# scanner-research/scannertools

Measured on AMD Instinct MI355X. Metric: 1080p frames/sec (optical-flow + histogram ops), higher is better.
Workload: dtype f32 (u8 frames in; the box filter's running sums in f64, re-anchored every 32 rows / 8 columns, column sums handed to the row pass as f32)

## Files before the change

scannertools_amd/csrc/st_context.hip:

```cpp
#include <cstring>
#include <vector>
#include <mutex>
#include <chrono>
#include <cstdlib>

#include "st_internal.h"

int st_set_error(st_ctx* ctx, int status, const char* fmt, ...) {
  char buf[512];
  va_list ap;
  va_start(ap, fmt);
  vsnprintf(buf, sizeof(buf), fmt, ap);
  va_end(ap);
  if (ctx) ctx->last_error = buf;
  return status;
}

int st_enter(st_ctx* ctx) {
  if (!ctx) return ST_ERR_INVALID;
  ST_HIP(ctx, hipSetDevice(ctx->device));
  return ST_OK;
}

namespace {
struct CtxRegistry { std::mutex mu; std::vector<st_ctx*> live; };
CtxRegistry& registry() { static CtxRegistry* r = new CtxRegistry; return *r; }
long long now_ns() {
  return std::chrono::duration_cast<std::chrono::nanoseconds>(std::chrono::steady_clock::now().time_since_epoch()).count();
}
void reg_add(st_ctx* c) { CtxRegistry& r = registry(); std::lock_guard<std::mutex> lk(r.mu); r.live.push_back(c); }
void reg_remove(st_ctx* c) {
  CtxRegistry& r = registry();
  std::lock_guard<std::mutex> lk(r.mu);
  for (size_t i = 0; i < r.live.size(); ++i)
    if (r.live[i] == c) { r.live.erase(r.live.begin() + i); break; }
}
}

bool st_flow_call_begins(st_ctx* ctx) {
  const long long t = now_ns();
  ctx->flow_enter_ns.store(t, std::memory_order_relaxed);
  ctx->flow_busy.store(true, std::memory_order_release);
  if (ctx->concurrency_mode >= 0) return ctx->concurrency_mode != 0;
  constexpr long long kWindowNs = 50LL * 1000 * 1000;
  int others = 0;
  CtxRegistry& r = registry();
  std::lock_guard<std::mutex> lk(r.mu);
  for (st_ctx* o : r.live)
    if (o != ctx && o->device == ctx->device && o->flow_busy.load(std::memory_order_acquire) &&
        t - o->flow_enter_ns.load(std::memory_order_relaxed) < kWindowNs)
      ++others;
  return others >= 2;
}

ST_EXPORT int st_abi_version(void) { return ST_ABI_VERSION; }

#ifndef ST_SRC_HASH
#define ST_SRC_HASH "unknown"
#endif
#ifndef ST_BUILD_HOST
#define ST_BUILD_HOST "unknown"
#endif
#ifndef ST_BUILD_TIME
#define ST_BUILD_TIME "unknown"
#endif
ST_EXPORT const char* st_build_info(void) { return "src=" ST_SRC_HASH " host=" ST_BUILD_HOST " at=" ST_BUILD_TIME; }

ST_EXPORT const char* st_status_string(int status) {
  switch (status) {
    case ST_OK: return "ok";
    case ST_ERR_INVALID: return "invalid argument";
    case ST_ERR_HIP: return "HIP runtime error";
    case ST_ERR_OOM: return "out of device memory";
    case ST_ERR_UNSUPPORTED: return "unsupported parameters";
    default: return "unknown status";
  }
}

ST_EXPORT int st_device_count(int* count) {
  if (!count) return ST_ERR_INVALID;
  int n = 0;
  hipError_t e = hipGetDeviceCount(&n);
  if (e != hipSuccess) { *count = 0; return ST_ERR_HIP; }
  *count = n;
  return ST_OK;
}

static constexpr size_t kMinLdsBytes = 160 * 1024;

ST_EXPORT int st_ctx_create(int device_id, st_ctx** out_ctx) {
  if (!out_ctx) return ST_ERR_INVALID;
  *out_ctx = nullptr;
  int n = 0;
  if (hipGetDeviceCount(&n) != hipSuccess || device_id < 0 || device_id >= n) return ST_ERR_INVALID;
  if (hipSetDevice(device_id) != hipSuccess) return ST_ERR_HIP;
  st_ctx* c = new (std::nothrow) st_ctx();
  if (!c) return ST_ERR_OOM;
  c->device = device_id;
  if (hipStreamCreateWithFlags(&c->own_stream, hipStreamNonBlocking) != hipSuccess) {
    delete c;
    return ST_ERR_HIP;
  }
  c->stream = c->own_stream;
  if (const char* e = getenv("ST_ITER_TILE")) c->tile_mode = atoi(e);
  c->fold_gray = getenv("ST_PYR_FOLD_GRAY") != nullptr;
  if (const char* e = getenv("ST_POLY_U8")) c->poly_u8 = atoi(e) != 0;
  if (const char* e = getenv("ST_ITER_ROLES")) c->roles_mode = atoi(e);
  if (const char* e = getenv("ST_ROLES_NCW")) c->roles_ncw = atoi(e);
  if (const char* e = getenv("ST_PYR_ROLES")) c->pyr_roles = atoi(e);
  if (const char* e = getenv("ST_PYR_ROLES_RGB")) c->pyr_roles_rgb = atoi(e) != 0;
  if (const char* e = getenv("ST_CONV_TILE")) c->conv_tile = atoi(e);
  if (const char* e = getenv("ST_CONCURRENT")) c->concurrency_mode = atoi(e);
  hipDeviceProp_t prop;
  if (hipGetDeviceProperties(&prop, device_id) == hipSuccess) {
    c->num_cus = prop.multiProcessorCount;
    if (prop.sharedMemPerBlock < kMinLdsBytes || strncmp(prop.gcnArchName, "gfx950", 6) != 0) {
      (void)hipStreamDestroy(c->own_stream);
      delete c;
      return ST_ERR_UNSUPPORTED;
    }
  }
  reg_add(c);
  *out_ctx = c;
  return ST_OK;
}

ST_EXPORT int st_ctx_destroy(st_ctx* ctx) {
  if (!ctx) return ST_ERR_INVALID;
  reg_remove(ctx);
  (void)hipSetDevice(ctx->device);
  (void)hipStreamSynchronize(ctx->stream);
  for (auto& t : ctx->timing) {
    for (auto e : t.starts) (void)hipEventDestroy(e);
    for (auto e : t.stops) (void)hipEventDestroy(e);
  }
  if (ctx->ws) (void)hipFree(ctx->ws);
  st_jpeg_release(ctx);
  st_jpeg_enc_release(ctx);
  st_netin_release(ctx);
  st_detect_release(ctx);
  if (ctx->own_stream) (void)hipStreamDestroy(ctx->own_stream);
  delete ctx;
  return ST_OK;
}

ST_EXPORT int st_ctx_set_stream(st_ctx* ctx, void* hip_stream) {
  ST_TRY(st_enter(ctx));
  ST_HIP(ctx, hipStreamSynchronize(ctx->stream));
  ctx->flow_busy.store(false, std::memory_order_release);
  ctx->stream = (hipStream_t)hip_stream;
  return ST_OK;
}

ST_EXPORT int st_ctx_reset_stream(st_ctx* ctx) {
  ST_TRY(st_enter(ctx));
  ST_HIP(ctx, hipStreamSynchronize(ctx->stream));
  ctx->flow_busy.store(false, std::memory_order_release);
  ctx->stream = ctx->own_stream;
  return ST_OK;
}

ST_EXPORT int st_ctx_sync(st_ctx* ctx) {
  ST_TRY(st_enter(ctx));
  ST_HIP(ctx, hipStreamSynchronize(ctx->stream));
  ctx->flow_busy.store(false, std::memory_order_release);
  return ST_OK;
}

ST_EXPORT int st_ctx_flow_concurrent(st_ctx* ctx) { return ctx && ctx->flow_concurrent ? 1 : 0; }

ST_EXPORT int st_ctx_set_workspace_limit(st_ctx* ctx, size_t bytes) {
  if (!ctx) return ST_ERR_INVALID;
  ctx->ws_limit = bytes ? bytes : ((size_t)64 << 30);
  return ST_OK;
}

ST_EXPORT int st_ctx_release_workspace(st_ctx* ctx) {
  ST_TRY(st_enter(ctx));
  ST_HIP(ctx, hipStreamSynchronize(ctx->stream));
  if (ctx->ws) ST_HIP(ctx, hipFree(ctx->ws));
  ctx->ws = nullptr;
  ctx->ws_bytes = 0;
  ctx->ws_off = 0;
  return ST_OK;
}

ST_EXPORT const char* st_ctx_last_error(const st_ctx* ctx) { return ctx ? ctx->last_error.c_str() : "null context"; }

int st_ws_reserve(st_ctx* ctx, size_t total_bytes) {
  ctx->ws_off = 0;
  if (total_bytes <= ctx->ws_bytes) return ST_OK;
  if (total_bytes > ctx->ws_limit)
    return st_set_error(ctx, ST_ERR_OOM, "workspace request %zu exceeds limit %zu", total_bytes, ctx->ws_limit);
  ST_HIP(ctx, hipStreamSynchronize(ctx->stream));
  if (ctx->ws) ST_HIP(ctx, hipFree(ctx->ws));
  ctx->ws = nullptr;
  ctx->ws_bytes = 0;
  size_t want = total_bytes + total_bytes / 8;
  if (want > ctx->ws_limit) want = total_bytes;
  hipError_t e = hipMalloc(&ctx->ws, want);
  if (e != hipSuccess) {
    (void)hipGetLastError();
    want = total_bytes;
    e = hipMalloc(&ctx->ws, want);
  }
  if (e != hipSuccess) {
    (void)hipGetLastError();
    ctx->ws = nullptr;
    return st_set_error(ctx, ST_ERR_OOM, "hipMalloc(%zu) failed: %s", want, hipGetErrorString(e));
  }
  ctx->ws_bytes = want;
  return ST_OK;
}

void st_ws_reset(st_ctx* ctx) { ctx->ws_off = 0; }

void* st_ws_alloc(st_ctx* ctx, size_t bytes) {
  size_t off = st_align_up(ctx->ws_off);
  if (off + bytes > ctx->ws_bytes) return nullptr;
  ctx->ws_off = off + bytes;
  return (char*)ctx->ws + off;
}

ST_EXPORT int st_ctx_timing_enable(st_ctx* ctx, unsigned kernel_mask) {
  if (!ctx) return ST_ERR_INVALID;
  ctx->timing_mask = kernel_mask;
  return ST_OK;
}

static int timing_fold(st_ctx* ctx, st_timing_slot& t) {
  for (size_t i = 0; i < t.used; ++i) {
    float ms = 0.f;
    ST_HIP(ctx, hipEventElapsedTime(&ms, t.starts[i], t.stops[i]));
    t.total_ms += ms;
  }
  t.used = 0;
  return ST_OK;
}

ST_EXPORT int st_ctx_timing_reset(st_ctx* ctx) {
  ST_TRY(st_enter(ctx));
  ST_HIP(ctx, hipStreamSynchronize(ctx->stream));
  for (auto& t : ctx->timing) {
    t.used = 0;
    t.launches = 0;
    t.total_ms = 0.0;
  }
  return ST_OK;
}

ST_EXPORT int st_ctx_timing_read(st_ctx* ctx, int kernel_id, int* launches, double* total_ms) {
  ST_TRY(st_enter(ctx));
  if (kernel_id < 0 || kernel_id >= ST_K_COUNT) return ST_ERR_INVALID;
  ST_HIP(ctx, hipStreamSynchronize(ctx->stream));
  st_timing_slot& t = ctx->timing[kernel_id];
  ST_TRY(timing_fold(ctx, t));
  if (launches) *launches = t.launches;
  if (total_ms) *total_ms = t.total_ms;
  return ST_OK;
}

int st_time_begin(st_ctx* ctx, int id) {
  if (!(ctx->timing_mask & (1u << id))) return ST_OK;
  st_timing_slot& t = ctx->timing[id];
  if (t.used == t.starts.size()) {
    if (t.used >= 4096) {
      ST_HIP(ctx, hipStreamSynchronize(ctx->stream));
      ST_TRY(timing_fold(ctx, t));
    } else {
      hipEvent_t a, b;
      ST_HIP(ctx, hipEventCreate(&a));
      if (hipEventCreate(&b) != hipSuccess) {
        (void)hipEventDestroy(a);
        return st_set_error(ctx, ST_ERR_HIP, "timing: hipEventCreate failed");
      }
      t.starts.push_back(a);
      t.stops.push_back(b);
    }
  }
  ST_HIP(ctx, hipEventRecord(t.starts[t.used], ctx->stream));
  return ST_OK;
}

int st_time_dispatch(st_ctx* ctx, int id, hipEvent_t* start, hipEvent_t* stop) {
  *start = *stop = nullptr;
  if (!(ctx->timing_mask & (1u << id))) return ST_OK;
  st_timing_slot& t = ctx->timing[id];
  if (t.used == t.starts.size()) {
    if (t.used >= 4096) {
      ST_HIP(ctx, hipStreamSynchronize(ctx->stream));
      ST_TRY(timing_fold(ctx, t));
    } else {
      hipEvent_t a, b;
      ST_HIP(ctx, hipEventCreate(&a));
      if (hipEventCreate(&b) != hipSuccess) {
        (void)hipEventDestroy(a);
        return st_set_error(ctx, ST_ERR_HIP, "timing: hipEventCreate failed");
      }
      t.starts.push_back(a);
      t.stops.push_back(b);
    }
  }
  *start = t.starts[t.used];
  *stop = t.stops[t.used];
  t.used++;
  t.launches++;
  return ST_OK;
}

int st_time_end(st_ctx* ctx, int id) {
  if (!(ctx->timing_mask & (1u << id))) return ST_OK;
  st_timing_slot& t = ctx->timing[id];
  if (t.used >= t.stops.size()) return st_set_error(ctx, ST_ERR_INVALID, "timing: bracket closed without an open one");
  ST_HIP(ctx, hipEventRecord(t.stops[t.used], ctx->stream));
  t.used++;
  t.launches++;
  return ST_OK;
}
```

scannertools_amd/csrc/st_farneback.hip:

```cpp
#include <hip/hip_ext.h>

#include <cmath>
#include <cstdlib>
#include <cstring>

#include "st_internal.h"

namespace {

constexpr int kMaxTaps = 32;
constexpr int kMaxPolyN = 7;

inline int cv_round(double v) { return (int)lrint(v); }

struct LevelGeom {
  int lh, lw, ksize;
  double sigma, scale;
};

int fb_levels(int h, int w, const st_fb_params& p) {
  int k;
  double scale = 1;
  for (k = 0; k < p.num_levels; ++k) {
    scale *= p.pyr_scale;
// ... 644 lines not shown
          v.w = (hm[3] + hp[3]) * a.k0[0] + hc[3] * a.k0[1];
          *reinterpret_cast<float4*>(o0 + (size_t)yo * w + X0 + 4 * t) = v;
        }
#pragma unroll
        for (int j = 0; j < 4; ++j) { hm[j] = hc[j]; hc[j] = hp[j]; }
      }
      {
#pragma unroll
        for (int e = 0; e < 2; ++e) {
          const float nA = pf_rowfilter<3>(bb + 3 + 2 * e, a.k1), nB = pf_rowfilter<3>(bb + 4 + 2 * e, a.k1);
#pragma unroll
          for (int j = 0; j < 3; ++j) { r1A[e][j] = r1A[e][j + 1]; r1B[e][j] = r1B[e][j + 1]; }
          r1A[e][3] = nA; r1B[e][3] = nB;
        }
        if ((r & 1) == 0) {
          const int dy = (y - 2) >> 1;
          if (live && dy >= (Y0 >> 1) && dy < (Y1 >> 1)) {
            float2 v;
            {
              const float b00 = pf_colfilter<3>(r1A[0], a.k1), b01 = pf_colfilter<3>(r1B[0], a.k1);
              const float b10 = pf_colfilter<3>(r1A[0] + 1, a.k1), b11 = pf_colfilter<3>(r1B[0] + 1, a.k1);
              v.x = ((b00 + b01) + (b10 + b11)) * 0.25f;
            }
            {
              const float b00 = pf_colfilter<3>(r1A[1], a.k1), b01 = pf_colfilter<3>(r1B[1], a.k1);
              const float b10 = pf_colfilter<3>(r1A[1] + 1, a.k1), b11 = pf_colfilter<3>(r1B[1] + 1, a.k1);
              v.y = ((b00 + b01) + (b10 + b11)) * 0.25f;
            }
            *reinterpret_cast<float2*>(o1 + (size_t)dy * (w >> 1) + (X0 >> 1) + 2 * t) = v;
          }
        }
      }
      {
        const float nA = pf_rowfilter<9>(bb + 1, a.k2), nB = pf_rowfilter<9>(bb + 2, a.k2);
#pragma unroll
        for (int j = 0; j < 9; ++j) { r2A[j] = r2A[j + 1]; r2B[j] = r2B[j + 1]; }
        r2A[9] = nA; r2B[9] = nB;
        if ((r & 3) == 2) {
          const int dy = (y - 6) >> 2;
          if (live && dy >= (Y0 >> 2) && dy < (Y1 >> 2)) {
            const float b00 = pf_colfilter<9>(r2A, a.k2), b01 = pf_colfilter<9>(r2B, a.k2);
            const float b10 = pf_colfilter<9>(r2A + 1, a.k2), b11 = pf_colfilter<9>(r2B + 1, a.k2);
            const float q0 = b00 * 0.5f + b01 * 0.5f, q1 = b10 * 0.5f + b11 * 0.5f;
            o2[(size_t)dy * (w >> 2) + (X0 >> 2) + t] = q0 * 0.5f + q1 * 0.5f;
          }
        }
      }
      {
        unsigned dw[6];
#pragma unroll
        for (int q = 0; q < 6; ++q) dw[q] = s[2 * u + q];
        float cb[21];
#pragma unroll
        for (int q = 0; q < 6; ++q) {
          const unsigned d = __builtin_amdgcn_alignbyte(dw[q + 1 < 6 ? q + 1 : 5], dw[q], (unsigned)half);
#pragma unroll
          for (int k = 0; k < 4; ++k)
            if (4 * q + k < 21) cb[4 * q + k] = pf_byte(d, k);
        }
        const float n3 = pf_rowfilter<19>(cb + 2, a.k3);
#pragma unroll
        for (int j = 0; j < 19; ++j) r3[j] = r3[j + 1];
        r3[19] = n3;
        if (r == 5) {
          const int dy = (y - 13) >> 3;
          if (dy >= (Y0 >> 3) && dy < (Y1 >> 3)) {
            const float c0 = pf_colfilter<19>(r3, a.k3), c1 = pf_colfilter<19>(r3 + 1, a.k3);
            const float p0 = __shfl_xor(c0, 32), p1 = __shfl_xor(c1, 32);
            if (half == 0 && live3) {
              const float q0 = c0 * 0.5f + p0 * 0.5f, q1 = c1 * 0.5f + p1 * 0.5f;
              o3[(size_t)dy * (w >> 3) + (X0 >> 3) + u] = q0 * 0.5f + q1 * 0.5f;
            }
          }
        }
      }
    }
    if (b + 1 < nb) stash(buf ^ 1);
    __syncthreads();
  }
}

typedef unsigned pf_u3nt __attribute__((ext_vector_type(3), aligned(4)));
__device__ __forceinline__ pf_u3nt pf_fetch_rgb(const uint8_t* __restrict__ row, int col0, int w, const PyrFusedArgs& a) {
  if (col0 >= 0 && col0 + 3 < w) return __builtin_nontemporal_load(reinterpret_cast<const pf_u3nt*>(row + 3 * col0));
  pf_u3nt v = {0u, 0u, 0u};
  if (col0 >= w + 8 || col0 < -8) return v;
#pragma unroll
  for (int k = 0; k < 4; ++k) v.x |= pf_gray1(row + 3 * d_reflect101(col0 + k, w), a) << (8 * k);
  return v;
}
__device__ __forceinline__ unsigned pf_gray_of(pf_u3nt v, bool inside, const PyrFusedArgs& a) {
  if (!inside) return v.x;
  const unsigned w0 = v.x, w1 = v.y, w2 = v.z;
  const int g0 = (int)((w0 & 0xff) * a.cb + ((w0 >> 8) & 0xff) * a.cg + ((w0 >> 16) & 0xff) * a.cr + a.rnd) >> a.shift;
  const int g1 = (int)((w0 >> 24) * a.cb + (w1 & 0xff) * a.cg + ((w1 >> 8) & 0xff) * a.cr + a.rnd) >> a.shift;
  const int g2 = (int)(((w1 >> 16) & 0xff) * a.cb + (w1 >> 24) * a.cg + (w2 & 0xff) * a.cr + a.rnd) >> a.shift;
  const int g3 = (int)(((w2 >> 8) & 0xff) * a.cb + ((w2 >> 16) & 0xff) * a.cg + (w2 >> 24) * a.cr + a.rnd) >> a.shift;
  return (unsigned)g0 | ((unsigned)g1 << 8) | ((unsigned)g2 << 16) | ((unsigned)g3 << 24);
}

template <int ROLE, bool L0 = true, bool RGB = false>
__device__ __forceinline__ void pyr_role_run(const PyrFusedArgs& a, unsigned (*srow)[PF_RB][PF_ROWDW]) {
  const int t = threadIdx.x & 255, lane = t & 63, wv = t >> 6;
  const int h = a.h, w = a.w;
  const int SW = a.strip_w;
  const int X0 = blockIdx.x * SW;
  const int Y0 = blockIdx.y * a.rows_per_seg, Y1 = min(h, Y0 + a.rows_per_seg);
  const size_t np = (size_t)h * w;
  const uint8_t* __restrict__ g = RGB ? st_gl(a.frames[blockIdx.z]) : a.gray + (size_t)blockIdx.z * np;
  const int gw = RGB ? 3 * w : w;
  float* __restrict__ o0 = a.img0 + (size_t)blockIdx.z * np;
  float* __restrict__ o1 = a.img1 + (size_t)blockIdx.z * (np >> 2);
  float* __restrict__ o2 = a.img2 + (size_t)blockIdx.z * (np >> 4);
  float* __restrict__ o3 = a.img3 + (size_t)blockIdx.z * (np >> 6);
  const int u = wv * 32 + (lane & 31), half = lane >> 5;
  const bool live = 4 * t < SW && X0 + 4 * t < w;
  const bool live3 = 8 * u < SW && X0 + 8 * u < w;
  const int hq = t & 3, hrow = (t >> 2) & 7;
  const int hcol = hq < 2 ? X0 - 8 + 4 * hq : X0 + SW + 4 * (hq - 2);
  const int hidx = hq < 2 ? hq : 2 + (SW >> 2) + (hq - 2);
  const bool in_t = X0 + 4 * t + 3 < w, in_h = hcol >= 0 && hcol + 3 < w;
  uint8_t* __restrict__ gout = RGB ? a.gray_out + (size_t)blockIdx.z * np : nullptr;

  unsigned pre[3], preh = 0u;
  pf_u3nt raw[3] = {{0u, 0u, 0u}, {0u, 0u, 0u}, {0u, 0u, 0u}}, rawh = {0u, 0u, 0u};
  auto fetch = [&](int ybase) {
#pragma unroll
    for (int j = 0; j < 3; ++j) {
      const int r = ROLE + 3 * j;
      if (r < PF_RB) {
        if (RGB) { if (4 * t < SW) raw[j] = pf_fetch_rgb(g + (size_t)d_reflect101(ybase + r, h) * gw, X0 + 4 * t, w, a); }
        else pre[j] = pf_load4(g + (size_t)d_reflect101(ybase + r, h) * gw, X0 + 4 * t, w);
      }
    }
    if (ROLE == 0 && t < 32) {
      if (RGB) rawh = pf_fetch_rgb(g + (size_t)d_reflect101(ybase + hrow, h) * gw, hcol, w, a);
      else preh = pf_load4(g + (size_t)d_reflect101(ybase + hrow, h) * gw, hcol, w);
    }
  };
  auto stash = [&](int buf, int ybase) {
    const bool own = RGB && ybase >= Y0 && ybase < Y1;
    if (4 * t < SW) {
#pragma unroll
      for (int j = 0; j < 3; ++j) {
        const int r = ROLE + 3 * j;
        if (r < PF_RB) {
          const unsigned v = RGB ? pf_gray_of(raw[j], in_t, a) : pre[j];
          srow[buf][r][2 + t] = v;
          if (RGB && own && live) *reinterpret_cast<unsigned*>(gout + (size_t)(ybase + r) * w + X0 + 4 * t) = v;
        }
      }
    }
    if (ROLE == 0 && t < 32) srow[buf][hrow][hidx] = RGB ? pf_gray_of(rawh, in_h, a) : preh;
  };

  float hm[4], hc[4], r1A[2][4], r1B[2][4];
  float r2A[10], r2B[10];
  float r3[20];
  if (ROLE == 0) {
#pragma unroll
    for (int j = 0; j < 4; ++j) { hm[j] = hc[j] = 0.f; r1A[0][j] = r1A[1][j] = r1B[0][j] = r1B[1][j] = 0.f; }
  } else if (ROLE == 1) {
#pragma unroll
    for (int j = 0; j < 10; ++j) r2A[j] = r2B[j] = 0.f;
  } else {
#pragma unroll
    for (int j = 0; j < 20; ++j) r3[j] = 0.f;
  }

  const int nb = (Y1 - Y0) / PF_RB + 2;
  fetch(Y0 - PF_RB);
  stash(0, Y0 - PF_RB);
  __syncthreads();
  for (int b = 0; b < nb; ++b) {
    const int ybase = Y0 - PF_RB + b * PF_RB;
    const int buf = b & 1;
    if (b + 1 < nb) fetch(ybase + PF_RB);
#pragma unroll
    for (int r = 0; r < PF_RB; ++r) {
      const int y = ybase + r;
      const unsigned* __restrict__ s = srow[buf][r];
      if (ROLE == 0) {
        const unsigned d0 = s[t + 1], d1 = s[t + 2], d2 = s[t + 3];
        float bb[12];
#pragma unroll
        for (int k = 0; k < 4; ++k) { bb[k] = pf_byte(d0, k); bb[4 + k] = pf_byte(d1, k); bb[8 + k] = pf_byte(d2, k); }
        if (L0) {
          float hp[4];
#pragma unroll
          for (int j = 0; j < 4; ++j) hp[j] = bb[4 + j] * a.k0[1] + (bb[3 + j] + bb[5 + j]) * a.k0[0];
          const int yo = y - 1;
          if (live && yo >= Y0 && yo < Y1) {
            float4 v;
            v.x = (hm[0] + hp[0]) * a.k0[0] + hc[0] * a.k0[1];
            v.y = (hm[1] + hp[1]) * a.k0[0] + hc[1] * a.k0[1];
            v.z = (hm[2] + hp[2]) * a.k0[0] + hc[2] * a.k0[1];
            v.w = (hm[3] + hp[3]) * a.k0[0] + hc[3] * a.k0[1];
            *reinterpret_cast<float4*>(o0 + (size_t)yo * w + X0 + 4 * t) = v;
          }
#pragma unroll
          for (int j = 0; j < 4; ++j) { hm[j] = hc[j]; hc[j] = hp[j]; }
        }
        {
#pragma unroll
          for (int e = 0; e < 2; ++e) {
            const float nA = pf_rowfilter<3>(bb + 3 + 2 * e, a.k1), nB = pf_rowfilter<3>(bb + 4 + 2 * e, a.k1);
#pragma unroll
            for (int j = 0; j < 3; ++j) { r1A[e][j] = r1A[e][j + 1]; r1B[e][j] = r1B[e][j + 1]; }
            r1A[e][3] = nA; r1B[e][3] = nB;
          }
          if ((r & 1) == 0) {
            const int dy = (y - 2) >> 1;
            if (live && dy >= (Y0 >> 1) && dy < (Y1 >> 1)) {
              float2 v;
              {
                const float b00 = pf_colfilter<3>(r1A[0], a.k1), b01 = pf_colfilter<3>(r1B[0], a.k1);
                const float b10 = pf_colfilter<3>(r1A[0] + 1, a.k1), b11 = pf_colfilter<3>(r1B[0] + 1, a.k1);
                v.x = ((b00 + b01) + (b10 + b11)) * 0.25f;
              }
              {
                const float b00 = pf_colfilter<3>(r1A[1], a.k1), b01 = pf_colfilter<3>(r1B[1], a.k1);
                const float b10 = pf_colfilter<3>(r1A[1] + 1, a.k1), b11 = pf_colfilter<3>(r1B[1] + 1, a.k1);
                v.y = ((b00 + b01) + (b10 + b11)) * 0.25f;
              }
              *reinterpret_cast<float2*>(o1 + (size_t)dy * (w >> 1) + (X0 >> 1) + 2 * t) = v;
            }
          }
        }
      } else if (ROLE == 1) {
        const unsigned d0 = s[t + 1], d1 = s[t + 2], d2 = s[t + 3];
        float bb[12];
#pragma unroll
        for (int k = 0; k < 4; ++k) { bb[k] = pf_byte(d0, k); bb[4 + k] = pf_byte(d1, k); bb[8 + k] = pf_byte(d2, k); }
        const float nA = pf_rowfilter<9>(bb + 1, a.k2), nB = pf_rowfilter<9>(bb + 2, a.k2);
#pragma unroll
        for (int j = 0; j < 9; ++j) { r2A[j] = r2A[j + 1]; r2B[j] = r2B[j + 1]; }
        r2A[9] = nA; r2B[9] = nB;
        if ((r & 3) == 2) {
          const int dy = (y - 6) >> 2;
          if (live && dy >= (Y0 >> 2) && dy < (Y1 >> 2)) {
            const float b00 = pf_colfilter<9>(r2A, a.k2), b01 = pf_colfilter<9>(r2B, a.k2);
            const float b10 = pf_colfilter<9>(r2A + 1, a.k2), b11 = pf_colfilter<9>(r2B + 1, a.k2);
            const float q0 = b00 * 0.5f + b01 * 0.5f, q1 = b10 * 0.5f + b11 * 0.5f;
            o2[(size_t)dy * (w >> 2) + (X0 >> 2) + t] = q0 * 0.5f + q1 * 0.5f;
          }
        }
      } else {
        unsigned dw[6];
#pragma unroll
        for (int q = 0; q < 6; ++q) dw[q] = s[2 * u + q];
        float cb[21];
#pragma unroll
        for (int q = 0; q < 6; ++q) {
          const unsigned d = __builtin_amdgcn_alignbyte(dw[q + 1 < 6 ? q + 1 : 5], dw[q], (unsigned)half);
#pragma unroll
          for (int k = 0; k < 4; ++k)
            if (4 * q + k < 21) cb[4 * q + k] = pf_byte(d, k);
        }
        const float n3 = pf_rowfilter<19>(cb + 2, a.k3);
#pragma unroll
        for (int j = 0; j < 19; ++j) r3[j] = r3[j + 1];
        r3[19] = n3;
        if (r == 5) {
          const int dy = (y - 13) >> 3;
          if (dy >= (Y0 >> 3) && dy < (Y1 >> 3)) {
            const float c0 = pf_colfilter<19>(r3, a.k3), c1 = pf_colfilter<19>(r3 + 1, a.k3);
            const float p0 = __shfl_xor(c0, 32), p1 = __shfl_xor(c1, 32);
            if (half == 0 && live3) {
              const float q0 = c0 * 0.5f + p0 * 0.5f, q1 = c1 * 0.5f + p1 * 0.5f;
              o3[(size_t)dy * (w >> 3) + (X0 >> 3) + u] = q0 * 0.5f + q1 * 0.5f;
            }
          }
        }
      }
    }
    if (b + 1 < nb) stash(buf ^ 1, ybase + PF_RB);
    __syncthreads();
  }
}

template <bool L0, bool RGB = false>
__global__ __launch_bounds__(768) void k_pyr_roles(PyrFusedArgs a) {
  static_assert(!(L0 && RGB), "the RGB-source instance leaves level 0 to k_polyexp_u8");
  __shared__ unsigned srow[2][PF_RB][PF_ROWDW];
  const int role = threadIdx.x >> 8;
  if (role == 0) pyr_role_run<0, L0, RGB>(a, srow);
  else if (role == 1) pyr_role_run<1, true, RGB>(a, srow);
  else pyr_role_run<2, true, RGB>(a, srow);
}

typedef float f2u __attribute__((ext_vector_type(2), aligned(4)));
typedef float f4v16 __attribute__((ext_vector_type(4)));
__device__ __forceinline__ __amdgpu_buffer_rsrc_t st_rsrc(const void* base, size_t bytes) {
  return __builtin_amdgcn_make_buffer_rsrc(const_cast<void*>(base), 0, (int)(bytes > 0xfffffffcull ? 0xfffffffcull : bytes), 0x00020000);
}
__device__ __forceinline__ float bld1(__amdgpu_buffer_rsrc_t r, unsigned voff, unsigned soff) {
  return __builtin_bit_cast(float, __builtin_amdgcn_raw_buffer_load_b32(r, (int)voff, (int)soff, 0));
}
template <int AUX = 0>
__device__ __forceinline__ void bst1(__amdgpu_buffer_rsrc_t r, unsigned voff, unsigned soff, float v) {
  __builtin_amdgcn_raw_buffer_store_b32(__builtin_bit_cast(unsigned, v), r, (int)voff, (int)soff, AUX);
}
template <int AUX = 0>
__device__ __forceinline__ void bst4(__amdgpu_buffer_rsrc_t r, unsigned voff, float4 v) {
  typedef unsigned u4 __attribute__((ext_vector_type(4)));
  u4 q;
  q.x = __builtin_bit_cast(unsigned, v.x); q.y = __builtin_bit_cast(unsigned, v.y);
  q.z = __builtin_bit_cast(unsigned, v.z); q.w = __builtin_bit_cast(unsigned, v.w);
  __builtin_amdgcn_raw_buffer_store_b128(q, r, (int)voff, 0, AUX);
}

__device__ __forceinline__ float ldf(const float* __restrict__ base, unsigned byte_off) {
  return *reinterpret_cast<const float*>(reinterpret_cast<const char*>(base) + byte_off);
}
__device__ __forceinline__ f2u ldf2(const float* __restrict__ base, unsigned byte_off) {
  return *reinterpret_cast<const f2u*>(reinterpret_cast<const char*>(base) + byte_off);
}
__device__ __forceinline__ float4 ldf4(const float* __restrict__ base, unsigned byte_off) {
  return *reinterpret_cast<const float4*>(reinterpret_cast<const char*>(base) + byte_off);
}



struct PolyArgs {
  const float* img;
  const uint8_t* gray;
  float* R;
  int h, w, rows_per_seg;
  PolyCoef c;
};

constexpr int PE_RB = 4;
constexpr int PE_OUT = 240;

template <int N, class A, bool U8 = false>
__device__ __forceinline__ void polyexp_body(const A& a, const float* __restrict__ img, float* __restrict__ Rbase, int h, int w,
                                             int rows_per_seg, int bx, int by, int z, const uint8_t* __restrict__ gray = nullptr) {
  constexpr int PXW = 3 * PE_RB + 1;
  __shared__ float sv[2][256 * PXW];
  const int tid = threadIdx.x;
  const int np = h * w;
  const float* __restrict__ I = img + (size_t)z * (size_t)np;
  float* __restrict__ R = Rbase + (size_t)z * 5 * (size_t)np;
  const int x = bx * PE_OUT - N + tid;
  const int xc = d_clamp(x, 0, w - 1);
  const int y0 = by * rows_per_seg;
  const int y1 = min(h, y0 + rows_per_seg);
  const bool writer = tid >= N && tid < N + PE_OUT && x < w;
  const unsigned voff = 4u * (unsigned)xc;
  const unsigned xo = writer ? (unsigned)x : 0u;
  const unsigned xo16 = writer ? 16u * xo : 0x80000000u, xo4 = writer ? 4u * xo : 0x80000000u;
  const __amdgpu_buffer_rsrc_t Rnull = st_rsrc(R, 0);
  const __amdgpu_buffer_rsrc_t Ib = st_rsrc(I, 4 * (size_t)np), Rb = st_rsrc(R, 20 * (size_t)np);
  auto opaque = [](unsigned v) { asm volatile("" : "+v"(v)); return v; };
  auto src = [&](int row) { return bld1(Ib, voff, 4u * (unsigned)w * (unsigned)d_clamp(row, 0, h - 1)); };
  const __amdgpu_buffer_rsrc_t Gb = st_rsrc(U8 ? gray + (size_t)z * (size_t)np : nullptr, U8 ? (size_t)np : 0);
  const unsigned lx = !U8 ? 0u : xc == 0 ? 0u : xc >= w - 2 ? (unsigned)(w - 4) : (unsigned)(xc - 1);
  const unsigned wsel = xc == 0 ? 0x00000202u : xc == w - 1 ? 0x02020000u : xc == w - 2 ? 0x01020100u : 0x00010201u;
  auto graw = [&](int grow) { return (unsigned)__builtin_amdgcn_raw_buffer_load_b32(Gb, (int)lx, (int)((unsigned)w * (unsigned)grow), 0); };
  auto hsum = [&](unsigned d) { return __builtin_amdgcn_udot4(d, wsel, 0u, false); };
  auto blur16 = [](unsigned a0, unsigned b0, unsigned c0) { return (float)(a0 + 2u * b0 + c0) * 0.0625f; };
  unsigned hsB = 0, hsC = 0;

  float ring[2 * N + PE_RB];
  if (!U8) {
#pragma unroll
    for (int j = 0; j < 2 * N + PE_RB; ++j) ring[j] = src(y0 - N + j);
  } else {
    constexpr int NR = 2 * N + PE_RB;
    const int r0 = d_clamp(y0 - N, 0, h - 1);
    const unsigned rm = graw(d_reflect101(r0 - 1, h)), rc = graw(r0);
    unsigned rn[NR];
#pragma unroll
    for (int j = 0; j < NR; ++j) rn[j] = graw(d_reflect101(d_clamp(y0 - N + j, 0, h - 1) + 1, h));
    unsigned hsA = hsum(rm);
    hsB = hsum(rc);
#pragma unroll
    for (int j = 0; j < NR; ++j) {
      hsC = hsum(rn[j]);
      ring[j] = blur16(hsA, hsB, hsC);
      if (j + 1 < NR && d_clamp(y0 - N + j + 1, 0, h - 1) != d_clamp(y0 - N + j, 0, h - 1)) { hsA = hsB; hsB = hsC; }
    }
  }

  int buf = 0;
  for (int y = y0; y < y1; y += PE_RB) {
#pragma unroll
    for (int r = 0; r < PE_RB; ++r) {
      float r0 = ring[r + N] * a.c.g[0], r1 = 0.f, r2 = 0.f;
#pragma unroll
      for (int k = 1; k <= N; ++k) {
        float p = ring[r + N - k] + ring[r + N + k];
        float t0 = r0 + a.c.g[k] * p;
        float t1 = r2 + a.c.xxg[k] * p;
        p = ring[r + N + k] - ring[r + N - k];
        float t2 = r1 + a.c.xg[k] * p;
        r0 = t0; r1 = t2; r2 = t1;
      }
      float* __restrict__ d = &sv[buf][tid * PXW + 3 * r];
      d[0] = r0; d[1] = r1; d[2] = r2;
    }
    float nxt[PE_RB];
    unsigned nraw[PE_RB];
#pragma unroll
    for (int r = 0; r < PE_RB; ++r) {
      if (U8) nraw[r] = graw(d_reflect101(min(y + PE_RB + N + r, h - 1) + 1, h));
      else nxt[r] = src(y + PE_RB + N + r);
    }
    __syncthreads();
    if (U8) {
      float last = ring[2 * N + PE_RB - 1];
#pragma unroll
      for (int r = 0; r < PE_RB; ++r) {
        if (y + PE_RB + N + r <= h - 1) {
          const unsigned hsA = hsB;
          hsB = hsC; hsC = hsum(nraw[r]);
          last = blur16(hsA, hsB, hsC);
        }
        nxt[r] = last;
      }
    }
#pragma unroll
    for (int j = 0; j < 2 * N; ++j) ring[j] = ring[j + PE_RB];
#pragma unroll
    for (int r = 0; r < PE_RB; ++r) ring[2 * N + r] = nxt[r];
    __builtin_amdgcn_sched_barrier(0);
    {
      const unsigned pix0 = opaque(writer ? (unsigned)(tid - N) * PXW : 0u);
#pragma unroll
      for (int r = 0; r < PE_RB; ++r) {
        const float* __restrict__ s = &sv[buf][pix0 + 3 * r];
        float g0 = a.c.g[0];
        const float cx = s[N * PXW], cy = s[N * PXW + 1], cz = s[N * PXW + 2];
        double b1 = cx * g0, b2 = 0, b3 = cy * g0, b4 = 0, b5 = cz * g0, b6 = 0;
#pragma unroll
        for (int k = 1; k <= N; ++k) {
          const float* __restrict__ pp = s + (N + k) * PXW;
          const float* __restrict__ mm = s + (N - k) * PXW;
          const float p0 = pp[0], m0 = mm[0];
          const float p1 = pp[1], m1 = mm[1];
          const float p2 = pp[2], m2 = mm[2];
          double tg = p0 + m0;
          g0 = a.c.g[k];
          b1 = __builtin_fma(tg, (double)g0, b1);
          b4 = __builtin_fma(tg, (double)a.c.xxg[k], b4);
          b2 += (p0 - m0) * a.c.xg[k];
          b3 += (p1 + m1) * g0;
          b6 += (p1 - m1) * a.c.xg[k];
          b5 += (p2 + m2) * g0;
        }
        const bool row_ok = y + r < y1;
        const unsigned rowo = (unsigned)(y + r) * (unsigned)w;
        bst4(row_ok ? Rb : Rnull, xo16 + 16u * rowo, make_float4((float)(b3 * a.c.ig11), (float)(b2 * a.c.ig11),
                                                                                  (float)(b1 * a.c.ig03 + b5 * a.c.ig33), (float)(b1 * a.c.ig03 + b4 * a.c.ig33)));
        bst1(row_ok ? Rb : Rnull, xo4, 16u * (unsigned)np + 4u * rowo, (float)(b6 * a.c.ig55));
      }
    }
    buf ^= 1;
  }
}

template <int N>
__global__ __launch_bounds__(256) void k_polyexp(PolyArgs a) {
  polyexp_body<N>(a, a.img, a.R, a.h, a.w, a.rows_per_seg, (int)blockIdx.x, (int)blockIdx.y, (int)blockIdx.z);
}

template <int N>
__global__ __launch_bounds__(256, 1) void k_polyexp_u8(PolyArgs a) {
  polyexp_body<N, PolyArgs, true>(a, nullptr, a.R, a.h, a.w, a.rows_per_seg, (int)blockIdx.x, (int)blockIdx.y, (int)blockIdx.z, a.gray);
}

struct PolyLevel {
  const float* img;
  float* R;
  int h, w, rows_per_seg, strips, block0;
};
struct PolyArgsML {
  PolyLevel lv[4];
  int nlv;
  PolyCoef c;
};
template <int N>
__global__ __launch_bounds__(256) void k_polyexp_ml(PolyArgsML a) {
  int l = 0;
#pragma unroll
  for (int i = 1; i < 4; ++i)
    if (i < a.nlv && (int)blockIdx.x >= a.lv[i].block0) l = i;
  const float* img = a.lv[0].img; float* R = a.lv[0].R;
  int h = a.lv[0].h, w = a.lv[0].w, rows = a.lv[0].rows_per_seg, strips = a.lv[0].strips, b0 = a.lv[0].block0;
#pragma unroll
  for (int i = 1; i < 4; ++i)
    if (l == i) { img = a.lv[i].img; R = a.lv[i].R; h = a.lv[i].h; w = a.lv[i].w; rows = a.lv[i].rows_per_seg; strips = a.lv[i].strips; b0 = a.lv[i].block0; }
  const int local = (int)blockIdx.x - b0;
  polyexp_body<N>(a, img, R, h, w, rows, local % strips, local / strips, (int)blockIdx.y);
}

__device__ __forceinline__ void update_matrices_px(const float* __restrict__ R0, const float* __restrict__ R1,
                                                   int np, int h, int w, int x, int y, float dx, float dy,
                                                   float m[5]) {
  const int o = y * w + x;
  float fx = x + dx, fy = y + dy;
  const int x1 = (int)floorf(fx), y1 = (int)floorf(fy);
  float r2, r3, r4, r5, r6;
  fx -= x1; fy -= y1;
  const float4 q = reinterpret_cast<const float4*>(R0)[o];
  const float q0 = q.x, q1 = q.y, q2 = q.z, q3 = q.w, q4 = R0[4 * (size_t)np + o];
  if ((unsigned)x1 < (unsigned)(w - 1) && (unsigned)y1 < (unsigned)(h - 1)) {
    const float a00 = (1.f - fx) * (1.f - fy), a01 = fx * (1.f - fy), a10 = (1.f - fx) * fy, a11 = fx * fy;
    const int gi = y1 * w + x1;
    const float4* __restrict__ Q = reinterpret_cast<const float4*>(R1);
    const float* __restrict__ S = R1 + 4 * (size_t)np;
    const float4 t0 = Q[gi], t1 = Q[gi + 1], b0 = Q[gi + w], b1 = Q[gi + w + 1];
    r2 = a00 * t0.x + a01 * t1.x + a10 * b0.x + a11 * b1.x;
    r3 = a00 * t0.y + a01 * t1.y + a10 * b0.y + a11 * b1.y;
    r4 = a00 * t0.z + a01 * t1.z + a10 * b0.z + a11 * b1.z;
    r5 = a00 * t0.w + a01 * t1.w + a10 * b0.w + a11 * b1.w;
    r6 = a00 * S[gi] + a01 * S[gi + 1] + a10 * S[gi + w] + a11 * S[gi + w + 1];
    r4 = (q2 + r4) * 0.5f;
    r5 = (q3 + r5) * 0.5f;
    r6 = (q4 + r6) * 0.25f;
  } else {
    r2 = r3 = 0.f;
    r4 = q2;
    r5 = q3;
    r6 = q4 * 0.5f;
  }
  r2 = (q0 - r2) * 0.5f;
  r3 = (q1 - r3) * 0.5f;
  r2 += r4 * dy + r6 * dx;
  r3 += r6 * dy + r5 * dx;
  constexpr int BORDER = 5;
  if ((unsigned)(x - BORDER) >= (unsigned)(w - BORDER * 2) || (unsigned)(y - BORDER) >= (unsigned)(h - BORDER * 2)) {
    auto bsel = [](int i) -> float { return i < 2 ? 0.14f : 0.4472f; };
    const float scale = (x < BORDER ? bsel(x) : 1.f) * (x >= w - BORDER ? bsel(w - x - 1) : 1.f) *
                        (y < BORDER ? bsel(y) : 1.f) * (y >= h - BORDER ? bsel(h - y - 1) : 1.f);
    r2 *= scale; r3 *= scale; r4 *= scale; r5 *= scale; r6 *= scale;
  }
  m[0] = r4 * r4 + r6 * r6;
  m[1] = (r4 + r5) * r6;
  m[2] = r5 * r5 + r6 * r6;
  m[3] = r4 * r2 + r6 * r3;
  m[4] = r6 * r2 + r5 * r3;
}


struct UmLoads {
  float4 q;
  float qs;
  float4 t0, t1, b0, b1;
  f2u ts, bs;
};

__device__ __forceinline__ void um_gather(const float* __restrict__ R1, unsigned single, unsigned gi, unsigned gb, UmLoads& L);
__device__ __forceinline__ void um_issue(const float* __restrict__ R0, const float* __restrict__ R1, int np, int h,
                                         int w, int x, int y, float2 f, UmLoads& L) {
  float fx = x + f.x, fy = y + f.y;
  const int x1 = (int)floorf(fx), y1 = (int)floorf(fy);
  const bool inb = (unsigned)x1 < (unsigned)(w - 1) && (unsigned)y1 < (unsigned)(h - 1);
  const unsigned gi = inb ? (unsigned)(y1 * w + x1) : 0u;
  const unsigned gb = gi + (inb ? (unsigned)w : 0u);
  const unsigned o = (unsigned)(y * w + x);
  const unsigned single = 16u * (unsigned)np;
  L.q = ldf4(R0, 16u * o);
  L.qs = ldf(R0, single + 4u * o);
  um_gather(R1, single, gi, gb, L);
}

__device__ __forceinline__ void um_gather(const float* __restrict__ R1, unsigned single, unsigned gi, unsigned gb, UmLoads& L) {
  L.t0 = ldf4(R1, 16u * gi);
  L.t1 = ldf4(R1 + 4, 16u * gi);
  L.b0 = ldf4(R1, 16u * gb);
  L.b1 = ldf4(R1 + 4, 16u * gb);
  L.ts = ldf2(R1, single + 4u * gi);
  L.bs = ldf2(R1, single + 4u * gb);
}

__device__ __forceinline__ void um_finish(const UmLoads& L, int h, int w, int x, int y, float2 f, float m[5]) {
  const float dx = f.x, dy = f.y;
  float fx = x + dx, fy = y + dy;
  const int x1 = (int)floorf(fx), y1 = (int)floorf(fy);
  fx -= x1; fy -= y1;
  const bool inb = (unsigned)x1 < (unsigned)(w - 1) && (unsigned)y1 < (unsigned)(h - 1);
  float r2, r3, r4, r5, r6;
  if (inb) {
    const float a00 = (1.f - fx) * (1.f - fy), a01 = fx * (1.f - fy), a10 = (1.f - fx) * fy, a11 = fx * fy;
    r2 = a00 * L.t0.x + a01 * L.t1.x + a10 * L.b0.x + a11 * L.b1.x;
    r3 = a00 * L.t0.y + a01 * L.t1.y + a10 * L.b0.y + a11 * L.b1.y;
    r4 = a00 * L.t0.z + a01 * L.t1.z + a10 * L.b0.z + a11 * L.b1.z;
    r5 = a00 * L.t0.w + a01 * L.t1.w + a10 * L.b0.w + a11 * L.b1.w;
    r6 = a00 * L.ts.x + a01 * L.ts.y + a10 * L.bs.x + a11 * L.bs.y;
    r4 = (L.q.z + r4) * 0.5f;
    r5 = (L.q.w + r5) * 0.5f;
    r6 = (L.qs + r6) * 0.25f;
  } else {
    r2 = r3 = 0.f;
    r4 = L.q.z;
    r5 = L.q.w;
    r6 = L.qs * 0.5f;
  }
  r2 = (L.q.x - r2) * 0.5f;
  r3 = (L.q.y - r3) * 0.5f;
  r2 += r4 * dy + r6 * dx;
  r3 += r6 * dy + r5 * dx;
  constexpr int BORDER = 5;
  if ((unsigned)(x - BORDER) >= (unsigned)(w - BORDER * 2) || (unsigned)(y - BORDER) >= (unsigned)(h - BORDER * 2)) {
    auto bsel = [](int i) -> float { return i < 2 ? 0.14f : 0.4472f; };
    const float scale = (x < BORDER ? bsel(x) : 1.f) * (x >= w - BORDER ? bsel(w - x - 1) : 1.f) *
                        (y < BORDER ? bsel(y) : 1.f) * (y >= h - BORDER ? bsel(h - y - 1) : 1.f);
    r2 *= scale; r3 *= scale; r4 *= scale; r5 *= scale; r6 *= scale;
  }
  m[0] = r4 * r4 + r6 * r6;
  m[1] = (r4 + r5) * r6;
  m[2] = r5 * r5 + r6 * r6;
  m[3] = r4 * r2 + r6 * r3;
  m[4] = r6 * r2 + r5 * r3;
}


struct UMArgs {
  const float* R;
  const int* pairs;
  const float* R1_direct;
  const float* flow;
  const float* coarse;
  float* M;
  int h, w, ch, cw;
  double scale_x, scale_y;
  float mul;
};

__device__ __forceinline__ float2 ld_flow(const float* __restrict__ f, int idx) {
  return *reinterpret_cast<const float2*>(reinterpret_cast<const char*>(f) + 8u * (unsigned)idx);
}

__global__ __launch_bounds__(256) void k_update_matrices(UMArgs a) {
  const int h = a.h, w = a.w;
  const size_t np = (size_t)h * w;
  const int pr = blockIdx.y;
  const float* R0;
  const float* R1;
  if (a.pairs) {
    R0 = a.R + (size_t)a.pairs[2 * pr] * 5 * np;
    R1 = a.R + (size_t)a.pairs[2 * pr + 1] * 5 * np;
  } else {
    R0 = a.R;
    R1 = a.R1_direct;
  }
  float* __restrict__ M = a.M + (size_t)pr * 5 * np;
  for (size_t i = (size_t)blockIdx.x * blockDim.x + threadIdx.x; i < np; i += (size_t)gridDim.x * blockDim.x) {
    const int y = (int)(i / w), x = (int)(i - (size_t)y * w);
    float dx = 0.f, dy = 0.f;
    if (a.coarse) {
      const float* C = a.coarse + (size_t)pr * 2 * a.ch * a.cw;
      float fx = (float)((x + 0.5) * a.scale_x - 0.5);
      int sx = (int)floorf(fx);
      fx -= sx;
      if (sx < 0) { fx = 0.f; sx = 0; }
      if (sx >= a.cw - 1) { fx = 0.f; sx = a.cw - 1; }
      float fy = (float)((y + 0.5) * a.scale_y - 0.5);
      int sy = (int)floorf(fy);
      fy -= sy;
      const int ya = d_clamp(sy, 0, a.ch - 1), yb = d_clamp(sy + 1, 0, a.ch - 1);
      const float a1 = fx, a0 = 1.f - fx, b0 = 1.f - fy, b1 = fy;
      float2 ta, tb;
      if (sx + 1 < a.cw) {
        float2 p = ld_flow(C, ya * a.cw + sx), q = ld_flow(C, ya * a.cw + sx + 1);
        ta.x = p.x * a0 + q.x * a1; ta.y = p.y * a0 + q.y * a1;
        p = ld_flow(C, yb * a.cw + sx); q = ld_flow(C, yb * a.cw + sx + 1);
        tb.x = p.x * a0 + q.x * a1; tb.y = p.y * a0 + q.y * a1;
      } else {
        float2 p = ld_flow(C, ya * a.cw + sx);
        ta.x = p.x * 1.f; ta.y = p.y * 1.f;
        p = ld_flow(C, yb * a.cw + sx);
        tb.x = p.x * 1.f; tb.y = p.y * 1.f;
      }
      dx = (ta.x * b0 + tb.x * b1) * a.mul;
      dy = (ta.y * b0 + tb.y * b1) * a.mul;
    } else if (a.flow) {
      float2 f = ld_flow(a.flow + (size_t)pr * 2 * np, (int)i);
      dx = f.x; dy = f.y;
    }
    float m[5];
    update_matrices_px(R0, R1, np, h, w, x, y, dx, dy, m);
    M[i] = m[0]; M[np + i] = m[1]; M[2 * np + i] = m[2]; M[3 * np + i] = m[3]; M[4 * np + i] = m[4];
  }
}

struct BlurArgs {
  const float* R;
  const int* pairs;
  const float* R1_direct;
  const float* Min;
  float* Mout;
  float* flow;
  float* const* flow_ptrs;
  int h, w, rows_per_seg, m;
  int update, write_flow;
  double scale;
};

constexpr int BLUR_T = 256;

__global__ __launch_bounds__(BLUR_T) void k_blur_update(BlurArgs a) {
  __shared__ double sv[2][5][BLUR_T];
  const int tid = threadIdx.x;
  const int h = a.h, w = a.w, m = a.m;
  const size_t np = (size_t)h * w;
  const int pr = blockIdx.z;
  const float* __restrict__ Min = a.Min + (size_t)pr * 5 * np;
  const int x = (int)blockIdx.x * (BLUR_T - 2 * m) - m + tid;
  const int xc = d_clamp(x, 0, w - 1);
  const int y0 = blockIdx.y * a.rows_per_seg;
  const int y1 = min(h, y0 + a.rows_per_seg);
  const bool writer = tid >= m && tid < BLUR_T - m && x < w;

  const float* R0 = nullptr;
  const float* R1 = nullptr;
  float* Mout = nullptr;
  if (a.update) {
    if (a.pairs) {
      R0 = a.R + (size_t)a.pairs[2 * pr] * 5 * np;
      R1 = a.R + (size_t)a.pairs[2 * pr + 1] * 5 * np;
    } else {
      R0 = a.R;
      R1 = a.R1_direct;
    }
    Mout = a.Mout + (size_t)pr * 5 * np;
  }
  float* flow = nullptr;
  if (a.write_flow) flow = a.flow_ptrs ? st_gl(a.flow_ptrs[pr]) : a.flow + (size_t)pr * 2 * np;

  double vs[5] = {0, 0, 0, 0, 0};
  if (y0 == 0) {
#pragma unroll
    for (int c = 0; c < 5; ++c) vs[c] = (double)(Min[c * np + xc] * (float)(m + 2));
    for (int yy = 1; yy < m; ++yy) {
      const size_t o = (size_t)min(yy, h - 1) * w + xc;
#pragma unroll
      for (int c = 0; c < 5; ++c) vs[c] += (double)Min[c * np + o];
    }
    const size_t oa = (size_t)min(m, h - 1) * w + xc;
#pragma unroll
    for (int c = 0; c < 5; ++c) {
      const float d = Min[c * np + oa] - Min[c * np + xc];
      vs[c] += d;
    }
  } else {
    for (int dy = -m; dy <= m; ++dy) {
      const size_t o = (size_t)d_clamp(y0 + dy, 0, h - 1) * w + xc;
#pragma unroll
      for (int c = 0; c < 5; ++c) vs[c] += (double)Min[c * np + o];
    }
  }

  for (int y = y0; y < y1; ++y) {
    double(*s)[BLUR_T] = sv[y & 1];
#pragma unroll
    for (int c = 0; c < 5; ++c) s[c][tid] = vs[c];
    if (y + 1 < y1) {
      const size_t oa = (size_t)d_clamp(y + 1 + m, 0, h - 1) * w + xc;
      const size_t ob = (size_t)d_clamp(y - m, 0, h - 1) * w + xc;
#pragma unroll
      for (int c = 0; c < 5; ++c) {
        const float d = Min[c * np + oa] - Min[c * np + ob];
        vs[c] += d;
      }
    }
    __syncthreads();
    if (writer) {
      double g[5];
#pragma unroll
      for (int c = 0; c < 5; ++c) {
        double t = s[c][tid - m];
        for (int k = -m + 1; k <= m; ++k) t += s[c][tid + k];
        g[c] = t * a.scale;
      }
      const double idet = 1. / (g[0] * g[2] - g[1] * g[1] + 1e-3);
      const float u = (float)((g[0] * g[4] - g[1] * g[3]) * idet);
      const float v = (float)((g[2] * g[3] - g[1] * g[4]) * idet);
      const size_t o = (size_t)y * w + x;
      if (flow) *reinterpret_cast<float2*>(flow + 2 * o) = make_float2(u, v);
      if (a.update) {
        float mm[5];
        update_matrices_px(R0, R1, np, h, w, x, y, u, v, mm);
#pragma unroll
        for (int c = 0; c < 5; ++c) Mout[c * np + o] = mm[c];
      }
    }
  }
}

constexpr int B2_T = 256, B2_HALO = 8, B2_OUT = B2_T - 2 * B2_HALO, B2_RB = 5, B2_SEG = 5;
constexpr int B2_NSEG = B2_OUT / B2_SEG;

template <int M>
__global__ __launch_bounds__(B2_T, 2) void k_blur_update_v2(BlurArgs a) {
  constexpr int W = 2 * M + 1;
  static_assert(W % B2_RB == 0 && M <= B2_HALO, "ring period must be a multiple of the batch");
  __shared__ float V[B2_RB][5][B2_T];
  __shared__ float2 F[B2_RB][B2_T];
  const int tid = threadIdx.x;
  const int h = a.h, w = a.w;
  const int np = h * w;
  const int pr = blockIdx.z;
  const float* __restrict__ Min = a.Min + (size_t)pr * 5 * (size_t)np;
  const int x = (int)blockIdx.x * B2_OUT - B2_HALO + tid;
  const int xc = d_clamp(x, 0, w - 1);
  const int y0 = blockIdx.y * a.rows_per_seg;
  const int y1 = min(h, y0 + a.rows_per_seg);
  const bool writer = tid >= B2_HALO && tid < B2_T - B2_HALO && x < w;

  const float* R0 = nullptr;
  const float* R1 = nullptr;
  float* Mout = nullptr;
  if (a.update) {
    if (a.pairs) {
      R0 = a.R + (size_t)a.pairs[2 * pr] * 5 * (size_t)np;
      R1 = a.R + (size_t)a.pairs[2 * pr + 1] * 5 * (size_t)np;
    } else {
      R0 = a.R;
      R1 = a.R1_direct;
    }
    Mout = a.Mout + (size_t)pr * 5 * (size_t)np;
  }
  float* flow = nullptr;
  if (a.write_flow) flow = a.flow_ptrs ? st_gl(a.flow_ptrs[pr]) : a.flow + (size_t)pr * 2 * (size_t)np;

  float ring[W][5];
  double vs[5];
#pragma unroll
  for (int s = 0; s < W; ++s) {
    const int o = d_clamp(y0 - M + s, 0, h - 1) * w + xc;
#pragma unroll
    for (int c = 0; c < 5; ++c) ring[s][c] = Min[c * np + o];
  }
  if (y0 == 0) {
#pragma unroll
    for (int c = 0; c < 5; ++c) vs[c] = (double)(ring[M][c] * (float)(M + 2));
#pragma unroll
    for (int yy = 1; yy < M; ++yy)
#pragma unroll
      for (int c = 0; c < 5; ++c) vs[c] += (double)ring[M + yy][c];
#pragma unroll
    for (int c = 0; c < 5; ++c) {
      const float d = ring[2 * M][c] - ring[M][c];
      vs[c] += d;
    }
  } else {
#pragma unroll
    for (int c = 0; c < 5; ++c) vs[c] = 0;
#pragma unroll
    for (int s = 0; s < W; ++s)
#pragma unroll
      for (int c = 0; c < 5; ++c) vs[c] += (double)ring[s][c];
  }

  for (int yb = y0; yb < y1; yb += W) {
#pragma unroll
    for (int b = 0; b < W / B2_RB; ++b) {
      const int ybb = yb + b * B2_RB;
      if (ybb < y1) {
        float nw[B2_RB][5];
#pragma unroll
        for (int r = 0; r < B2_RB; ++r) {
          const int o = d_clamp(ybb + r + M + 1, 0, h - 1) * w + xc;
#pragma unroll
          for (int c = 0; c < 5; ++c) nw[r][c] = Min[c * np + o];
        }
#pragma unroll
        for (int r = 0; r < B2_RB; ++r) {
#pragma unroll
          for (int c = 0; c < 5; ++c) {
            V[r][c][tid] = (float)vs[c];
            const float d = nw[r][c] - ring[b * B2_RB + r][c];
            vs[c] += d;
            ring[b * B2_RB + r][c] = nw[r][c];
          }
        }
        __syncthreads();
        if (tid < B2_RB * B2_NSEG) {
          const int r = tid / B2_NSEG, sg = tid - r * B2_NSEG;
          const int j0 = B2_HALO + sg * B2_SEG;
          double t[5];
#pragma unroll
          for (int c = 0; c < 5; ++c) {
            const float* vp = &V[r][c][j0 - M];
            double acc = vp[0];
#pragma unroll
            for (int i = 1; i < W; ++i) acc += (double)vp[i];
            t[c] = acc;
            __builtin_amdgcn_sched_barrier(0);
          }
#pragma unroll
          for (int i = 0; i < B2_SEG; ++i) {
            if (i > 0) {
#pragma unroll
              for (int c = 0; c < 5; ++c) t[c] += (double)V[r][c][j0 + i + M] - (double)V[r][c][j0 + i - M - 1];
            }
            const double g11 = t[0] * a.scale, g12 = t[1] * a.scale, g22 = t[2] * a.scale;
            const double h1 = t[3] * a.scale, h2 = t[4] * a.scale;
            const double idet = 1. / (g11 * g22 - g12 * g12 + 1e-3);
            F[r][j0 + i] = make_float2((float)((g11 * h2 - g12 * h1) * idet), (float)((g22 * h1 - g12 * h2) * idet));
            __builtin_amdgcn_sched_barrier(0);
          }
        }
        __syncthreads();
        if (writer) {
#pragma unroll
          for (int r = 0; r < B2_RB; ++r) {
            const int y = ybb + r;
            if (y < y1) {
              const float2 f = F[r][tid];
              const int o = y * w + x;
              if (flow) *reinterpret_cast<float2*>(flow + 2 * o) = f;
              if (a.update) {
                float mm[5];
                update_matrices_px(R0, R1, np, h, w, x, y, f.x, f.y, mm);
#pragma unroll
                for (int c = 0; c < 5; ++c) Mout[c * np + o] = mm[c];
              }
            }
          }
        }
      }
    }
  }
}

struct IterArgs {
  const float* R;
  const int* pairs;
  const float* R1_direct;
  const float* flow_in;
  const float* coarse;
  float* flow_out;
  float* const* flow_ptrs;
  int h, w, ch, cw, rows_per_seg;
  int out_w;
  double scale_x, scale_y;
  float mul;
  double scale;
};

enum { FLOW_ZERO = 0, FLOW_FIELD = 1, FLOW_COARSE = 2, FLOW_ANY = 3,
       FLOW_COARSE2 = 4 };

struct CoarseX {
  int sx;
  float a0, a1;
  bool pair;
};

__device__ __forceinline__ CoarseX coarse_x(const IterArgs& a, int x) {
  CoarseX cx;
  float fx = (float)((x + 0.5) * a.scale_x - 0.5);
  int sx = (int)floorf(fx);
  fx -= sx;
  if (sx < 0) { fx = 0.f; sx = 0; }
  if (sx >= a.cw - 1) { fx = 0.f; sx = a.cw - 1; }
  cx.sx = sx; cx.a1 = fx; cx.a0 = 1.f - fx; cx.pair = sx + 1 < a.cw;
  return cx;
}

typedef float f4u8 __attribute__((ext_vector_type(4), aligned(8)));
struct FlowRaw {
  f4u8 pa, pb;
};

template <int MODE = FLOW_ANY>
__device__ __forceinline__ void flow_issue(const IterArgs& a, const float* __restrict__ fin,
                                           const float* __restrict__ C, const CoarseX& cx, int x, int y, FlowRaw& r) {
  if (MODE == FLOW_COARSE || MODE == FLOW_COARSE2 || (MODE == FLOW_ANY && C)) {
    const float fy = (float)((y + 0.5) * a.scale_y - 0.5);
    const int sy = (int)floorf(fy);
    const int ya = d_clamp(sy, 0, a.ch - 1), yb = d_clamp(sy + 1, 0, a.ch - 1);
    if (cx.pair) {
      r.pa = *reinterpret_cast<const f4u8*>(reinterpret_cast<const char*>(C) + 8u * (unsigned)(ya * a.cw + cx.sx));
      r.pb = *reinterpret_cast<const f4u8*>(reinterpret_cast<const char*>(C) + 8u * (unsigned)(yb * a.cw + cx.sx));
    } else {
      float2 p = ld_flow(C, ya * a.cw + cx.sx);
      r.pa.x = p.x; r.pa.y = p.y; r.pa.z = 0.f; r.pa.w = 0.f;
      p = ld_flow(C, yb * a.cw + cx.sx);
      r.pb.x = p.x; r.pb.y = p.y; r.pb.z = 0.f; r.pb.w = 0.f;
    }
  } else if (MODE == FLOW_FIELD || (MODE == FLOW_ANY && fin)) {
    const float2 p = ld_flow(fin, y * a.w + x);
    r.pa.x = p.x; r.pa.y = p.y;
  }
}

template <int MODE = FLOW_ANY>
__device__ __forceinline__ float2 flow_finish(const IterArgs& a, const float* __restrict__ fin,
                                              const float* __restrict__ C, const CoarseX& cx, int y, const FlowRaw& r) {
  if (MODE == FLOW_COARSE || MODE == FLOW_COARSE2 || (MODE == FLOW_ANY && C)) {
    float fy = (float)((y + 0.5) * a.scale_y - 0.5);
    const int sy = (int)floorf(fy);
    fy -= sy;
    const float a1 = cx.a1, a0 = cx.a0, b0 = 1.f - fy, b1 = fy;
    float2 ta, tb;
    if (cx.pair) {
      ta.x = r.pa.x * a0 + r.pa.z * a1; ta.y = r.pa.y * a0 + r.pa.w * a1;
      tb.x = r.pb.x * a0 + r.pb.z * a1; tb.y = r.pb.y * a0 + r.pb.w * a1;
    } else {
      ta.x = r.pa.x * 1.f; ta.y = r.pa.y * 1.f;
      tb.x = r.pb.x * 1.f; tb.y = r.pb.y * 1.f;
    }
    return make_float2((ta.x * b0 + tb.x * b1) * a.mul, (ta.y * b0 + tb.y * b1) * a.mul);
  }
  if (MODE == FLOW_FIELD || (MODE == FLOW_ANY && fin)) return make_float2(r.pa.x, r.pa.y);
  return make_float2(0.f, 0.f);
}

__device__ __forceinline__ int coarse_row0(const IterArgs& a, int y0) {
  return (int)floorf((float)((y0 + 0.5) * a.scale_y - 0.5));
}

template <int MODE = FLOW_ANY>
__device__ __forceinline__ float2 iter_flow_at(const IterArgs& a, const float* __restrict__ fin,
                                               const float* __restrict__ C, const CoarseX& cx, int x, int y) {
  FlowRaw r;
  flow_issue<MODE>(a, fin, C, cx, x, y, r);
  return flow_finish<MODE>(a, fin, C, cx, y, r);
}

constexpr int F3_GROUP = 8, F3_SW = 8, F3_NSEG = B2_OUT / F3_SW, F3_RING = 16, F3_ANCHOR = 32;
constexpr int F3_PADW = B2_T + B2_T / 8;
static_assert(B2_OUT % F3_SW == 0 && F3_GROUP * F3_NSEG <= B2_T && F3_ANCHOR % F3_RING == 0 && F3_RING % F3_GROUP == 0, "bad v3 geometry");
__device__ __forceinline__ constexpr int f3_pos(int x) { return x + (x >> 3); }

__device__ __forceinline__ int coarse2_row(int y) { return ((y + 1) >> 1) - 1; }

template <int RB>
struct FlowRawN {
  f4u8 row[RB / 2 + 2];
};
template <int RB>
__device__ __forceinline__ void coarseN_issue(const IterArgs& a, const float* __restrict__ C, const CoarseX& cx, int y0,
                                              FlowRawN<RB>& r) {
  const int s = coarse2_row(y0);
#pragma unroll
  for (int j = 0; j < RB / 2 + 2; ++j) {
    const int yy = d_clamp(s + j, 0, a.ch - 1);
    if (cx.pair) {
      r.row[j] = *reinterpret_cast<const f4u8*>(reinterpret_cast<const char*>(C) + 8u * (unsigned)(yy * a.cw + cx.sx));
    } else {
      const float2 p = ld_flow(C, yy * a.cw + cx.sx);
      r.row[j].x = p.x; r.row[j].y = p.y; r.row[j].z = 0.f; r.row[j].w = 0.f;
    }
  }
}
template <int RB>
__device__ __forceinline__ void coarse2_finish_batch(const IterArgs& a, const CoarseX& cx, int y0, const int (&ys)[RB],
                                                     const FlowRawN<RB>& r, float2 (&out)[RB]) {
  const int s = coarse2_row(y0);
  const float a1 = cx.a1, a0 = cx.a0;
  float2 hx[RB / 2 + 2];
#pragma unroll
  for (int j = 0; j < RB / 2 + 2; ++j) {
    if (cx.pair) {
      hx[j].x = r.row[j].x * a0 + r.row[j].z * a1; hx[j].y = r.row[j].y * a0 + r.row[j].w * a1;
    } else {
      hx[j].x = r.row[j].x * 1.f; hx[j].y = r.row[j].y * 1.f;
    }
  }
#pragma unroll
  for (int i = 0; i < RB; ++i) {
    const int y = ys[i];
    const int idx = coarse2_row(y) - s;
    const float fy = (y & 1) ? 0.25f : 0.75f;
    const float b0 = 1.f - fy, b1 = fy;
    float2 ta = hx[0], tb = hx[1];
#pragma unroll
    for (int j = 1; j <= RB / 2; ++j)
      if (idx == j) { ta = hx[j]; tb = hx[j + 1]; }
    out[i] = make_float2((ta.x * b0 + tb.x * b1) * a.mul, (ta.y * b0 + tb.y * b1) * a.mul);
  }
}

struct Coarse2Window {
  float2 hx0, hx1;
  f4u8 raw;
};
__device__ __forceinline__ void coarse2_row_issue(const IterArgs& a, const float* __restrict__ C, const CoarseX& cx, int u,
                                                  f4u8& r) {
  const int yy = d_clamp(u, 0, a.ch - 1);
  if (cx.pair) {
    r = *reinterpret_cast<const f4u8*>(reinterpret_cast<const char*>(C) + 8u * (unsigned)(yy * a.cw + cx.sx));
  } else {
    const float2 p = ld_flow(C, yy * a.cw + cx.sx);
    r.x = p.x; r.y = p.y; r.z = 0.f; r.w = 0.f;
  }
}
__device__ __forceinline__ float2 coarse2_row_hx(const CoarseX& cx, const f4u8& r) {
  float2 hx;
  if (cx.pair) {
    hx.x = r.x * cx.a0 + r.z * cx.a1; hx.y = r.y * cx.a0 + r.w * cx.a1;
  } else {
    hx.x = r.x * 1.f; hx.y = r.y * 1.f;
  }
  return hx;
}
__device__ __forceinline__ void coarse2_window_start(const IterArgs& a, const float* __restrict__ C, const CoarseX& cx,
                                                     int yu, Coarse2Window& win) {
  const int u = coarse2_row(yu);
  f4u8 r0, r1;
  coarse2_row_issue(a, C, cx, u, r0);
  coarse2_row_issue(a, C, cx, u + 1, r1);
  coarse2_row_issue(a, C, cx, u + 2, win.raw);
  win.hx0 = coarse2_row_hx(cx, r0);
  win.hx1 = coarse2_row_hx(cx, r1);
}
__device__ __forceinline__ void coarse2_window_batch(const IterArgs& a, const float* __restrict__ C, const CoarseX& cx, int yu,
                                                     Coarse2Window& win, float2 (&out)[2]) {
  const int u = coarse2_row(yu);
  const float2 hx2 = coarse2_row_hx(cx, win.raw);
#pragma unroll
  for (int i = 0; i < 2; ++i) {
    const int y = min(yu + i, a.h - 1);
    const bool second = coarse2_row(yu + i) > u;
    const float fy = (y & 1) ? 0.25f : 0.75f;
    const float b0 = 1.f - fy, b1 = fy;
    const float2 ta = second ? win.hx1 : win.hx0, tb = second ? hx2 : win.hx1;
    out[i] = make_float2((ta.x * b0 + tb.x * b1) * a.mul, (ta.y * b0 + tb.y * b1) * a.mul);
  }
  win.hx0 = win.hx1;
  win.hx1 = hx2;
  coarse2_row_issue(a, C, cx, u + 3, win.raw);
}

template <int RB>
__device__ __forceinline__ float2 coarseN_finish(const IterArgs& a, const CoarseX& cx, int y0, int y, const FlowRawN<RB>& r) {
  float fy = (float)((y + 0.5) * a.scale_y - 0.5);
  const int sy = (int)floorf(fy);
  fy -= sy;
  const int idx = sy - coarse_row0(a, y0);
  f4u8 pa = r.row[0], pb = r.row[1];
#pragma unroll
  for (int j = 1; j <= RB / 2; ++j)
    if (idx == j) { pa = r.row[j]; pb = r.row[j + 1]; }
  const float a1 = cx.a1, a0 = cx.a0, b0 = 1.f - fy, b1 = fy;
  float2 ta, tb;
  if (cx.pair) {
    ta.x = pa.x * a0 + pa.z * a1; ta.y = pa.y * a0 + pa.w * a1;
    tb.x = pb.x * a0 + pb.z * a1; tb.y = pb.y * a0 + pb.w * a1;
  } else {
    ta.x = pa.x * 1.f; ta.y = pa.y * 1.f;
    tb.x = pb.x * 1.f; tb.y = pb.y * 1.f;
  }
  return make_float2((ta.x * b0 + tb.x * b1) * a.mul, (ta.y * b0 + tb.y * b1) * a.mul);
}

__device__ __forceinline__ void xcd_remap(unsigned& bx, unsigned& by, unsigned& bz) {
  const unsigned gx = gridDim.x, gy = gridDim.y, gz = gridDim.z;
  const unsigned C = gx * gy, N = C * gz;
  if (N % 8u) return;
  const unsigned L = bx + gx * (by + gy * bz), xcd = L % 8u, slot = L / 8u;
  unsigned col, pair;
  if (C % 8u == 0) {
    const unsigned cpx = C / 8u;
    col = xcd + 8u * (slot % cpx);
    pair = slot / cpx;
  } else if (8u % C == 0 && gz % (8u / C) == 0) {
    col = xcd % C;
    pair = (xcd / C) * (gz / (8u / C)) + slot;
  } else {
    return;
  }
  bx = col % gx; by = col / gx; bz = pair;
}

template <int MODE>
__global__ __launch_bounds__(B2_T, 2) void k_flow_iter3(IterArgs a) {
  typedef float f2v __attribute__((ext_vector_type(2)));
  constexpr int M = 7, W = 2 * M + 1, RB = 2;
  static_assert(W == F3_RING - 1 && F3_GROUP % RB == 0 && M <= B2_HALO, "ring of 16 = window of 15 + the entering row");
  __shared__ float Vs[F3_GROUP][5][F3_PADW];
  __shared__ float2 Fs[F3_GROUP][F3_PADW];
  const int tid = threadIdx.x;
  const int h = a.h, w = a.w;
  const int np = h * w;
  unsigned bx = blockIdx.x, by = blockIdx.y, bz = blockIdx.z;
  xcd_remap(bx, by, bz);
  const int pr = bz;
  const int x = (int)bx * B2_OUT - B2_HALO + tid;
  const int xc = d_clamp(x, 0, w - 1);
  const int y0 = by * a.rows_per_seg;
  const int y1 = by + 1 == gridDim.y ? h : min(h, y0 + a.rows_per_seg);
  const bool writer = tid >= B2_HALO && tid < B2_T - B2_HALO && x < w;
  const int vpos = f3_pos(tid);
  typedef float f4v __attribute__((ext_vector_type(4), aligned(8)));
  const bool pair_tid = tid >= B2_HALO && tid < B2_T - B2_HALO;
  const int pair_k = pair_tid ? tid - B2_HALO : 0, pair_j = pair_k % (B2_OUT / 2);
  const int pair_r0 = (pair_k / (B2_OUT / 2)) * (F3_GROUP / 2);
  const int pair_x = (int)bx * B2_OUT + 2 * pair_j;
  const int pair_pos = f3_pos(B2_HALO + 2 * pair_j);

  const float* __restrict__ R0;
  const float* __restrict__ R1;
  if (a.pairs) {
    R0 = a.R + (size_t)a.pairs[2 * pr] * 5 * (size_t)np;
    R1 = a.R + (size_t)a.pairs[2 * pr + 1] * 5 * (size_t)np;
  } else {
    R0 = a.R;
    R1 = a.R1_direct;
  }
  const float* __restrict__ fin = a.flow_in ? a.flow_in + (size_t)pr * 2 * (size_t)np : nullptr;
  const float* __restrict__ C = a.coarse ? a.coarse + (size_t)pr * 2 * (size_t)a.ch * a.cw : nullptr;
  float* fout = a.flow_ptrs ? st_gl(a.flow_ptrs[pr]) : a.flow_out + (size_t)pr * 2 * (size_t)np;
  const CoarseX cx = (MODE == FLOW_COARSE || MODE == FLOW_COARSE2) ? coarse_x(a, xc) : CoarseX{0, 1.f, 0.f, false};

  float ring[F3_RING][5];
#pragma unroll
  for (int s0 = 0; s0 < W; s0 += 3) {
    UmLoads Li[3];
    float2 f[3];
#pragma unroll
    for (int i = 0; i < 3; ++i) {
      const int yy = d_clamp(y0 - M + s0 + i, 0, h - 1);
      f[i] = iter_flow_at<MODE>(a, fin, C, cx, xc, yy);
      um_issue(R0, R1, np, h, w, xc, yy, f[i], Li[i]);
    }
#pragma unroll
    for (int i = 0; i < 3; ++i) um_finish(Li[i], h, w, xc, d_clamp(y0 - M + s0 + i, 0, h - 1), f[i], ring[s0 + i]);
    __builtin_amdgcn_sched_barrier(0);
  }
#pragma unroll
  for (int c = 0; c < 5; ++c) ring[F3_RING - 1][c] = 0.f;
  double vs[5];
  if (y0 == 0) {
#pragma unroll
    for (int c = 0; c < 5; ++c) vs[c] = (double)(ring[M][c] * (float)(M + 2));
#pragma unroll
    for (int yy = 1; yy < M; ++yy)
#pragma unroll
      for (int c = 0; c < 5; ++c) vs[c] += (double)ring[M + yy][c];
#pragma unroll
    for (int c = 0; c < 5; ++c) {
      const float d = ring[2 * M][c] - ring[M][c];
      vs[c] += d;
    }
  } else {
#pragma unroll
    for (int c = 0; c < 5; ++c) vs[c] = 0;
#pragma unroll
    for (int s = 0; s < W; ++s)
#pragma unroll
      for (int c = 0; c < 5; ++c) vs[c] += (double)ring[s][c];
  }

  float2 fcur[RB], fnext[RB];
  UmLoads L[RB];
#pragma unroll
  for (int r = 0; r < RB; ++r) {
    fcur[r] = iter_flow_at<MODE>(a, fin, C, cx, xc, d_clamp(y0 + r + M + 1, 0, h - 1));
    um_issue(R0, R1, np, h, w, xc, d_clamp(y0 + r + M + 1, 0, h - 1), fcur[r], L[r]);
  }
#pragma unroll
  for (int r = 0; r < RB; ++r) fnext[r] = iter_flow_at<MODE>(a, fin, C, cx, xc, d_clamp(y0 + RB + r + M + 1, 0, h - 1));
  static_assert(RB == 2, "Coarse2Window moves one coarse row per batch of two fine rows");
  FlowRaw raw[MODE == FLOW_COARSE2 ? 1 : RB];
  Coarse2Window win;
  if (MODE == FLOW_COARSE2) {
    coarse2_window_start(a, C, cx, y0 + 2 * RB + M + 1, win);
  } else {
#pragma unroll
    for (int r = 0; r < RB; ++r) flow_issue<MODE>(a, fin, C, cx, xc, d_clamp(y0 + 2 * RB + r + M + 1, 0, h - 1), raw[r]);
  }

#pragma unroll 1
  for (int ybase = y0; ybase < y1; ybase += F3_RING) {
    if (ybase > y0 && (ybase - y0) % F3_ANCHOR == 0) {
#pragma unroll
      for (int c = 0; c < 5; ++c) vs[c] = 0;
#pragma unroll
      for (int s = 0; s < W; ++s) {
#pragma unroll
        for (int c = 0; c < 5; ++c) vs[c] += (double)ring[s][c];
        __builtin_amdgcn_sched_barrier(0);
      }
    }
#pragma unroll
    for (int g = 0; g < F3_RING / F3_GROUP; ++g) {
      const int yg = ybase + g * F3_GROUP;
      if (yg >= y1) break;
      if (yg > y0) {
        if (!(w & 1)) {
          if (pair_x < w && pair_tid) {
#pragma unroll
            for (int r = 0; r < F3_GROUP / 2; ++r) {
              const int rr = pair_r0 + r;
              const float2 fa = Fs[rr][pair_pos], fb = Fs[rr][pair_pos + 1];
              f4v v4;
              v4.x = fa.x; v4.y = fa.y; v4.z = fb.x; v4.w = fb.y;
              __builtin_nontemporal_store(v4, reinterpret_cast<f4v*>(fout + 2 * (size_t)((yg - F3_GROUP + rr) * w + pair_x)));
            }
          }
        } else if (writer) {
#pragma unroll
          for (int r = 0; r < F3_GROUP; ++r) {
            const float2 fv = Fs[r][vpos];
            f2v v2;
            v2.x = fv.x; v2.y = fv.y;
            __builtin_nontemporal_store(v2, reinterpret_cast<f2v*>(fout + 2 * (size_t)((yg - F3_GROUP + r) * w + x)));
          }
        }
      }
      __builtin_amdgcn_s_setprio(2);
#pragma unroll
      for (int bb = 0; bb < F3_GROUP / RB; ++bb) {
        const int ybb = yg + bb * RB;
#pragma unroll
        for (int r = 0; r < RB; ++r) {
          const int t = g * F3_GROUP + bb * RB + r;
          float m[5];
          um_finish(L[r], h, w, xc, d_clamp(ybb + r + M + 1, 0, h - 1), fcur[r], m);
#pragma unroll
          for (int c = 0; c < 5; ++c) {
            Vs[bb * RB + r][c][vpos] = (float)vs[c];
            const float d = m[c] - ring[t % F3_RING][c];
            vs[c] += d;
            ring[(t + W) % F3_RING][c] = m[c];
          }
          fcur[r] = fnext[r];
          um_issue(R0, R1, np, h, w, xc, d_clamp(ybb + RB + r + M + 1, 0, h - 1), fcur[r], L[r]);
        }
        if (MODE == FLOW_COARSE2) {
          coarse2_window_batch(a, C, cx, ybb + 2 * RB + M + 1, win, fnext);
        } else {
#pragma unroll
          for (int r = 0; r < RB; ++r) fnext[r] = flow_finish<MODE>(a, fin, C, cx, d_clamp(ybb + 2 * RB + r + M + 1, 0, h - 1), raw[MODE == FLOW_COARSE2 ? 0 : r]);
#pragma unroll
          for (int r = 0; r < RB; ++r) flow_issue<MODE>(a, fin, C, cx, xc, d_clamp(ybb + 3 * RB + r + M + 1, 0, h - 1), raw[MODE == FLOW_COARSE2 ? 0 : r]);
        }
      }
      __builtin_amdgcn_s_setprio(0);
      __syncthreads();
      if (tid < F3_GROUP * F3_NSEG) {
        const int r = tid / F3_NSEG, sg = tid - r * F3_NSEG;
        const int j0 = B2_HALO + sg * F3_SW;
        const float* __restrict__ vrow = &Vs[r][0][j0 + (j0 >> 3)];
        double t[5];
#pragma unroll
        for (int c = 0; c < 5; ++c) {
          const float* vp = vrow + c * F3_PADW;
          double acc = vp[-8];
#pragma unroll
          for (int k = -6; k <= 7; ++k) acc += (double)vp[k < 0 ? k - 1 : k];
          t[c] = acc;
          __builtin_amdgcn_sched_barrier(0);
        }
#pragma unroll
        for (int i = 0; i < F3_SW; ++i) {
          if (i > 0) {
#pragma unroll
            for (int c = 0; c < 5; ++c) {
              const float* vp = vrow + c * F3_PADW;
              const int ke = i + 7, kl = i - 8;
              t[c] += (double)vp[ke >= 8 ? ke + 1 : ke] - (double)vp[kl < 0 ? (kl < -8 ? kl - 2 : kl - 1) : kl];
            }
          }
          const double g11 = t[0] * a.scale, g12 = t[1] * a.scale, g22 = t[2] * a.scale;
          const double h1 = t[3] * a.scale, h2 = t[4] * a.scale;
          const double idet = d_rcp_pos(g11 * g22 - g12 * g12 + 1e-3);
          Fs[r][j0 + (j0 >> 3) + i] = make_float2((float)((g11 * h2 - g12 * h1) * idet), (float)((g22 * h1 - g12 * h2) * idet));
          __builtin_amdgcn_sched_barrier(0);
        }
      }
      __syncthreads();
    }
  }
  if (writer) {
    const int ylast = y0 + ((y1 - y0 - 1) / F3_GROUP) * F3_GROUP;
#pragma unroll
    for (int r = 0; r < F3_GROUP; ++r) {
      const int y = ylast + r;
      if (y < y1) *reinterpret_cast<float2*>(fout + 2 * (size_t)(y * w + x)) = Fs[r][vpos];
    }
  }
}

constexpr int FR_G = 4;
template <int NCW>
struct FrGeom {
  static constexpr int COLS = 64 * NCW, OUTMAX = COLS - 2 * B2_HALO, PADW = COLS + COLS / 8;
  static constexpr int NSEGMAX = OUTMAX / F3_SW;
  static constexpr int THREADS = 3 * COLS;
  static_assert(FR_G * 2 * NSEGMAX <= COLS, "one solver thread per (row, half segment)");
  static_assert(THREADS <= 1024, "workgroup size");
};

template <int NCW, int MODE>
__global__ __launch_bounds__((FrGeom<NCW>::THREADS)) void k_flow_iter_roles(IterArgs a) {
  typedef FrGeom<NCW> G;
  constexpr int M = 7, W = 15, RB = 2;
  static_assert(FR_G % RB == 0, "a step is a whole number of batches");
  __shared__ float Mb[2][FR_G][5][G::COLS];
  __shared__ float Vs[3][FR_G][5][G::PADW];
  __shared__ double Ts[2][FR_G][2 * G::NSEGMAX][5];
  const int tid = threadIdx.x;
  const int role = tid < G::COLS ? 0 : (tid < 2 * G::COLS ? 1 : 2);
  const int h = a.h, w = a.w;
  const int np = h * w;
  unsigned bx = blockIdx.x, by = blockIdx.y, bz = blockIdx.z;
  xcd_remap(bx, by, bz);
  const int pr = bz;
  const int y0 = by * a.rows_per_seg;
  const int y1 = min(h, y0 + a.rows_per_seg);
  const int SM = 4 + (y1 - y0 + FR_G - 1) / FR_G;
  const int T = SM + 3;
  const int nseg = a.out_w / F3_SW;

  if (role == 0) {
    const int t = tid;
    const int x = (int)bx * a.out_w - B2_HALO + t;
    const int xc = d_clamp(x, 0, min(w - 1, (int)bx * a.out_w + a.out_w + B2_HALO - 1));
    const float* __restrict__ R0;
    const float* __restrict__ R1;
    if (a.pairs) {
      R0 = a.R + (size_t)a.pairs[2 * pr] * 5 * (size_t)np;
      R1 = a.R + (size_t)a.pairs[2 * pr + 1] * 5 * (size_t)np;
    } else {
      R0 = a.R;
      R1 = a.R1_direct;
    }
    const float* __restrict__ fin = a.flow_in ? a.flow_in + (size_t)pr * 2 * (size_t)np : nullptr;
    const float* __restrict__ C = a.coarse ? a.coarse + (size_t)pr * 2 * (size_t)a.ch * a.cw : nullptr;
    const CoarseX cx = (MODE == FLOW_COARSE || MODE == FLOW_COARSE2) ? coarse_x(a, xc) : CoarseX{0, 1.f, 0.f, false};
    constexpr int NB = FR_G / RB;
    auto rowk = [&](int k) { return d_clamp(y0 - 8 + k, 0, h - 1); };
    float2 fcur[RB], fnext[RB];
    UmLoads L[RB];
    FlowRaw raw[MODE == FLOW_COARSE2 ? 1 : RB];
    FlowRawN<RB> rawn;
#pragma unroll
    for (int r = 0; r < RB; ++r) {
      fcur[r] = iter_flow_at<MODE>(a, fin, C, cx, xc, rowk(r));
      um_issue(R0, R1, np, h, w, xc, rowk(r), fcur[r], L[r]);
    }
#pragma unroll
    for (int r = 0; r < RB; ++r) fnext[r] = iter_flow_at<MODE>(a, fin, C, cx, xc, rowk(RB + r));
    if (MODE == FLOW_COARSE2) {
      coarseN_issue<RB>(a, C, cx, rowk(2 * RB), rawn);
    } else {
#pragma unroll
      for (int r = 0; r < RB; ++r) flow_issue<MODE>(a, fin, C, cx, xc, rowk(2 * RB + r), raw[r]);
    }
    for (int sb = 0; sb < T; sb += 2) {
#pragma unroll
      for (int u = 0; u < 2; ++u) {
        const int s = sb + u;
        if (s < T) {
          if (s < SM) {
#pragma unroll
            for (int bb = 0; bb < NB; ++bb) {
              const int k0 = FR_G * s + bb * RB;
              const int i0 = bb * RB;
#pragma unroll
              for (int r = 0; r < RB; ++r) {
                float m[5];
                um_finish(L[r], h, w, xc, rowk(k0 + r), fcur[r], m);
#pragma unroll
                for (int c = 0; c < 5; ++c) Mb[u][i0 + r][c][t] = m[c];
                fcur[r] = fnext[r];
                um_issue(R0, R1, np, h, w, xc, rowk(k0 + RB + r), fcur[r], L[r]);
              }
              if (MODE == FLOW_COARSE2) {
                int ysb[RB];
#pragma unroll
                for (int r = 0; r < RB; ++r) ysb[r] = rowk(k0 + 2 * RB + r);
                coarse2_finish_batch<RB>(a, cx, ysb[0], ysb, rawn, fnext);
                coarseN_issue<RB>(a, C, cx, rowk(k0 + 3 * RB), rawn);
              } else {
#pragma unroll
                for (int r = 0; r < RB; ++r) fnext[r] = flow_finish<MODE>(a, fin, C, cx, rowk(k0 + 2 * RB + r), raw[MODE == FLOW_COARSE2 ? 0 : r]);
#pragma unroll
                for (int r = 0; r < RB; ++r) flow_issue<MODE>(a, fin, C, cx, xc, rowk(k0 + 3 * RB + r), raw[MODE == FLOW_COARSE2 ? 0 : r]);
              }
            }
          }
          __syncthreads();
        }
      }
    }
  } else if (role == 1) {
    const int t = tid - G::COLS;
    const int vpos = f3_pos(t);
    float ring[F3_RING][5];
    double vs[5];
#pragma unroll
    for (int s2 = 0; s2 < F3_RING; ++s2)
#pragma unroll
      for (int c = 0; c < 5; ++c) ring[s2][c] = 0.f;
#pragma unroll
    for (int c = 0; c < 5; ++c) vs[c] = 0;
    const int nitem = FR_G * nseg * 5;
    constexpr int NR = (FR_G * G::NSEGMAX * 5 + G::COLS - 1) / G::COLS;
    int it_off[NR];
    static_assert(FR_G * 5 * G::PADW < 65536 && FR_G * 2 * G::NSEGMAX * 5 < 32768, "packed item offsets");
#pragma unroll
    for (int j = 0; j < NR; ++j) {
      const int e = t + G::COLS * j;
      const int sg = e % nseg, rc = e / nseg, c = rc % 5, r = rc / 5;
      it_off[j] = e < nitem ? (((r * 5 + c) * G::PADW + 9 + 9 * sg) | (((r * 2 * G::NSEGMAX + 2 * sg) * 5 + c) << 16)) : -1;
    }
    int vgen = 0;
    for (int sb = 0; sb < T; sb += 4) {
#pragma unroll
      for (int u = 0; u < 4; ++u) {
        const int s = sb + u;
        if (s < T) {
          const int c4 = (u + 3) & 3;
          if (s >= 1 && s <= SM) {
            const int cstep = s - 1;
            if (cstep < 4) {
#pragma unroll
              for (int i = 0; i < FR_G; ++i)
#pragma unroll
                for (int c = 0; c < 5; ++c) ring[4 * c4 + i][c] = Mb[c4 & 1][i][c][t];
              if (c4 == 3) {
                if (y0 == 0) {
#pragma unroll
                  for (int c = 0; c < 5; ++c) vs[c] = (double)(ring[M + 1][c] * (float)(M + 2));
#pragma unroll
                  for (int yy = 1; yy < M; ++yy)
#pragma unroll
                    for (int c = 0; c < 5; ++c) vs[c] += (double)ring[M + 1 + yy][c];
#pragma unroll
                  for (int c = 0; c < 5; ++c) {
                    const float d = ring[2 * M + 1][c] - ring[M + 1][c];
                    vs[c] += d;
                  }
                } else {
#pragma unroll
                  for (int c = 0; c < 5; ++c) vs[c] = 0;
#pragma unroll
                  for (int s2 = 1; s2 <= W; ++s2)
#pragma unroll
                    for (int c = 0; c < 5; ++c) vs[c] += (double)ring[s2][c];
                }
              }
            } else {
              if (c4 == 0 && cstep > 4 && ((FR_G * cstep) & 31) == 16) {
#pragma unroll
                for (int c = 0; c < 5; ++c) vs[c] = 0;
#pragma unroll
                for (int s2 = 1; s2 <= W; ++s2) {
#pragma unroll
                  for (int c = 0; c < 5; ++c) vs[c] += (double)ring[s2][c];
                  __builtin_amdgcn_sched_barrier(0);
                }
              }
#pragma unroll
              for (int i = 0; i < FR_G; ++i) {
                const int slot = 4 * c4 + i;
#pragma unroll
                for (int c = 0; c < 5; ++c) {
                  const float m = Mb[c4 & 1][i][c][t];
                  Vs[vgen][i][c][vpos] = (float)vs[c];
                  const float d = m - ring[(slot + 1) & 15][c];
                  vs[c] += d;
                  ring[slot][c] = m;
                }
              }
            }
          }
          if (s >= 6 && s <= SM + 1) {
            const int pg = vgen == 0 ? 2 : vgen - 1;
            const float* __restrict__ vbase = &Vs[pg][0][0][0];
            double* __restrict__ tbase = &Ts[u & 1][0][0][0];
#pragma unroll
            for (int j = 0; j < NR; ++j) {
              if (it_off[j] >= 0) {
                const float* __restrict__ vp = vbase + (it_off[j] & 0xffff);
                double* __restrict__ tp = tbase + (it_off[j] >> 16);
                double acc = vp[-8];
#pragma unroll
                for (int k = -6; k <= 7; ++k) acc += (double)vp[k < 0 ? k - 1 : k];
                tp[0] = acc;
#pragma unroll
                for (int i = 1; i <= 4; ++i) acc += (double)vp[8 + i] - (double)vp[i - 9];
                tp[5] = acc;
              }
            }
          }
          if (s >= 5 && s <= SM) vgen = vgen == 2 ? 0 : vgen + 1;
          __syncthreads();
        }
      }
    }
  } else {
    const int t = tid - 2 * G::COLS;
    const int nq = 2 * nseg;
    const int r = t / nq, q = t - r * nq;
    const int sg = q >> 1, hf = q & 1;
    const bool item = t < FR_G * nq;
    float* fout = a.flow_ptrs ? st_gl(a.flow_ptrs[pr]) : a.flow_out + (size_t)pr * 2 * (size_t)np;
    const int x0 = (int)bx * a.out_w + sg * F3_SW + 4 * hf;
    const bool wide = !(w & 1) && (((uintptr_t)fout) & 15) == 0;
    typedef float f4v __attribute__((ext_vector_type(4)));
    typedef float f2v __attribute__((ext_vector_type(2)));
    int rgen = 0;
    for (int sb = 0; sb < T; sb += 2) {
#pragma unroll
      for (int u = 0; u < 2; ++u) {
        const int s = sb + u;
        if (s < T) {
          const int y = y0 + FR_G * (s - 7) + r;
          if (s >= 7 && item && y < y1 && x0 < w) {
            const float* __restrict__ vrow = &Vs[rgen][r][0][9 + 9 * sg + 4 * hf];
            double tt[5];
#pragma unroll
            for (int c = 0; c < 5; ++c) tt[c] = Ts[(u + 1) & 1][r][q][c];
            float2 res[4];
#pragma unroll
            for (int i = 0; i < 4; ++i) {
              if (i > 0) {
#pragma unroll
                for (int c = 0; c < 5; ++c) {
                  const float* vp = vrow + c * G::PADW;
                  tt[c] += (double)vp[8 + i] - (double)vp[i - 9];
                }
              }
              const double g11 = tt[0] * a.scale, g12 = tt[1] * a.scale, g22 = tt[2] * a.scale;
              const double h1 = tt[3] * a.scale, h2 = tt[4] * a.scale;
              const double idet = d_rcp_pos(g11 * g22 - g12 * g12 + 1e-3);
              res[i] = make_float2((float)((g11 * h2 - g12 * h1) * idet), (float)((g22 * h1 - g12 * h2) * idet));
            }
            float* dst = fout + 2 * ((size_t)y * w + x0);
            if (wide && x0 + 4 <= w) {
#pragma unroll
              for (int i = 0; i < 4; i += 2) {
                f4v v4;
                v4.x = res[i].x; v4.y = res[i].y; v4.z = res[i + 1].x; v4.w = res[i + 1].y;
                __builtin_nontemporal_store(v4, reinterpret_cast<f4v*>(dst + 2 * i));
              }
            } else {
#pragma unroll
              for (int i = 0; i < 4; ++i)
                if (x0 + i < w) {
                  f2v v2;
                  v2.x = res[i].x; v2.y = res[i].y;
                  __builtin_nontemporal_store(v2, reinterpret_cast<f2v*>(dst + 2 * i));
                }
            }
          }
          if (s >= 7) rgen = rgen == 2 ? 0 : rgen + 1;
          __syncthreads();
        }
      }
    }
  }
}

constexpr int FT_T = 32, FT_M = 7, FT_S = FT_T + 2 * FT_M, FT_NT = 512;
static_assert(FT_T == F3_ANCHOR && FT_T % F3_SW == 0 && B2_OUT % F3_SW == 0, "tile anchors must coincide with k_flow_iter3's");

template <int MODE>
__global__ __launch_bounds__(FT_NT) void k_flow_iter_tile(IterArgs a) {
  constexpr int W = 2 * FT_M + 1;
  constexpr int NSEG = FT_T / F3_SW;
  __shared__ float Mt[5][FT_S][FT_S];
  __shared__ double Tt[FT_T][2 * NSEG][5];
  const int tid = threadIdx.x;
  const int h = a.h, w = a.w;
  const int np = h * w;
  const int pr = blockIdx.z;
  const int X0 = blockIdx.x * FT_T, Y0 = blockIdx.y * FT_T;
  const float* __restrict__ R0;
  const float* __restrict__ R1;
  if (a.pairs) {
    R0 = a.R + (size_t)a.pairs[2 * pr] * 5 * (size_t)np;
    R1 = a.R + (size_t)a.pairs[2 * pr + 1] * 5 * (size_t)np;
  } else {
    R0 = a.R;
    R1 = a.R1_direct;
  }
  const float* __restrict__ fin = a.flow_in ? a.flow_in + (size_t)pr * 2 * (size_t)np : nullptr;
  const float* __restrict__ C = a.coarse ? a.coarse + (size_t)pr * 2 * (size_t)a.ch * a.cw : nullptr;
  float* fout = a.flow_ptrs ? st_gl(a.flow_ptrs[pr]) : a.flow_out + (size_t)pr * 2 * (size_t)np;

  constexpr int NI = (FT_S * FT_S + FT_NT - 1) / FT_NT;
  int px[NI], py[NI];
  FlowRaw raw[NI];
  CoarseX cxs[NI];
#pragma unroll
  for (int k = 0; k < NI; ++k) {
    const int i = min(tid + FT_NT * k, FT_S * FT_S - 1);
    const int ty = i / FT_S, tx = i - ty * FT_S;
    px[k] = d_clamp(X0 - FT_M + tx, 0, w - 1);
    py[k] = d_clamp(Y0 - FT_M + ty, 0, h - 1);
    cxs[k] = (MODE == FLOW_COARSE) ? coarse_x(a, px[k]) : CoarseX{0, 1.f, 0.f, false};
    flow_issue<MODE>(a, fin, C, cxs[k], px[k], py[k], raw[k]);
  }
  float2 fl[NI];
#pragma unroll
  for (int k = 0; k < NI; ++k) fl[k] = flow_finish<MODE>(a, fin, C, cxs[k], py[k], raw[k]);
#pragma unroll
  for (int k0 = 0; k0 < NI; k0 += 3) {
    constexpr int CH = 3;
    UmLoads L[CH];
#pragma unroll
    for (int j = 0; j < CH; ++j)
      if (k0 + j < NI) um_issue(R0, R1, np, h, w, px[k0 + j], py[k0 + j], fl[k0 + j], L[j]);
#pragma unroll
    for (int j = 0; j < CH; ++j) {
      if (k0 + j < NI) {
        float m[5];
        um_finish(L[j], h, w, px[k0 + j], py[k0 + j], fl[k0 + j], m);
        const int i = tid + FT_NT * (k0 + j);
        if (i < FT_S * FT_S) {
          const int ty = i / FT_S, tx = i - ty * FT_S;
#pragma unroll
          for (int c = 0; c < 5; ++c) Mt[c][ty][tx] = m[c];
        }
      }
    }
    __builtin_amdgcn_sched_barrier(0);
  }
  __syncthreads();
  for (int i = tid; i < 5 * FT_S; i += FT_NT) {
    const int c = i / FT_S, col = i - c * FT_S;
    float mv[FT_S];
#pragma unroll
    for (int j = 0; j < FT_S; ++j) mv[j] = Mt[c][j][col];
    double vs;
    if (Y0 == 0) {
      vs = (double)(mv[FT_M] * (float)(FT_M + 2));
#pragma unroll
      for (int yy = 1; yy < FT_M; ++yy) vs += (double)mv[FT_M + yy];
      const float d = mv[2 * FT_M] - mv[FT_M];
      vs += d;
    } else {
      vs = 0;
#pragma unroll
      for (int s2 = 0; s2 < W; ++s2) vs += (double)mv[s2];
    }
#pragma unroll
    for (int j = 0; j < FT_T; ++j) {
      Mt[c][j][col] = (float)vs;
      if (j + 1 < FT_T) {
        const float d = mv[j + W] - mv[j];
        vs += d;
      }
    }
  }
  __syncthreads();
  for (int i = tid; i < FT_T * NSEG * 5; i += FT_NT) {
    const int g = i % NSEG, rc = i / NSEG, c = rc % 5, r = rc / 5;
    const float* __restrict__ vp = &Mt[c][r][F3_SW * g];
    double acc = vp[0];
#pragma unroll
    for (int k = 1; k < W; ++k) acc += (double)vp[k];
    Tt[r][2 * g][c] = acc;
#pragma unroll
    for (int k = 1; k <= 4; ++k) acc += (double)vp[k + 2 * FT_M] - (double)vp[k - 1];
    Tt[r][2 * g + 1][c] = acc;
  }
  __syncthreads();
  for (int i = tid; i < FT_T * 2 * NSEG; i += FT_NT) {
    const int r = i / (2 * NSEG), q = i - r * (2 * NSEG);
    const int y = Y0 + r;
    if (y >= h) continue;
    const int j0 = FT_M + 4 * q;
    double t[5];
#pragma unroll
    for (int c = 0; c < 5; ++c) t[c] = Tt[r][q][c];
#pragma unroll
    for (int k = 0; k < 4; ++k) {
      if (k > 0) {
#pragma unroll
        for (int c = 0; c < 5; ++c) t[c] += (double)Mt[c][r][j0 + k + FT_M] - (double)Mt[c][r][j0 + k - FT_M - 1];
      }
      const double g11 = t[0] * a.scale, g12 = t[1] * a.scale, g22 = t[2] * a.scale;
      const double h1 = t[3] * a.scale, h2 = t[4] * a.scale;
      const double idet = d_rcp_pos(g11 * g22 - g12 * g12 + 1e-3);
      const int x = X0 + 4 * q + k;
      if (x < w)
        *reinterpret_cast<float2*>(fout + 2 * ((size_t)y * w + x)) =
            make_float2((float)((g11 * h2 - g12 * h1) * idet), (float)((g22 * h1 - g12 * h2) * idet));
    }
  }
}

struct PyrPlan {
  int kind;
  int mode, max_rows, max_cols;
  size_t lds;
};
constexpr size_t kPyrLdsMax = 64 * 1024;

PyrPlan pyr_plan(int h, int w, const LevelGeom& g) {
  PyrPlan q;
  memset(&q, 0, sizeof(q));
  if (g.lh == h && g.lw == w && g.ksize == 3 && h >= 2 && w >= 8) return q;
  if (w == 2 * g.lw && h == 2 * g.lh && g.ksize == 3) q.kind = 2;
  else if (w == 4 * g.lw && h == 4 * g.lh && g.ksize == 9) q.kind = 4;
  else if (w == 8 * g.lw && h == 8 * g.lh && g.ksize == 19) q.kind = 8;
  if (q.kind) return q;
  q.kind = 1;
  if (g.lh == h && g.lw == w) q.mode = PYR_COPY;
  else if (w == 2 * g.lw && h == 2 * g.lh) q.mode = PYR_AREA2;
  else q.mode = PYR_LINEAR;
  const double scale_x = 1. / ((double)g.lw / w), scale_y = 1. / ((double)g.lh / h);
  const int r = g.ksize / 2;
  q.max_rows = (int)std::ceil((PYR_OH - 1) * scale_y) + 3 + 2 * r + 1;
  q.max_cols = ((int)std::ceil((PYR_OW - 1) * scale_x) + 3 + 2 * r + 1 + 3) / 4 * 4;
  q.lds = sizeof(float) * (size_t)q.max_rows * 2 * PYR_OW + (size_t)q.max_rows * q.max_cols;
  return q;
}

int check_pyr_level(st_ctx* ctx, int h, int w, const LevelGeom& g, int k) {
  if (g.ksize > kMaxTaps - 1)
    return st_set_error(ctx, ST_ERR_UNSUPPORTED, "farneback: pyramid level %d: kernel size %d too large (at most %d)", k, g.ksize, kMaxTaps - 1);
  if (g.lh < 1 || g.lw < 1) return ST_OK;
  const PyrPlan q = pyr_plan(h, w, g);
  if (q.lds > kPyrLdsMax)
    return st_set_error(ctx, ST_ERR_UNSUPPORTED, "farneback: pyramid level %d (kernel size %d) needs a tile of %zu B of LDS (at most %zu)", k,
                        g.ksize, q.lds, kPyrLdsMax);
  return ST_OK;
}

int check_params(st_ctx* ctx, const st_fb_params& p, int h, int w) {
  if (h <= 0 || w <= 0) return st_set_error(ctx, ST_ERR_INVALID, "farneback: bad frame size %dx%d", w, h);
  if (p.flags != 0) return st_set_error(ctx, ST_ERR_UNSUPPORTED, "farneback: flags=%d (only 0 implemented)", p.flags);
  if (p.fast_pyramids) return st_set_error(ctx, ST_ERR_UNSUPPORTED, "farneback: fastPyramids not implemented");
  if (!(p.pyr_scale > 0 && p.pyr_scale < 1)) return st_set_error(ctx, ST_ERR_INVALID, "farneback: pyr_scale must be in (0,1)");
  if (p.poly_n != 5 && p.poly_n != 7) return st_set_error(ctx, ST_ERR_UNSUPPORTED, "farneback: poly_n=%d (5 or 7)", p.poly_n);
  if (p.win_size < 3 || p.win_size > 63 || !(p.win_size & 1))
    return st_set_error(ctx, ST_ERR_UNSUPPORTED, "farneback: win_size=%d (odd, 3...63)", p.win_size);
  if (p.num_iters < 1 || p.num_levels < 0) return st_set_error(ctx, ST_ERR_INVALID, "farneback: bad iteration/level count");
  if (p.gray_bits != 14 && p.gray_bits != 15) return st_set_error(ctx, ST_ERR_INVALID, "farneback: gray_bits must be 14 or 15");
  if ((long long)h * w > 200000000LL) return st_set_error(ctx, ST_ERR_UNSUPPORTED, "farneback: frames above 200 Mpx are not supported (32-bit plane offsets)");
  int levels = fb_levels(h, w, p);
  for (int k = 0; k <= levels; ++k) {
    LevelGeom g = fb_level_geom(h, w, p, k);
    ST_TRY(check_pyr_level(ctx, h, w, g, k));
    if (g.lh < 1 || g.lw < 1) return st_set_error(ctx, ST_ERR_INVALID, "farneback: empty pyramid level");
  }
  return ST_OK;
}

int rows_per_segment(st_ctx* ctx, int h, int strips, int batch, int halo) {
  long long target = (long long)ctx->num_cus * 8;
  long long per = (long long)strips * batch;
  long long segs = (target + per - 1) / per;
  if (segs < 1) segs = 1;
  int rows = (int)((h + segs - 1) / segs);
  int min_rows = 4 * halo;
  if (rows < min_rows) rows = min_rows;
  if (rows > h) rows = h;
  return rows;
}

constexpr double kPolyexpSegCostU8 = 1.5, kPolyexpSegCostF32 = 0.0, kPolyexpTail = 0.85;

double polyexp_plan_cost(int h, long long per, int num_cus, int rows, double c) {
  const long long nseg = (h + rows - 1) / rows;
  return (double)per * (h + nseg * c) / num_cus + kPolyexpTail * ((rows < h ? rows : h) + c);
}

int polyexp_rows(st_ctx* ctx, int h, int strips, int n, bool gray_source) {
  const int min_rows = 12;
  const long long target = (long long)ctx->num_cus * 8, per = (long long)strips * n;
  long long segs = (target + per - 1) / per;
  if (segs < 1) segs = 1;
  int rows = (int)((h + segs - 1) / segs);
  rows = (rows + PE_RB - 1) / PE_RB * PE_RB;
  if (rows < min_rows) rows = min_rows;
  if (rows > h) rows = h;
  const double c = gray_source ? kPolyexpSegCostU8 : kPolyexpSegCostF32;
  double best = polyexp_plan_cost(h, per, ctx->num_cus, rows, c);
  for (int r = (rows - 1) / PE_RB * PE_RB; r >= min_rows && (h + r - 1) / r <= 65535; r -= PE_RB) {
    const double cost = polyexp_plan_cost(h, per, ctx->num_cus, r, c);
    if (cost < best) { best = cost; rows = r; }
  }
  return rows;
}

int launch_gray(st_ctx* ctx, const uint8_t* const* frames_table_dev, int n, int h, int w, int bits, uint8_t* gray,
                bool frames_aligned4, const TablesArg* tables = nullptr) {
  GrayArgs a;
  a.frames = frames_table_dev;
  a.gray = gray;
  a.npix = h * w;
  if (bits == 14) { a.cb = 1868; a.cg = 9617; a.cr = 4899; } else { a.cb = 3735; a.cg = 19235; a.cr = 9798; }
  a.shift = bits;
  a.rnd = 1 << (bits - 1);
  const bool vec = frames_aligned4 && a.npix % 4 == 0 && ((uintptr_t)gray & 3) == 0;
  int bx = ((vec ? a.npix / 4 : a.npix) + 255) / 256;
  if (bx > 2048) bx = 2048;
  if (bx < 1) bx = 1;
  st_timed t(ctx, ST_K_GRAY);
  if (tables && vec) hipLaunchKernelGGL(k_gray_tab<true>, dim3(bx, n), dim3(256), 0, ctx->stream, a, *tables);
  else if (tables) hipLaunchKernelGGL(k_gray_tab<false>, dim3(bx, n), dim3(256), 0, ctx->stream, a, *tables);
  else if (vec) hipLaunchKernelGGL(k_gray4, dim3(bx, n), dim3(256), 0, ctx->stream, a);
  else hipLaunchKernelGGL(k_gray, dim3(bx, n), dim3(256), 0, ctx->stream, a);
  ST_HIP(ctx, hipGetLastError());
  return ST_OK;
}

int launch_pyr(st_ctx* ctx, const uint8_t* gray, int n, int h, int w, const LevelGeom& g, float* img) {
  PyrArgs a;
  memset(&a, 0, sizeof(a));
  a.gray = gray; a.img = img;
  a.sh = h; a.sw = w; a.dh = g.lh; a.dw = g.lw; a.ks = g.ksize;
  gaussian_kernel(g.ksize, g.sigma, a.taps);
  const double inv_sx = (double)g.lw / w, inv_sy = (double)g.lh / h;
  a.scale_x = 1. / inv_sx; a.scale_y = 1. / inv_sy;
  const PyrPlan q = pyr_plan(h, w, g);
  if (q.kind == 0) {
    Pyr0Args z;
    z.gray = gray; z.img = img; z.h = h; z.w = w; z.k0 = a.taps[1]; z.k1 = a.taps[2];
    const int bx = ((w + 3) / 4 + 255) / 256;
    long long segs = ((long long)ctx->num_cus * 8 + (long long)bx * n - 1) / ((long long)bx * n);
    int rows = (int)((h + segs - 1) / segs);
    if (rows < 32) rows = h < 32 ? h : 32;
    z.rows_per_seg = rows;
    st_timed t(ctx, ST_K_PYR);
    hipLaunchKernelGGL(k_pyr0, dim3(bx, (h + rows - 1) / rows, n), dim3(256), 0, ctx->stream, z);
    ST_HIP(ctx, hipGetLastError());
    return ST_OK;
  }
  if (q.kind != 1) {
    const int S = q.kind;
    PyrDecArgs z;
    z.gray = gray; z.img = img; z.sh = h; z.sw = w; z.dh = g.lh; z.dw = g.lw;
    memcpy(z.taps, a.taps, sizeof(z.taps));
    const int bx = (g.lw + 255) / 256;
    long long segs = ((long long)ctx->num_cus * 8 + (long long)bx * n - 1) / ((long long)bx * n);
    int rows = (int)((g.lh + segs - 1) / segs);
    const int min_rows = S == 8 ? 4 : 8;
    if (rows < min_rows) rows = g.lh < min_rows ? g.lh : min_rows;
    z.rows_per_seg = rows;
    dim3 grid(bx, (g.lh + rows - 1) / rows, n);
    st_timed t(ctx, ST_K_PYR);
    if (S == 2) hipLaunchKernelGGL((k_pyr_dec<2, 3>), grid, dim3(256), 0, ctx->stream, z);
    else if (S == 4) hipLaunchKernelGGL((k_pyr_dec<4, 9>), grid, dim3(256), 0, ctx->stream, z);
    else hipLaunchKernelGGL((k_pyr_dec<8, 19>), grid, dim3(256), 0, ctx->stream, z);
    ST_HIP(ctx, hipGetLastError());
    return ST_OK;
  }
  a.mode = q.mode; a.max_rows = q.max_rows; a.max_cols = q.max_cols;
  const size_t lds = q.lds;
  if (lds > kPyrLdsMax) return st_set_error(ctx, ST_ERR_UNSUPPORTED, "farneback: pyramid tile needs %zu B of LDS", lds);
  dim3 grid((g.lw + PYR_OW - 1) / PYR_OW, (g.lh + PYR_OH - 1) / PYR_OH, n);
  st_timed t(ctx, ST_K_PYR);
  hipLaunchKernelGGL(k_pyr, grid, dim3(256), lds, ctx->stream, a);
  ST_HIP(ctx, hipGetLastError());
  return ST_OK;
}

bool pyr_fused_ok(int h, int w, const st_fb_params& p) {
  if (fb_levels(h, w, p) != 3 || (h & 7) || (w & 7)) return false;
  static const int ks[4] = {3, 3, 9, 19};
  for (int k = 0; k <= 3; ++k) {
    const LevelGeom g = fb_level_geom(h, w, p, k);
    if (g.lh != (h >> k) || g.lw != (w >> k) || g.ksize != ks[k]) return false;
  }
  return true;
}

int launch_pyr_fused(st_ctx* ctx, const uint8_t* gray, const uint8_t* const* frames, int n, int h, int w,
                     const st_fb_params& p, float* const imgs[4], bool skip0 = false, bool gray_out = false) {
  PyrFusedArgs a;
  memset(&a, 0, sizeof(a));
  a.gray = gray; a.frames = frames;
  if (gray_out) a.gray_out = const_cast<uint8_t*>(gray);
  if (p.gray_bits == 14) { a.cb = 1868; a.cg = 9617; a.cr = 4899; } else { a.cb = 3735; a.cg = 19235; a.cr = 9798; }
  a.shift = p.gray_bits; a.rnd = 1 << (p.gray_bits - 1);
  a.img0 = imgs[0]; a.img1 = imgs[1]; a.img2 = imgs[2]; a.img3 = imgs[3];
  a.h = h; a.w = w;
  float* taps[4] = {a.k0, a.k1, a.k2, a.k3};
  for (int k = 0; k <= 3; ++k) {
    const LevelGeom g = fb_level_geom(h, w, p, k);
    float full[kMaxTaps];
    gaussian_kernel(g.ksize, g.sigma, full);
    for (int i = 0; i <= g.ksize / 2; ++i) {
      if (full[i] != full[g.ksize - 1 - i]) return st_set_error(ctx, ST_ERR_UNSUPPORTED, "pyr: asymmetric Gaussian taps");
      taps[k][i] = full[i];
    }
  }
  const int strips = (w + 1023) / 1024;
  a.strip_w = ((w + strips - 1) / strips + 7) / 8 * 8;
  const bool roles_on = gray && ctx->pyr_roles != 0;
  long long segs = ((long long)ctx->num_cus * (roles_on ? 14 : 8) + (long long)strips * n - 1) / ((long long)strips * n);
  int rows = (int)((h + segs - 1) / segs);
  rows = (rows + 7) / 8 * 8;
  const int min_rows = (long long)strips * n * ((h + 63) / 64) >= 2LL * ctx->num_cus ? 64 : 16;
  if (rows < min_rows) rows = h < min_rows ? h : min_rows;
  a.rows_per_seg = rows;
  st_timed t(ctx, ST_K_PYR);
  const int roles_env = ctx->pyr_roles;
  const bool roles = gray && roles_env != 0;
  if (skip0 && !roles) return st_set_error(ctx, ST_ERR_INVALID, "pyr: level 0 can only be left out of the role-split kernel");
  if (gray_out && !(skip0 && frames)) return st_set_error(ctx, ST_ERR_INVALID, "pyr: the RGB-source role-split kernel leaves level 0 out");
  if (gray_out) hipLaunchKernelGGL((k_pyr_roles<false, true>), dim3(strips, (h + rows - 1) / rows, n), dim3(768), 0, ctx->stream, a);
  else if (roles && skip0) hipLaunchKernelGGL(k_pyr_roles<false>, dim3(strips, (h + rows - 1) / rows, n), dim3(768), 0, ctx->stream, a);
  else if (roles) hipLaunchKernelGGL(k_pyr_roles<true>, dim3(strips, (h + rows - 1) / rows, n), dim3(768), 0, ctx->stream, a);
  else if (gray) hipLaunchKernelGGL(k_pyr_fused<false>, dim3(strips, (h + rows - 1) / rows, n), dim3(256), 0, ctx->stream, a);
  else hipLaunchKernelGGL(k_pyr_fused<true>, dim3(strips, (h + rows - 1) / rows, n), dim3(256), 0, ctx->stream, a);
  ST_HIP(ctx, hipGetLastError());
  return ST_OK;
}

static bool polyexp_frame_fits(int h, int w) { return (unsigned long long)h * (unsigned long long)w <= (1ull << 26); }

int launch_polyexp(st_ctx* ctx, const float* img, int n, int h, int w, int poly_n, double poly_sigma, float* R,
                   const uint8_t* gray = nullptr) {
  if (!polyexp_frame_fits(h, w)) return st_set_error(ctx, ST_ERR_UNSUPPORTED, "polyexp: frames above 64 M pixels are not supported");
  PolyArgs a;
  a.img = img; a.gray = gray; a.R = R; a.h = h; a.w = w;
  poly_prepare(poly_n, poly_sigma, &a.c);
  const int strips = (w + PE_OUT - 1) / PE_OUT;
  a.rows_per_seg = polyexp_rows(ctx, h, strips, n, gray != nullptr);
  dim3 grid(strips, (h + a.rows_per_seg - 1) / a.rows_per_seg, n);
  st_timed t(ctx, ST_K_POLYEXP);
  if (gray && w < 8) return st_set_error(ctx, ST_ERR_INVALID, "polyexp: the gray-source instance needs rows of at least 8 pixels");
  if (gray && poly_n == 5) hipLaunchKernelGGL(k_polyexp_u8<5>, grid, dim3(256), 0, ctx->stream, a);
  else if (gray) hipLaunchKernelGGL(k_polyexp_u8<7>, grid, dim3(256), 0, ctx->stream, a);
  else if (poly_n == 5) hipLaunchKernelGGL(k_polyexp<5>, grid, dim3(256), 0, ctx->stream, a);
  else hipLaunchKernelGGL(k_polyexp<7>, grid, dim3(256), 0, ctx->stream, a);
  ST_HIP(ctx, hipGetLastError());
  return ST_OK;
}

int launch_polyexp_ml(st_ctx* ctx, float* const* imgs, const LevelGeom* geom, float* const* R, const int* ks, int nk, int n,
                      int poly_n, double poly_sigma) {
  if (nk < 1 || nk > 4) return st_set_error(ctx, ST_ERR_INVALID, "polyexp: bad level list");
  PolyArgsML a;
  memset(&a, 0, sizeof(a));
  poly_prepare(poly_n, poly_sigma, &a.c);
  a.nlv = nk;
  int blocks = 0;
  for (int i = 0; i < nk; ++i) {
    const LevelGeom& g = geom[ks[i]];
    PolyLevel& l = a.lv[i];
    if (!polyexp_frame_fits(g.lh, g.lw)) return st_set_error(ctx, ST_ERR_UNSUPPORTED, "polyexp: frames above 64 M pixels are not supported");
    l.img = imgs[ks[i]]; l.R = R[ks[i]]; l.h = g.lh; l.w = g.lw;
    l.strips = (g.lw + PE_OUT - 1) / PE_OUT;
    l.rows_per_seg = polyexp_rows(ctx, g.lh, l.strips, n, false);
    l.block0 = blocks;
    blocks += l.strips * ((g.lh + l.rows_per_seg - 1) / l.rows_per_seg);
  }
  st_timed t(ctx, ST_K_POLYEXP);
  if (poly_n == 5) hipLaunchKernelGGL(k_polyexp_ml<5>, dim3(blocks, n), dim3(256), 0, ctx->stream, a);
  else hipLaunchKernelGGL(k_polyexp_ml<7>, dim3(blocks, n), dim3(256), 0, ctx->stream, a);
  ST_HIP(ctx, hipGetLastError());
  return ST_OK;
}

int launch_update_matrices(st_ctx* ctx, UMArgs a, int n_pairs) {
  const size_t np = (size_t)a.h * a.w;
  int bx = (int)((np + 255) / 256);
  if (bx > 4096) bx = 4096;
  st_timed t(ctx, ST_K_UPDATE_MATRICES);
  hipLaunchKernelGGL(k_update_matrices, dim3(bx, n_pairs), dim3(256), 0, ctx->stream, a);
  ST_HIP(ctx, hipGetLastError());
  return ST_OK;
}

int launch_blur(st_ctx* ctx, BlurArgs a, int n_pairs) {
  if (a.m == 7) {
    const int strips = (a.w + B2_OUT - 1) / B2_OUT;
    long long segs = ((long long)ctx->num_cus * 4 + (long long)strips - 1) / ((long long)strips);
    int rows = (int)((a.h + segs - 1) / segs);
    rows = (rows + 14) / 15 * 15;
    if (rows < 15) rows = 15;
    if (rows > 135 && a.h > 135) rows = 135;
    a.rows_per_seg = rows;
    dim3 grid(strips, (a.h + rows - 1) / rows, n_pairs);
    st_timed t(ctx, ST_K_BLUR_UPDATE);
    hipLaunchKernelGGL((k_blur_update_v2<7>), grid, dim3(B2_T), 0, ctx->stream, a);
    ST_HIP(ctx, hipGetLastError());
    return ST_OK;
  }
  const int strips = (a.w + (BLUR_T - 2 * a.m) - 1) / (BLUR_T - 2 * a.m);
  a.rows_per_seg = rows_per_segment(ctx, a.h, strips, 1, 2 * a.m + 1);
  dim3 grid(strips, (a.h + a.rows_per_seg - 1) / a.rows_per_seg, n_pairs);
  st_timed t(ctx, ST_K_BLUR_UPDATE);
  hipLaunchKernelGGL(k_blur_update, grid, dim3(BLUR_T), 0, ctx->stream, a);
  ST_HIP(ctx, hipGetLastError());
  return ST_OK;
}

int launch_flow_iter(st_ctx* ctx, IterArgs a, int n_pairs) {
  hipEvent_t e0, e1;
  constexpr long long kTilePx = 600000;
  const bool tile = ctx->tile_mode == 1 || (ctx->tile_mode != 0 && (long long)n_pairs * a.h * a.w <= kTilePx);
  if (tile && (a.h + FT_T - 1) / FT_T <= 65535) {
    dim3 grid((a.w + FT_T - 1) / FT_T, (a.h + FT_T - 1) / FT_T, n_pairs);
    ST_TRY(st_time_dispatch(ctx, ST_K_BLUR_UPDATE, &e0, &e1));
    if (a.coarse) hipExtLaunchKernelGGL((k_flow_iter_tile<FLOW_COARSE>), grid, dim3(FT_NT), 0, ctx->stream, e0, e1, 0, a);
    else if (a.flow_in) hipExtLaunchKernelGGL((k_flow_iter_tile<FLOW_FIELD>), grid, dim3(FT_NT), 0, ctx->stream, e0, e1, 0, a);
    else hipExtLaunchKernelGGL((k_flow_iter_tile<FLOW_ZERO>), grid, dim3(FT_NT), 0, ctx->stream, e0, e1, 0, a);
    ST_HIP(ctx, hipGetLastError());
    return ST_OK;
  }
  const int strips = (a.w + B2_OUT - 1) / B2_OUT;
  const long long resident = (long long)ctx->num_cus * 2;
  const int periods = (a.h + F3_ANCHOR - 1) / F3_ANCHOR;
  int rows = periods * F3_ANCHOR;
  long long rounds3 = 1, wgs3 = 1;
  double best = 1e300;
  for (int segs = 1; segs <= periods; ++segs) {
    const int r = (periods + segs - 1) / segs * F3_ANCHOR;
    const long long nseg = (a.h + r - 1) / r;
    const long long wgs = (long long)strips * n_pairs * nseg;
    const long long rounds = (wgs + resident - 1) / resident;
    const double cost = (double)rounds * (r + 15);
    if (cost < best * 0.999) { best = cost; rows = r; rounds3 = rounds; wgs3 = wgs; }
  }
  const int roles_env = ctx->roles_mode == -1 && ctx->flow_concurrent ? 0 : ctx->roles_mode;
  const int roles_ncw = ctx->roles_ncw;
  const long long roles_limit = a.coarse ? resident * 62 / 100 : resident * 95 / 100;
  if (roles_env == 1 || (roles_env != 0 && rounds3 == 1 && wgs3 < roles_limit)) {
    int best_ncw = 0, best_out = 0, best_rows = 0;
    double bestr = 1e300;
    for (int ncw = 5; ncw >= 4; --ncw) {
      if (roles_ncw && ncw != roles_ncw) continue;
      const int outmax = 64 * ncw - 2 * B2_HALO;
      const int rstrips = (a.w + outmax - 1) / outmax;
      const int out_w = ((a.w + rstrips - 1) / rstrips + 7) / 8 * 8;
      for (int segs = 1; segs <= periods; ++segs) {
        const int r = (periods + segs - 1) / segs * F3_ANCHOR;
        const long long nseg = (a.h + r - 1) / r;
        const long long wgs = (long long)rstrips * n_pairs * nseg;
        const long long rounds = (wgs + ctx->num_cus - 1) / ctx->num_cus;
        const double cost = (double)rounds * (r + 16 + 3 * FR_G) * (ncw == 5 ? 1.3 : 1.0);
        if (cost < bestr * 0.999) { bestr = cost; best_ncw = ncw; best_out = out_w; best_rows = r; }
      }
    }
    if (best_ncw) {
      a.rows_per_seg = best_rows;
      a.out_w = best_out;
      const int rstrips = (a.w + best_out - 1) / best_out;
      dim3 grid(rstrips, (a.h + best_rows - 1) / best_rows, n_pairs);
      ST_TRY(st_time_dispatch(ctx, ST_K_BLUR_UPDATE, &e0, &e1));
      const int mode = a.coarse ? (a.h == 2 * a.ch ? FLOW_COARSE2 : FLOW_COARSE) : (a.flow_in ? FLOW_FIELD : FLOW_ZERO);
      if (best_ncw == 5) {
        const dim3 blk(FrGeom<5>::THREADS);
        if (mode == FLOW_COARSE2) hipExtLaunchKernelGGL((k_flow_iter_roles<5, FLOW_COARSE2>), grid, blk, 0, ctx->stream, e0, e1, 0, a);
        else if (mode == FLOW_COARSE) hipExtLaunchKernelGGL((k_flow_iter_roles<5, FLOW_COARSE>), grid, blk, 0, ctx->stream, e0, e1, 0, a);
        else if (mode == FLOW_FIELD) hipExtLaunchKernelGGL((k_flow_iter_roles<5, FLOW_FIELD>), grid, blk, 0, ctx->stream, e0, e1, 0, a);
        else hipExtLaunchKernelGGL((k_flow_iter_roles<5, FLOW_ZERO>), grid, blk, 0, ctx->stream, e0, e1, 0, a);
      } else {
        const dim3 blk(FrGeom<4>::THREADS);
        if (mode == FLOW_COARSE2) hipExtLaunchKernelGGL((k_flow_iter_roles<4, FLOW_COARSE2>), grid, blk, 0, ctx->stream, e0, e1, 0, a);
        else if (mode == FLOW_COARSE) hipExtLaunchKernelGGL((k_flow_iter_roles<4, FLOW_COARSE>), grid, blk, 0, ctx->stream, e0, e1, 0, a);
        else if (mode == FLOW_FIELD) hipExtLaunchKernelGGL((k_flow_iter_roles<4, FLOW_FIELD>), grid, blk, 0, ctx->stream, e0, e1, 0, a);
        else hipExtLaunchKernelGGL((k_flow_iter_roles<4, FLOW_ZERO>), grid, blk, 0, ctx->stream, e0, e1, 0, a);
      }
      ST_HIP(ctx, hipGetLastError());
      return ST_OK;
    }
  }
  int nseg3 = (a.h + rows - 1) / rows;
  for (int segs = 1; segs <= periods; ++segs) {
    const int r = periods / segs * F3_ANCHOR;
    if (r < F3_ANCHOR) break;
    const int last = a.h - (segs - 1) * r;
    const long long wgs = (long long)strips * n_pairs * segs;
    const long long rounds = (wgs + resident - 1) / resident;
    const double cost = (double)rounds * ((r > last ? r : last) + 15);
    if (cost < best * 0.999) { best = cost; rows = r; nseg3 = segs; }
  }
  a.rows_per_seg = rows;
  dim3 grid(strips, nseg3, n_pairs);
  ST_TRY(st_time_dispatch(ctx, ST_K_BLUR_UPDATE, &e0, &e1));
  const int mode = a.coarse ? (a.h == 2 * a.ch ? FLOW_COARSE2 : FLOW_COARSE) : (a.flow_in ? FLOW_FIELD : FLOW_ZERO);
  if (mode == FLOW_COARSE2) hipExtLaunchKernelGGL((k_flow_iter3<FLOW_COARSE2>), grid, dim3(B2_T), 0, ctx->stream, e0, e1, 0, a);
  else if (mode == FLOW_COARSE) hipExtLaunchKernelGGL((k_flow_iter3<FLOW_COARSE>), grid, dim3(B2_T), 0, ctx->stream, e0, e1, 0, a);
  else if (mode == FLOW_FIELD) hipExtLaunchKernelGGL((k_flow_iter3<FLOW_FIELD>), grid, dim3(B2_T), 0, ctx->stream, e0, e1, 0, a);
  else hipExtLaunchKernelGGL((k_flow_iter3<FLOW_ZERO>), grid, dim3(B2_T), 0, ctx->stream, e0, e1, 0, a);
  ST_HIP(ctx, hipGetLastError());
  return ST_OK;
}

bool fused_path(int h, int w, const st_fb_params& p) {
  if (p.win_size != 15) return false;
  const int levels = fb_levels(h, w, p);
  for (int k = 0; k <= levels; ++k) {
    LevelGeom g = fb_level_geom(h, w, p, k);
    if (g.lh < 2 || g.lw < 2) return false;
  }
  return true;
}

size_t pass_bytes(int h, int w, const st_fb_params& p, int nf, int npairs) {
  const int levels = fb_levels(h, w, p);
  size_t np0 = (size_t)h * w;
  size_t maxCoarse = 0;
  for (int k = 0; k <= levels; ++k) {
    LevelGeom g = fb_level_geom(h, w, p, k);
    size_t npk = (size_t)g.lh * g.lw;
    if (k >= 1 && npk > maxCoarse) maxCoarse = npk;
  }
  size_t b = 0;
  b += st_align_up(np0 * nf);
  b += st_align_up(sizeof(float) * np0 * nf);
  if (pyr_fused_ok(h, w, p))
    for (int k = 1; k <= 3; ++k) b += st_align_up(sizeof(float) * (np0 >> (2 * k)) * nf);
  for (int k = 0; k <= levels; ++k) {
    LevelGeom g = fb_level_geom(h, w, p, k);
    b += st_align_up(sizeof(float) * 5 * (size_t)g.lh * g.lw * nf);
  }
  b += 2 * st_align_up(sizeof(float) * (fused_path(h, w, p) ? 2 : 5) * np0 * npairs);
  b += 2 * st_align_up(sizeof(float) * 2 * (maxCoarse ? maxCoarse : 1) * npairs);
  b += st_align_up(sizeof(void*) * nf) + st_align_up(sizeof(int) * 2 * npairs) + st_align_up(sizeof(void*) * npairs);
  return b + 4096;
}

int farneback_pass(st_ctx* ctx, const uint8_t* const* frames, int nf, const int32_t* pairs, int npairs, int h, int w,
                   const st_fb_params& p, float* const* outs) {
  const int levels = fb_levels(h, w, p);
  const size_t np0 = (size_t)h * w;
  ST_TRY(st_ws_reserve(ctx, pass_bytes(h, w, p, nf, npairs)));
  uint8_t* gray = (uint8_t*)st_ws_alloc(ctx, np0 * nf);
  float* img = (float*)st_ws_alloc(ctx, sizeof(float) * np0 * nf);
  const bool pyr1 = pyr_fused_ok(h, w, p);
  float* imgs[4] = {img, nullptr, nullptr, nullptr};
  if (pyr1)
    for (int k = 1; k <= 3; ++k) {
      imgs[k] = (float*)st_ws_alloc(ctx, sizeof(float) * (np0 >> (2 * k)) * nf);
      if (!imgs[k]) return st_set_error(ctx, ST_ERR_OOM, "farneback: scratch plan exhausted");
    }
  std::vector<float*> R(levels + 1);
  std::vector<LevelGeom> geom(levels + 1);
  size_t maxCoarse = 1;
  for (int k = 0; k <= levels; ++k) {
    geom[k] = fb_level_geom(h, w, p, k);
    size_t npk = (size_t)geom[k].lh * geom[k].lw;
    if (k >= 1 && npk > maxCoarse) maxCoarse = npk;
    R[k] = (float*)st_ws_alloc(ctx, sizeof(float) * 5 * npk * nf);
  }
  float* M[2];
  const bool fused = fused_path(h, w, p);
  M[0] = (float*)st_ws_alloc(ctx, sizeof(float) * (fused ? 2 : 5) * np0 * npairs);
  M[1] = (float*)st_ws_alloc(ctx, sizeof(float) * (fused ? 2 : 5) * np0 * npairs);
  float* cflow[2];
  cflow[0] = (float*)st_ws_alloc(ctx, sizeof(float) * 2 * maxCoarse * npairs);
  cflow[1] = (float*)st_ws_alloc(ctx, sizeof(float) * 2 * maxCoarse * npairs);
  const uint8_t** d_frames = (const uint8_t**)st_ws_alloc(ctx, sizeof(void*) * nf);
  int* d_pairs = (int*)st_ws_alloc(ctx, sizeof(int) * 2 * npairs);
  float** d_outs = (float**)st_ws_alloc(ctx, sizeof(void*) * npairs);
  if (!gray || !img || !M[0] || !M[1] || !cflow[0] || !cflow[1] || !d_frames || !d_pairs || !d_outs || !R[levels])
    return st_set_error(ctx, ST_ERR_OOM, "farneback: scratch plan exhausted");
  TablesArg ta;
  const bool small_tables = nf <= kTabMax && npairs <= kTabMax;
  if (small_tables) {
    memset(&ta, 0, sizeof(ta));
    ta.d_frames = d_frames; ta.d_outs = d_outs; ta.d_pairs = d_pairs; ta.nf = nf; ta.npairs = npairs;
    for (int i = 0; i < nf; ++i) ta.frames[i] = frames[i];
    for (int i = 0; i < npairs; ++i) { ta.outs[i] = outs[i]; ta.pairs[2 * i] = pairs[2 * i]; ta.pairs[2 * i + 1] = pairs[2 * i + 1]; }
    static_assert(kTabMax <= 64, "one thread per table entry");
  } else {
    ST_HIP(ctx, hipMemcpyAsync(d_frames, frames, sizeof(void*) * nf, hipMemcpyHostToDevice, ctx->stream));
    ST_HIP(ctx, hipMemcpyAsync(d_pairs, pairs, sizeof(int) * 2 * npairs, hipMemcpyHostToDevice, ctx->stream));
    ST_HIP(ctx, hipMemcpyAsync(d_outs, outs, sizeof(void*) * npairs, hipMemcpyHostToDevice, ctx->stream));
  }

  bool aligned4 = true;
  for (int i = 0; i < nf; ++i) aligned4 = aligned4 && ((uintptr_t)frames[i] & 3) == 0;
  const bool pyr_rgb = pyr1 && aligned4 && ctx->fold_gray;
  const bool single = pyr1 && levels >= 1 && levels <= 3 && npairs <= 16;
  const bool poly_u8 = pyr1 && !pyr_rgb && !single && ctx->poly_u8 && ctx->pyr_roles != 0 && geom[0].ksize == 3 && geom[0].sigma <= 0 &&
                       geom[0].lh == h && geom[0].lw == w && w >= 8;
  const bool roles_rgb = poly_u8 && aligned4 && ctx->pyr_roles_rgb;
  if (!pyr_rgb && !roles_rgb) {
    ST_TRY(launch_gray(ctx, d_frames, nf, h, w, p.gray_bits, gray, aligned4, small_tables ? &ta : nullptr));
  } else if (small_tables) {
    hipLaunchKernelGGL(k_set_tables, dim3(1), dim3(64), 0, ctx->stream, ta);
    ST_HIP(ctx, hipGetLastError());
  }
  if (pyr1) ST_TRY(launch_pyr_fused(ctx, pyr_rgb ? nullptr : gray, d_frames, nf, h, w, p, imgs, poly_u8, roles_rgb));
  if (single) {
    int ks[4], nk = 0;
    for (int k = 0; k <= levels; ++k) ks[nk++] = k;
    ST_TRY(launch_polyexp_ml(ctx, imgs, geom.data(), R.data(), ks, nk, nf, p.poly_n, p.poly_sigma));
  } else {
    for (int k = levels; k >= 0; --k) {
      if (!pyr1) ST_TRY(launch_pyr(ctx, gray, nf, h, w, geom[k], img));
      ST_TRY(launch_polyexp(ctx, pyr1 ? imgs[k] : img, nf, geom[k].lh, geom[k].lw, p.poly_n, p.poly_sigma, R[k],
                            k == 0 && poly_u8 ? gray : nullptr));
    }
  }
  if (fused) {
    float* fbuf[2] = {M[0], M[1]};
    int cur = 0;
    for (int k = levels; k >= 0; --k) {
      const int lh = geom[k].lh, lw = geom[k].lw;
      for (int it = 0; it < p.num_iters; ++it) {
        const bool last = it == p.num_iters - 1;
        IterArgs q;
        memset(&q, 0, sizeof(q));
        q.R = R[k]; q.pairs = d_pairs; q.h = lh; q.w = lw;
        q.scale = 1. / ((double)p.win_size * p.win_size);
        if (it == 0) {
          if (k < levels) {
            q.coarse = cflow[cur];
            q.ch = geom[k + 1].lh; q.cw = geom[k + 1].lw;
            q.scale_x = 1. / ((double)lw / q.cw);
            q.scale_y = 1. / ((double)lh / q.ch);
            q.mul = (float)(1. / p.pyr_scale);
          }
        } else {
          q.flow_in = fbuf[(it - 1) & 1];
        }
        if (last) {
          if (k == 0) q.flow_ptrs = d_outs; else q.flow_out = cflow[cur ^ 1];
        } else {
          q.flow_out = fbuf[it & 1];
        }
        ST_TRY(launch_flow_iter(ctx, q, npairs));
      }
      cur ^= 1;
    }
    return ST_OK;
  }
  int cur = 0;
  for (int k = levels; k >= 0; --k) {
    const int lh = geom[k].lh, lw = geom[k].lw;
    UMArgs u;
    memset(&u, 0, sizeof(u));
    u.R = R[k]; u.pairs = d_pairs; u.M = M[0]; u.h = lh; u.w = lw;
    if (k < levels) {
      u.ch = geom[k + 1].lh; u.cw = geom[k + 1].lw;
      u.coarse = cflow[cur];
      u.scale_x = 1. / ((double)lw / u.cw);
      u.scale_y = 1. / ((double)lh / u.ch);
      u.mul = (float)(1. / p.pyr_scale);
    }
    ST_TRY(launch_update_matrices(ctx, u, npairs));
    int mi = 0;
    for (int it = 0; it < p.num_iters; ++it) {
      const bool last = it == p.num_iters - 1;
      BlurArgs bl;
      memset(&bl, 0, sizeof(bl));
      bl.R = R[k]; bl.pairs = d_pairs; bl.Min = M[mi]; bl.Mout = M[mi ^ 1];
      bl.h = lh; bl.w = lw; bl.m = p.win_size / 2;
      bl.update = !last; bl.write_flow = last;
      bl.scale = 1. / ((double)p.win_size * p.win_size);
      if (last) {
        if (k == 0) bl.flow_ptrs = d_outs; else bl.flow = cflow[cur ^ 1];
      }
      ST_TRY(launch_blur(ctx, bl, npairs));
      mi ^= 1;
    }
    cur ^= 1;
  }
  return ST_OK;
}

}

ST_EXPORT void st_fb_params_default(st_fb_params* p) {
  if (!p) return;
  p->num_levels = 3; p->pyr_scale = 0.5; p->fast_pyramids = 0; p->win_size = 15; p->num_iters = 3;
  p->poly_n = 5; p->poly_sigma = 1.2; p->flags = 0; p->gray_bits = 15;
}

ST_EXPORT int st_fb_levels(int h, int w, const st_fb_params* params) {
  if (!params || h <= 0 || w <= 0) return -1;
  return fb_levels(h, w, *params);
}

ST_EXPORT int st_fb_level_geom(int h, int w, const st_fb_params* params, int level, int* lh, int* lw, double* sigma,
                               int* ksize) {
  if (!params || h <= 0 || w <= 0 || level < 0) return ST_ERR_INVALID;
  LevelGeom g = fb_level_geom(h, w, *params, level);
  if (lh) *lh = g.lh;
  if (lw) *lw = g.lw;
  if (sigma) *sigma = g.sigma;
  if (ksize) *ksize = g.ksize;
  return ST_OK;
}

ST_EXPORT int st_farneback_pairs(st_ctx* ctx, const uint8_t* const* frames_dev, int n_frames, const int32_t* pairs,
                                 int n_pairs, int h, int w, const st_fb_params* params, float* const* flow_out_dev) {
  ST_TRY(st_enter(ctx));
  st_fb_params p;
  if (params) p = *params; else st_fb_params_default(&p);
  if (n_pairs < 0 || n_frames < 0) return st_set_error(ctx, ST_ERR_INVALID, "farneback: negative count");
  ST_TRY(check_params(ctx, p, h, w));
  if (n_pairs == 0) return ST_OK;
  if (!frames_dev || !pairs || !flow_out_dev) return st_set_error(ctx, ST_ERR_INVALID, "farneback: null table");
  ctx->flow_concurrent = st_flow_call_begins(ctx) && n_pairs <= 4;
  for (int i = 0; i < n_pairs; ++i) {
    if (pairs[2 * i] < 0 || pairs[2 * i] >= n_frames || pairs[2 * i + 1] < 0 || pairs[2 * i + 1] >= n_frames)
      return st_set_error(ctx, ST_ERR_INVALID, "farneback: pair %d indexes outside [0,%d)", i, n_frames);
    if (!flow_out_dev[i]) return st_set_error(ctx, ST_ERR_INVALID, "farneback: output %d is null", i);
  }
  int start = 0;
  std::vector<int> slot(n_frames);
  while (start < n_pairs) {
    int count = n_pairs - start;
    std::vector<const uint8_t*> pf;
    std::vector<int32_t> pp;
    for (;;) {
      std::fill(slot.begin(), slot.end(), -1);
      pf.clear(); pp.clear();
      for (int i = start; i < start + count; ++i)
        for (int e = 0; e < 2; ++e) {
          int f = pairs[2 * i + e];
          if (slot[f] < 0) {
            if (!frames_dev[f]) return st_set_error(ctx, ST_ERR_INVALID, "farneback: frame %d is null", f);
            slot[f] = (int)pf.size();
            pf.push_back(frames_dev[f]);
          }
          pp.push_back(slot[f]);
        }
      if (pass_bytes(h, w, p, (int)pf.size(), count) <= ctx->ws_limit || count == 1) break;
      count = (count + 1) / 2;
    }
    ST_TRY(farneback_pass(ctx, pf.data(), (int)pf.size(), pp.data(), count, h, w, p, flow_out_dev + start));
    start += count;
  }
  return ST_OK;
}

ST_EXPORT int st_gray_u8(st_ctx* ctx, const uint8_t* rgb_dev, int h, int w, int gray_bits, uint8_t* gray_dev) {
  ST_TRY(st_enter(ctx));
  if (!rgb_dev || !gray_dev || h <= 0 || w <= 0 || (gray_bits != 14 && gray_bits != 15))
    return st_set_error(ctx, ST_ERR_INVALID, "gray: bad arguments");
  ST_TRY(st_ws_reserve(ctx, 4096));
  const uint8_t** t = (const uint8_t**)st_ws_alloc(ctx, sizeof(void*));
  ST_HIP(ctx, hipMemcpyAsync(t, &rgb_dev, sizeof(void*), hipMemcpyHostToDevice, ctx->stream));
  return launch_gray(ctx, t, 1, h, w, gray_bits, gray_dev, ((uintptr_t)rgb_dev & 3) == 0);
}

ST_EXPORT int st_fb_pyr_image(st_ctx* ctx, const uint8_t* gray_dev, int h, int w, const st_fb_params* params, int level,
                              float* img_dev) {
  ST_TRY(st_enter(ctx));
  st_fb_params p;
  if (params) p = *params; else st_fb_params_default(&p);
  if (!gray_dev || !img_dev || level < 0) return st_set_error(ctx, ST_ERR_INVALID, "pyr: bad arguments");
  ST_TRY(check_params(ctx, p, h, w));
  LevelGeom g = fb_level_geom(h, w, p, level);
  ST_TRY(check_pyr_level(ctx, h, w, g, level));
  if (g.lh < 1 || g.lw < 1) return st_set_error(ctx, ST_ERR_UNSUPPORTED, "pyr: level %d is empty", level);
  if (pyr_fused_ok(h, w, p) && level <= 3) {
    const size_t np0 = (size_t)h * w;
    size_t bytes = 0;
    for (int k = 0; k <= 3; ++k) bytes += st_align_up(sizeof(float) * (np0 >> (2 * k)));
    ST_TRY(st_ws_reserve(ctx, bytes));
    float* imgs[4];
    for (int k = 0; k <= 3; ++k) {
      imgs[k] = k == level ? img_dev : (float*)st_ws_alloc(ctx, sizeof(float) * (np0 >> (2 * k)));
      if (!imgs[k]) return st_set_error(ctx, ST_ERR_OOM, "pyr: scratch exhausted");
    }
    return launch_pyr_fused(ctx, gray_dev, nullptr, 1, h, w, p, imgs);
  }
  return launch_pyr(ctx, gray_dev, 1, h, w, g, img_dev);
}

ST_EXPORT int st_fb_polyexp(st_ctx* ctx, const float* img_dev, int h, int w, int poly_n, double poly_sigma, float* r_dev) {
  ST_TRY(st_enter(ctx));
  if (!img_dev || !r_dev || h <= 0 || w <= 0) return st_set_error(ctx, ST_ERR_INVALID, "polyexp: bad arguments");
  if (poly_n != 5 && poly_n != 7) return st_set_error(ctx, ST_ERR_UNSUPPORTED, "polyexp: poly_n=%d (5 or 7)", poly_n);
  return launch_polyexp(ctx, img_dev, 1, h, w, poly_n, poly_sigma, r_dev);
}

ST_EXPORT int st_fb_update_matrices(st_ctx* ctx, const float* r0_dev, const float* r1_dev, const float* flow_dev,
                                    const float* coarse_flow_dev, int ch, int cw, double pyr_scale, int h, int w,
                                    float* m_dev) {
  ST_TRY(st_enter(ctx));
  if (!r0_dev || !r1_dev || !m_dev || h <= 0 || w <= 0) return st_set_error(ctx, ST_ERR_INVALID, "update_matrices: bad arguments");
  UMArgs u;
  memset(&u, 0, sizeof(u));
  u.R = r0_dev; u.R1_direct = r1_dev; u.M = m_dev; u.h = h; u.w = w;
  if (coarse_flow_dev) {
    if (ch <= 0 || cw <= 0 || !(pyr_scale > 0)) return st_set_error(ctx, ST_ERR_INVALID, "update_matrices: bad coarse geometry");
    u.coarse = coarse_flow_dev; u.ch = ch; u.cw = cw;
    u.scale_x = 1. / ((double)w / cw);
    u.scale_y = 1. / ((double)h / ch);
    u.mul = (float)(1. / pyr_scale);
  } else {
    u.flow = flow_dev;
  }
  return launch_update_matrices(ctx, u, 1);
}

ST_EXPORT int st_fb_flow_iteration(st_ctx* ctx, const float* r0_dev, const float* r1_dev, const float* flow_in_dev,
                                    const float* coarse_flow_dev, int ch, int cw, double pyr_scale, int h, int w,
                                    int block_size, float* flow_out_dev) {
  ST_TRY(st_enter(ctx));
  if (!r0_dev || !r1_dev || !flow_out_dev || h <= 0 || w <= 0)
    return st_set_error(ctx, ST_ERR_INVALID, "flow_iteration: bad arguments");
  if (block_size != 15) return st_set_error(ctx, ST_ERR_UNSUPPORTED, "flow_iteration: block_size=%d (15 only)", block_size);
  if (h < 2 || w < 2) return st_set_error(ctx, ST_ERR_UNSUPPORTED, "flow_iteration: needs at least 2x2 pixels");
  if (flow_out_dev == flow_in_dev) return st_set_error(ctx, ST_ERR_INVALID, "flow_iteration: in-place not allowed");
  IterArgs q;
  memset(&q, 0, sizeof(q));
  q.R = r0_dev; q.R1_direct = r1_dev; q.h = h; q.w = w; q.flow_out = flow_out_dev;
  q.scale = 1. / ((double)block_size * block_size);
  if (coarse_flow_dev) {
    if (ch <= 0 || cw <= 0 || !(pyr_scale > 0)) return st_set_error(ctx, ST_ERR_INVALID, "flow_iteration: bad coarse geometry");
    q.coarse = coarse_flow_dev; q.ch = ch; q.cw = cw;
    q.scale_x = 1. / ((double)w / cw);
    q.scale_y = 1. / ((double)h / ch);
    q.mul = (float)(1. / pyr_scale);
  } else {
    q.flow_in = flow_in_dev;
  }
  return launch_flow_iter(ctx, q, 1);
}

ST_EXPORT int st_fb_update_flow_blur(st_ctx* ctx, const float* r0_dev, const float* r1_dev, const float* m_in_dev, int h,
                                     int w, int block_size, int update, float* flow_out_dev, float* m_out_dev) {
  ST_TRY(st_enter(ctx));
  if (!m_in_dev || !flow_out_dev || h <= 0 || w <= 0) return st_set_error(ctx, ST_ERR_INVALID, "update_flow_blur: bad arguments");
  if (block_size < 3 || block_size > 63 || !(block_size & 1))
    return st_set_error(ctx, ST_ERR_UNSUPPORTED, "update_flow_blur: block_size=%d (odd, 3...63)", block_size);
  if (update && (!r0_dev || !r1_dev || !m_out_dev || m_out_dev == m_in_dev))
    return st_set_error(ctx, ST_ERR_INVALID, "update_flow_blur: update needs R0, R1 and a distinct m_out");
  BlurArgs b;
  memset(&b, 0, sizeof(b));
  b.R = r0_dev; b.R1_direct = r1_dev; b.Min = m_in_dev; b.Mout = m_out_dev; b.flow = flow_out_dev;
  b.h = h; b.w = w; b.m = block_size / 2; b.update = update ? 1 : 0; b.write_flow = 1;
  b.scale = 1. / ((double)block_size * block_size);
  return launch_blur(ctx, b, 1);
}
```

scannertools_amd/csrc/st_internal.h:

```cpp
#ifndef ST_INTERNAL_H_
#define ST_INTERNAL_H_

#include <hip/hip_runtime.h>

#include <atomic>
#include <cstdarg>
#include <cstdio>
#include <string>
#include <vector>

#include "scannertools_hip.h"

#define ST_EXPORT extern "C" __attribute__((visibility("default")))

struct st_timing_slot {
  std::vector<hipEvent_t> starts, stops;
  size_t used = 0;
  int launches = 0;
  double total_ms = 0.0;
};

struct st_ctx {
  int device = 0;
  hipStream_t own_stream = nullptr;
  hipStream_t stream = nullptr;
  int tile_mode = -1;
  bool poly_u8 = true;
  bool fold_gray = false;
  int roles_mode = -1, roles_ncw = 0, pyr_roles = -1;
  bool pyr_roles_rgb = true;
  int conv_tile = -1;
  std::atomic<bool> flow_busy{false};
  std::atomic<long long> flow_enter_ns{0};
  bool flow_concurrent = false;
  int concurrency_mode = -1;
  void* ws = nullptr;
  size_t ws_bytes = 0;
  size_t ws_limit = (size_t)64 << 30;
  size_t ws_off = 0;
  unsigned timing_mask = 0;
  st_timing_slot timing[ST_K_COUNT];
  std::string last_error;
  int num_cus = 256;
  struct st_jpeg_state* jpeg = nullptr;
  struct st_netin_state* netin = nullptr;
  struct st_detect_state* detect = nullptr;
  struct st_jpeg_enc_state* jpeg_enc = nullptr;
};
void st_jpeg_release(st_ctx* ctx);
struct StJpegEntArgs;
int st_jpeg_entropy_launch(st_ctx* ctx, const StJpegEntArgs& a, unsigned max_groups);
struct StJsqArgs;
int st_jsq_round_launch(st_ctx* ctx, const StJsqArgs& a, unsigned max_groups, bool first, int par, unsigned* changed);
int st_jsq_finish_launch(st_ctx* ctx, const StJsqArgs& a, unsigned max_groups, unsigned max_segments, int par, size_t coef_bytes);
void st_jpeg_enc_release(st_ctx* ctx);
void st_netin_release(st_ctx* ctx);
void st_detect_release(st_ctx* ctx);

int st_set_error(st_ctx* ctx, int status, const char* fmt, ...);

#define ST_HIP(ctx, expr)                                                                   \
  do {                                                                                      \
    hipError_t _e = (expr);                                                                 \
    if (_e != hipSuccess)                                                                   \
      return st_set_error((ctx), ST_ERR_HIP, "%s failed: %s (%s:%d)", #expr,                \
                          hipGetErrorString(_e), __FILE__, __LINE__);                       \
  } while (0)

#define ST_TRY(expr)              \
  do {                            \
    int _s = (expr);              \
    if (_s != ST_OK) return _s;   \
  } while (0)

int st_enter(st_ctx* ctx);

bool st_flow_call_begins(st_ctx* ctx);

int st_ws_reserve(st_ctx* ctx, size_t total_bytes);
void st_ws_reset(st_ctx* ctx);
void* st_ws_alloc(st_ctx* ctx, size_t bytes);
inline size_t st_align_up(size_t v, size_t a = 256) { return (v + a - 1) / a * a; }

int st_time_begin(st_ctx* ctx, int id);
int st_time_end(st_ctx* ctx, int id);
int st_time_dispatch(st_ctx* ctx, int id, hipEvent_t* start, hipEvent_t* stop);

struct st_timed {
  st_ctx* ctx;
  int id;
  bool open;
  st_timed(st_ctx* c, int k) : ctx(c), id(k), open(st_time_begin(c, k) == ST_OK) {}
  ~st_timed() { if (open) (void)st_time_end(ctx, id); }
};

#ifdef __HIPCC__
template <class T>
__device__ __forceinline__ T* st_gl(T* p) {
  return (T*)((__attribute__((address_space(1))) T*)(uintptr_t)p);
}
#endif

enum { RS_NEAREST = 0, RS_LINEAR = 1, RS_AREA2 = 2, RS_COPY = 3, RS_CUBIC = 4, RS_AREA_INT = 5, RS_AREA = 6, RS_LINEAR_AREA = 7, RS_LANCZOS4 = 8 };

struct st_rs_scales {
  double scale_x, scale_y, inv_scale_x, inv_scale_y;
  int iscale_x, iscale_y;
  bool area_fast;
};
st_rs_scales st_rs_plan_scales(int h, int w, int out_h, int out_w);
inline int st_rs_linear_mode(int h, int w, int out_h, int out_w, const st_rs_scales& s) {
  if (h == out_h && w == out_w) return RS_COPY;
  if (s.area_fast && s.iscale_x == 2 && s.iscale_y == 2) return RS_AREA2;
  return RS_LINEAR;
}

#ifdef __HIPCC__
__host__ __device__ __forceinline__ int rs_coef(float v) {
  const float r = rintf(v);
  return r < -32768.f ? -32768 : (r > 32767.f ? 32767 : (int)r);
}

__host__ __device__ __forceinline__ float rs_linear_coord(int d, double scale, int* s) {
  const float f = (float)((d + 0.5) * scale - 0.5);
  *s = (int)floorf(f);
  return f - *s;
}

struct RsTapX { int sx, a0, a1; bool two; };
__host__ __device__ __forceinline__ RsTapX rs_linear_tap_x(int sx, float fx, int sw) {
  RsTapX t;
  if (sx < 0) { fx = 0; sx = 0; }
  if (sx >= sw - 1) { fx = 0; sx = sw - 1; }
  t.a0 = rs_coef((1.f - fx) * 2048); t.a1 = rs_coef(fx * 2048);
  t.two = sx + 1 < sw;
  t.sx = sx;
  return t;
}
struct RsTapY { int y0, y1, b0, b1; };
__host__ __device__ __forceinline__ RsTapY rs_linear_tap_y(int sy, float fy, int sh) {
  RsTapY t;
  t.b0 = rs_coef((1.f - fy) * 2048); t.b1 = rs_coef(fy * 2048);
  t.y0 = sy < 0 ? 0 : (sy > sh - 1 ? sh - 1 : sy);
  t.y1 = sy + 1 < 0 ? 0 : (sy + 1 > sh - 1 ? sh - 1 : sy + 1);
  return t;
}
__device__ __forceinline__ int rs_linear_h(int v0, int v1, int a0, int a1, bool two) { return two ? v0 * a0 + v1 * a1 : v0 * 2048; }
__device__ __forceinline__ int rs_linear_v(int r0, int r1, int b0, int b1) { return (((b0 * (r0 >> 4)) >> 16) + ((b1 * (r1 >> 4)) >> 16) + 2) >> 2; }

__device__ __forceinline__ void rs_linear_px_c3(const uint8_t* __restrict__ R0, const uint8_t* __restrict__ R1, int sxo, int a0, int a1, bool two,
                                                bool wide, int b0, int b1, int p, unsigned* out) {
  typedef unsigned u32u __attribute__((aligned(1)));
  int t0[6], t1[6];
  if (wide) {
    const unsigned l0 = *reinterpret_cast<const u32u*>(R0 + sxo), h0 = *reinterpret_cast<const u32u*>(R0 + sxo + 4);
    const unsigned l1 = *reinterpret_cast<const u32u*>(R1 + sxo), h1 = *reinterpret_cast<const u32u*>(R1 + sxo + 4);
#pragma unroll
    for (int k = 0; k < 4; ++k) { t0[k] = (l0 >> (8 * k)) & 0xff; t1[k] = (l1 >> (8 * k)) & 0xff; }
    t0[4] = h0 & 0xff; t0[5] = (h0 >> 8) & 0xff; t1[4] = h1 & 0xff; t1[5] = (h1 >> 8) & 0xff;
  } else {
#pragma unroll
    for (int k = 0; k < 3; ++k) { t0[k] = R0[sxo + k]; t1[k] = R1[sxo + k]; }
#pragma unroll
    for (int k = 3; k < 6; ++k) { t0[k] = two ? R0[sxo + k] : 0; t1[k] = two ? R1[sxo + k] : 0; }
  }
#pragma unroll
  for (int c = 0; c < 3; ++c) {
    const int r0 = rs_linear_h(t0[c], t0[3 + c], a0, a1, two);
    const int r1 = rs_linear_h(t1[c], t1[3 + c], a0, a1, two);
    const unsigned v = (unsigned)rs_linear_v(r0, r1, b0, b1) & 0xffu;
    out[(3 * p + c) >> 2] |= v << (8 * ((3 * p + c) & 3));
  }
}

__device__ __forceinline__ void rs_area2_4px_c3(const uint8_t* __restrict__ S0, const uint8_t* __restrict__ S1, unsigned* out) {
  typedef unsigned u32u __attribute__((aligned(1)));
  unsigned w0[6], w1[6];
#pragma unroll
  for (int k = 0; k < 6; ++k) { w0[k] = reinterpret_cast<const u32u*>(S0)[k]; w1[k] = reinterpret_cast<const u32u*>(S1)[k]; }
  out[0] = out[1] = out[2] = 0u;
#pragma unroll
  for (int p = 0; p < 4; ++p)
#pragma unroll
    for (int c = 0; c < 3; ++c) {
      const int i0 = 6 * p + c, i1 = 6 * p + 3 + c;
      const unsigned v = (((w0[i0 >> 2] >> (8 * (i0 & 3))) & 0xffu) + ((w0[i1 >> 2] >> (8 * (i1 & 3))) & 0xffu) +
                          ((w1[i0 >> 2] >> (8 * (i0 & 3))) & 0xffu) + ((w1[i1 >> 2] >> (8 * (i1 & 3))) & 0xffu) + 2u) >> 2;
      out[(3 * p + c) >> 2] |= v << (8 * ((3 * p + c) & 3));
    }
}
#endif

#endif
```

Measured before the change: 10420.

## Store the fifth polynomial coefficient as row-pair interleaved plane for paired gathers

Changes the polynomial-expansion output layout so the scalar fifth coefficient plane holds each pixel's value alongside the value of the row above, six floats per pixel instead of five. The flow-update kernels then fetch the 2x2 bilinear neighbourhood of that coefficient with one 16-byte load instead of two 8-byte loads, and share one paired load between the two rows processed together. This is meant to cut gather load instructions and memory transactions in the iteration kernels. The cost is extra polyexp writes and workspace, plus boundary-row handling in the writer. It is on by default and can be disabled with an environment variable.

```diff
diff --git a/scannertools_amd/csrc/st_context.hip b/scannertools_amd/csrc/st_context.hip
--- a/scannertools_amd/csrc/st_context.hip
+++ b/scannertools_amd/csrc/st_context.hip
@@ -105,6 +105,7 @@
   if (const char* e = getenv("ST_ITER_TILE")) c->tile_mode = atoi(e);
   c->fold_gray = getenv("ST_PYR_FOLD_GRAY") != nullptr;
   if (const char* e = getenv("ST_POLY_U8")) c->poly_u8 = atoi(e) != 0;
+  if (const char* e = getenv("ST_R_PAIRS")) c->r_pairs = atoi(e) != 0;
   if (const char* e = getenv("ST_ITER_ROLES")) c->roles_mode = atoi(e);
   if (const char* e = getenv("ST_ROLES_NCW")) c->roles_ncw = atoi(e);
   if (const char* e = getenv("ST_PYR_ROLES")) c->pyr_roles = atoi(e);
diff --git a/scannertools_amd/csrc/st_farneback.hip b/scannertools_amd/csrc/st_farneback.hip
--- a/scannertools_amd/csrc/st_farneback.hip
+++ b/scannertools_amd/csrc/st_farneback.hip
@@ -970,6 +970,13 @@
   __builtin_amdgcn_raw_buffer_store_b32(__builtin_bit_cast(unsigned, v), r, (int)voff, (int)soff, AUX);
 }
 template <int AUX = 0>
+__device__ __forceinline__ void bst2(__amdgpu_buffer_rsrc_t r, unsigned voff, unsigned soff, float v0, float v1) {
+  typedef unsigned u2 __attribute__((ext_vector_type(2)));
+  u2 q;
+  q.x = __builtin_bit_cast(unsigned, v0); q.y = __builtin_bit_cast(unsigned, v1);
+  __builtin_amdgcn_raw_buffer_store_b64(q, r, (int)voff, (int)soff, AUX);
+}
+template <int AUX = 0>
 __device__ __forceinline__ void bst4(__amdgpu_buffer_rsrc_t r, unsigned voff, float4 v) {
   typedef unsigned u4 __attribute__((ext_vector_type(4)));
   u4 q;
@@ -1001,7 +1008,7 @@
 constexpr int PE_RB = 4;
 constexpr int PE_OUT = 240;
 
-template <int N, class A, bool U8 = false>
+template <int N, class A, bool U8 = false, bool PR = false>
 __device__ __forceinline__ void polyexp_body(const A& a, const float* __restrict__ img, float* __restrict__ Rbase, int h, int w,
                                              int rows_per_seg, int bx, int by, int z, const uint8_t* __restrict__ gray = nullptr) {
   constexpr int PXW = 3 * PE_RB + 1;
@@ -1009,7 +1016,7 @@
   const int tid = threadIdx.x;
   const int np = h * w;
   const float* __restrict__ I = img + (size_t)z * (size_t)np;
-  float* __restrict__ R = Rbase + (size_t)z * 5 * (size_t)np;
+  float* __restrict__ R = Rbase + (size_t)z * (PR ? 6 : 5) * (size_t)np;
   const int x = bx * PE_OUT - N + tid;
   const int xc = d_clamp(x, 0, w - 1);
   const int y0 = by * rows_per_seg;
@@ -1017,9 +1024,9 @@
   const bool writer = tid >= N && tid < N + PE_OUT && x < w;
   const unsigned voff = 4u * (unsigned)xc;
   const unsigned xo = writer ? (unsigned)x : 0u;
-  const unsigned xo16 = writer ? 16u * xo : 0x80000000u, xo4 = writer ? 4u * xo : 0x80000000u;
+  const unsigned xo16 = writer ? 16u * xo : 0x80000000u, xo4 = writer ? (PR ? 8u : 4u) * xo : 0x80000000u;
   const __amdgpu_buffer_rsrc_t Rnull = st_rsrc(R, 0);
-  const __amdgpu_buffer_rsrc_t Ib = st_rsrc(I, 4 * (size_t)np), Rb = st_rsrc(R, 20 * (size_t)np);
+  const __amdgpu_buffer_rsrc_t Ib = st_rsrc(I, 4 * (size_t)np), Rb = st_rsrc(R, (PR ? 24 : 20) * (size_t)np);
   auto opaque = [](unsigned v) { asm volatile("" : "+v"(v)); return v; };
   auto src = [&](int row) { return bld1(Ib, voff, 4u * (unsigned)w * (unsigned)d_clamp(row, 0, h - 1)); };
   const __amdgpu_buffer_rsrc_t Gb = st_rsrc(U8 ? gray + (size_t)z * (size_t)np : nullptr, U8 ? (size_t)np : 0);
@@ -1051,6 +1058,7 @@
     }
   }
 
+  float above = 0.f;
   int buf = 0;
   for (int y = y0; y < y1; y += PE_RB) {
 #pragma unroll
@@ -1121,21 +1129,34 @@
         const unsigned rowo = (unsigned)(y + r) * (unsigned)w;
         bst4(row_ok ? Rb : Rnull, xo16 + 16u * rowo, make_float4((float)(b3 * a.c.ig11), (float)(b2 * a.c.ig11),
                                                                                   (float)(b1 * a.c.ig03 + b5 * a.c.ig33), (float)(b1 * a.c.ig03 + b4 * a.c.ig33)));
-        bst1(row_ok ? Rb : Rnull, xo4, 16u * (unsigned)np + 4u * rowo, (float)(b6 * a.c.ig55));
+        const float c4 = (float)(b6 * a.c.ig55);
+        if (!PR) {
+          bst1(row_ok ? Rb : Rnull, xo4, 16u * (unsigned)np + 4u * rowo, c4);
+        } else {
+          const unsigned prow = 16u * (unsigned)np + 8u * (rowo - (unsigned)w);
+          if (r == 0 && y == y0) bst1(row_ok && y0 > 0 ? Rb : Rnull, xo4, prow + 4u, c4);
+          else bst2(row_ok ? Rb : Rnull, xo4, prow, above, c4);
+          above = row_ok ? c4 : above;
+        }
       }
     }
     buf ^= 1;
   }
-}
-
-template <int N>
+  if (PR) {
+    const unsigned prow = 16u * (unsigned)np + 8u * (unsigned)(y1 - 1) * (unsigned)w;
+    if (y1 == h) bst2(Rb, xo4, prow, above, above);
+    else bst1(Rb, xo4, prow, above);
+  }
+}
+
+template <int N, bool PR>
 __global__ __launch_bounds__(256) void k_polyexp(PolyArgs a) {
-  polyexp_body<N>(a, a.img, a.R, a.h, a.w, a.rows_per_seg, (int)blockIdx.x, (int)blockIdx.y, (int)blockIdx.z);
-}
-
-template <int N>
+  polyexp_body<N, PolyArgs, false, PR>(a, a.img, a.R, a.h, a.w, a.rows_per_seg, (int)blockIdx.x, (int)blockIdx.y, (int)blockIdx.z);
+}
+
+template <int N, bool PR>
 __global__ __launch_bounds__(256, 1) void k_polyexp_u8(PolyArgs a) {
-  polyexp_body<N, PolyArgs, true>(a, nullptr, a.R, a.h, a.w, a.rows_per_seg, (int)blockIdx.x, (int)blockIdx.y, (int)blockIdx.z, a.gray);
+  polyexp_body<N, PolyArgs, true, PR>(a, nullptr, a.R, a.h, a.w, a.rows_per_seg, (int)blockIdx.x, (int)blockIdx.y, (int)blockIdx.z, a.gray);
 }
 
 struct PolyLevel {
@@ -1148,7 +1169,7 @@
   int nlv;
   PolyCoef c;
 };
-template <int N>
+template <int N, bool PR>
 __global__ __launch_bounds__(256) void k_polyexp_ml(PolyArgsML a) {
   int l = 0;
 #pragma unroll
@@ -1160,7 +1181,7 @@
   for (int i = 1; i < 4; ++i)
     if (l == i) { img = a.lv[i].img; R = a.lv[i].R; h = a.lv[i].h; w = a.lv[i].w; rows = a.lv[i].rows_per_seg; strips = a.lv[i].strips; b0 = a.lv[i].block0; }
   const int local = (int)blockIdx.x - b0;
-  polyexp_body<N>(a, img, R, h, w, rows, local % strips, local / strips, (int)blockIdx.y);
+  polyexp_body<N, PolyArgsML, false, PR>(a, img, R, h, w, rows, local % strips, local / strips, (int)blockIdx.y);
 }
 
 __device__ __forceinline__ void update_matrices_px(const float* __restrict__ R0, const float* __restrict__ R1,
@@ -1212,14 +1233,21 @@
 }
 
 
+
+typedef float f4pr __attribute__((ext_vector_type(4), aligned(8)));
 struct UmLoads {
   float4 q;
   float qs;
+  f2u qp;
   float4 t0, t1, b0, b1;
   f2u ts, bs;
+  f4pr p4;
 };
-
+enum { UM_QS_ROW = 0, UM_QS_PAIR = 1, UM_QS_NONE = 2 };
+
+template <bool PR>
 __device__ __forceinline__ void um_gather(const float* __restrict__ R1, unsigned single, unsigned gi, unsigned gb, UmLoads& L);
+template <bool PR, int QS = UM_QS_ROW>
 __device__ __forceinline__ void um_issue(const float* __restrict__ R0, const float* __restrict__ R1, int np, int h,
                                          int w, int x, int y, float2 f, UmLoads& L) {
   float fx = x + f.x, fy = y + f.y;
@@ -1230,19 +1258,35 @@
   const unsigned o = (unsigned)(y * w + x);
   const unsigned single = 16u * (unsigned)np;
   L.q = ldf4(R0, 16u * o);
-  L.qs = ldf(R0, single + 4u * o);
-  um_gather(R1, single, gi, gb, L);
-}
-
+  if (!PR) L.qs = ldf(R0, single + 4u * o);
+  else if (QS == UM_QS_ROW) L.qs = ldf(R0, single + 8u * o);
+  else if (QS == UM_QS_PAIR) L.qp = ldf2(R0, single + 8u * o);
+  um_gather<PR>(R1, single, gi, gb, L);
+}
+
+template <bool PR>
+__device__ __forceinline__ void um_pair_qs(UmLoads (&L)[2], bool same) {
+  if (PR) {
+    L[0].qs = L[0].qp.x;
+    L[1].qs = same ? L[0].qp.x : L[0].qp.y;
+  }
+}
+
+template <bool PR>
 __device__ __forceinline__ void um_gather(const float* __restrict__ R1, unsigned single, unsigned gi, unsigned gb, UmLoads& L) {
   L.t0 = ldf4(R1, 16u * gi);
   L.t1 = ldf4(R1 + 4, 16u * gi);
   L.b0 = ldf4(R1, 16u * gb);
   L.b1 = ldf4(R1 + 4, 16u * gb);
-  L.ts = ldf2(R1, single + 4u * gi);
-  L.bs = ldf2(R1, single + 4u * gb);
-}
-
+  if (!PR) {
+    L.ts = ldf2(R1, single + 4u * gi);
+    L.bs = ldf2(R1, single + 4u * gb);
+  } else {
+    L.p4 = *reinterpret_cast<const f4pr*>(reinterpret_cast<const char*>(R1) + (single + 8u * gi));
+  }
+}
+
+template <bool PR>
 __device__ __forceinline__ void um_finish(const UmLoads& L, int h, int w, int x, int y, float2 f, float m[5]) {
   const float dx = f.x, dy = f.y;
   float fx = x + dx, fy = y + dy;
@@ -1256,7 +1300,8 @@
     r3 = a00 * L.t0.y + a01 * L.t1.y + a10 * L.b0.y + a11 * L.b1.y;
     r4 = a00 * L.t0.z + a01 * L.t1.z + a10 * L.b0.z + a11 * L.b1.z;
     r5 = a00 * L.t0.w + a01 * L.t1.w + a10 * L.b0.w + a11 * L.b1.w;
-    r6 = a00 * L.ts.x + a01 * L.ts.y + a10 * L.bs.x + a11 * L.bs.y;
+    if (!PR) r6 = a00 * L.ts.x + a01 * L.ts.y + a10 * L.bs.x + a11 * L.bs.y;
+    else r6 = a00 * L.p4.x + a01 * L.p4.z + a10 * L.p4.y + a11 * L.p4.w;
     r4 = (L.q.z + r4) * 0.5f;
     r5 = (L.q.w + r5) * 0.5f;
     r6 = (L.qs + r6) * 0.25f;
@@ -1837,7 +1882,7 @@
   bx = col % gx; by = col / gx; bz = pair;
 }
 
-template <int MODE>
+template <int MODE, bool PR>
 __global__ __launch_bounds__(B2_T, 2) void k_flow_iter3(IterArgs a) {
   typedef float f2v __attribute__((ext_vector_type(2)));
   constexpr int M = 7, W = 2 * M + 1, RB = 2;
@@ -1866,8 +1911,8 @@
   const float* __restrict__ R0;
   const float* __restrict__ R1;
   if (a.pairs) {
-    R0 = a.R + (size_t)a.pairs[2 * pr] * 5 * (size_t)np;
-    R1 = a.R + (size_t)a.pairs[2 * pr + 1] * 5 * (size_t)np;
+    R0 = a.R + (size_t)a.pairs[2 * pr] * (PR ? 6 : 5) * (size_t)np;
+    R1 = a.R + (size_t)a.pairs[2 * pr + 1] * (PR ? 6 : 5) * (size_t)np;
   } else {
     R0 = a.R;
     R1 = a.R1_direct;
@@ -1886,10 +1931,10 @@
     for (int i = 0; i < 3; ++i) {
       const int yy = d_clamp(y0 - M + s0 + i, 0, h - 1);
       f[i] = iter_flow_at<MODE>(a, fin, C, cx, xc, yy);
-      um_issue(R0, R1, np, h, w, xc, yy, f[i], Li[i]);
-    }
-#pragma unroll
-    for (int i = 0; i < 3; ++i) um_finish(Li[i], h, w, xc, d_clamp(y0 - M + s0 + i, 0, h - 1), f[i], ring[s0 + i]);
+      um_issue<PR>(R0, R1, np, h, w, xc, yy, f[i], Li[i]);
+    }
+#pragma unroll
+    for (int i = 0; i < 3; ++i) um_finish<PR>(Li[i], h, w, xc, d_clamp(y0 - M + s0 + i, 0, h - 1), f[i], ring[s0 + i]);
     __builtin_amdgcn_sched_barrier(0);
   }
 #pragma unroll
@@ -1921,7 +1966,8 @@
 #pragma unroll
   for (int r = 0; r < RB; ++r) {
     fcur[r] = iter_flow_at<MODE>(a, fin, C, cx, xc, d_clamp(y0 + r + M + 1, 0, h - 1));
-    um_issue(R0, R1, np, h, w, xc, d_clamp(y0 + r + M + 1, 0, h - 1), fcur[r], L[r]);
+    if (r == 0) um_issue<PR, UM_QS_PAIR>(R0, R1, np, h, w, xc, d_clamp(y0 + r + M + 1, 0, h - 1), fcur[r], L[r]);
+    else um_issue<PR, UM_QS_NONE>(R0, R1, np, h, w, xc, d_clamp(y0 + r + M + 1, 0, h - 1), fcur[r], L[r]);
   }
 #pragma unroll
   for (int r = 0; r < RB; ++r) fnext[r] = iter_flow_at<MODE>(a, fin, C, cx, xc, d_clamp(y0 + RB + r + M + 1, 0, h - 1));
@@ -1977,11 +2023,12 @@
 #pragma unroll
       for (int bb = 0; bb < F3_GROUP / RB; ++bb) {
         const int ybb = yg + bb * RB;
+        um_pair_qs<PR>(L, d_clamp(ybb + M + 2, 0, h - 1) == d_clamp(ybb + M + 1, 0, h - 1));
 #pragma unroll
         for (int r = 0; r < RB; ++r) {
           const int t = g * F3_GROUP + bb * RB + r;
           float m[5];
-          um_finish(L[r], h, w, xc, d_clamp(ybb + r + M + 1, 0, h - 1), fcur[r], m);
+          um_finish<PR>(L[r], h, w, xc, d_clamp(ybb + r + M + 1, 0, h - 1), fcur[r], m);
 #pragma unroll
           for (int c = 0; c < 5; ++c) {
             Vs[bb * RB + r][c][vpos] = (float)vs[c];
@@ -1990,7 +2037,8 @@
             ring[(t + W) % F3_RING][c] = m[c];
           }
           fcur[r] = fnext[r];
-          um_issue(R0, R1, np, h, w, xc, d_clamp(ybb + RB + r + M + 1, 0, h - 1), fcur[r], L[r]);
+          if (r == 0) um_issue<PR, UM_QS_PAIR>(R0, R1, np, h, w, xc, d_clamp(ybb + RB + r + M + 1, 0, h - 1), fcur[r], L[r]);
+          else um_issue<PR, UM_QS_NONE>(R0, R1, np, h, w, xc, d_clamp(ybb + RB + r + M + 1, 0, h - 1), fcur[r], L[r]);
         }
         if (MODE == FLOW_COARSE2) {
           coarse2_window_batch(a, C, cx, ybb + 2 * RB + M + 1, win, fnext);
@@ -2057,7 +2105,7 @@
   static_assert(THREADS <= 1024, "workgroup size");
 };
 
-template <int NCW, int MODE>
+template <int NCW, int MODE, bool PR>
 __global__ __launch_bounds__((FrGeom<NCW>::THREADS)) void k_flow_iter_roles(IterArgs a) {
   typedef FrGeom<NCW> G;
   constexpr int M = 7, W = 15, RB = 2;
@@ -2085,8 +2133,8 @@
     const float* __restrict__ R0;
     const float* __restrict__ R1;
     if (a.pairs) {
-      R0 = a.R + (size_t)a.pairs[2 * pr] * 5 * (size_t)np;
-      R1 = a.R + (size_t)a.pairs[2 * pr + 1] * 5 * (size_t)np;
+      R0 = a.R + (size_t)a.pairs[2 * pr] * (PR ? 6 : 5) * (size_t)np;
+      R1 = a.R + (size_t)a.pairs[2 * pr + 1] * (PR ? 6 : 5) * (size_t)np;
     } else {
       R0 = a.R;
       R1 = a.R1_direct;
@@ -2103,7 +2151,8 @@
 #pragma unroll
     for (int r = 0; r < RB; ++r) {
       fcur[r] = iter_flow_at<MODE>(a, fin, C, cx, xc, rowk(r));
-      um_issue(R0, R1, np, h, w, xc, rowk(r), fcur[r], L[r]);
+      if (r == 0) um_issue<PR, UM_QS_PAIR>(R0, R1, np, h, w, xc, rowk(r), fcur[r], L[r]);
+      else um_issue<PR, UM_QS_NONE>(R0, R1, np, h, w, xc, rowk(r), fcur[r], L[r]);
     }
 #pragma unroll
     for (int r = 0; r < RB; ++r) fnext[r] = iter_flow_at<MODE>(a, fin, C, cx, xc, rowk(RB + r));
@@ -2123,14 +2172,16 @@
             for (int bb = 0; bb < NB; ++bb) {
               const int k0 = FR_G * s + bb * RB;
               const int i0 = bb * RB;
+              um_pair_qs<PR>(L, rowk(k0 + 1) == rowk(k0));
 #pragma unroll
               for (int r = 0; r < RB; ++r) {
                 float m[5];
-                um_finish(L[r], h, w, xc, rowk(k0 + r), fcur[r], m);
+                um_finish<PR>(L[r], h, w, xc, rowk(k0 + r), fcur[r], m);
 #pragma unroll
                 for (int c = 0; c < 5; ++c) Mb[u][i0 + r][c][t] = m[c];
                 fcur[r] = fnext[r];
-                um_issue(R0, R1, np, h, w, xc, rowk(k0 + RB + r), fcur[r], L[r]);
+                if (r == 0) um_issue<PR, UM_QS_PAIR>(R0, R1, np, h, w, xc, rowk(k0 + RB + r), fcur[r], L[r]);
+                else um_issue<PR, UM_QS_NONE>(R0, R1, np, h, w, xc, rowk(k0 + RB + r), fcur[r], L[r]);
               }
               if (MODE == FLOW_COARSE2) {
                 int ysb[RB];
@@ -2323,7 +2374,7 @@
 constexpr int FT_T = 32, FT_M = 7, FT_S = FT_T + 2 * FT_M, FT_NT = 512;
 static_assert(FT_T == F3_ANCHOR && FT_T % F3_SW == 0 && B2_OUT % F3_SW == 0, "tile anchors must coincide with k_flow_iter3's");
 
-template <int MODE>
+template <int MODE, bool PR>
 __global__ __launch_bounds__(FT_NT) void k_flow_iter_tile(IterArgs a) {
   constexpr int W = 2 * FT_M + 1;
   constexpr int NSEG = FT_T / F3_SW;
@@ -2337,8 +2388,8 @@
   const float* __restrict__ R0;
   const float* __restrict__ R1;
   if (a.pairs) {
-    R0 = a.R + (size_t)a.pairs[2 * pr] * 5 * (size_t)np;
-    R1 = a.R + (size_t)a.pairs[2 * pr + 1] * 5 * (size_t)np;
+    R0 = a.R + (size_t)a.pairs[2 * pr] * (PR ? 6 : 5) * (size_t)np;
+    R1 = a.R + (size_t)a.pairs[2 * pr + 1] * (PR ? 6 : 5) * (size_t)np;
   } else {
     R0 = a.R;
     R1 = a.R1_direct;
@@ -2369,12 +2420,12 @@
     UmLoads L[CH];
 #pragma unroll
     for (int j = 0; j < CH; ++j)
-      if (k0 + j < NI) um_issue(R0, R1, np, h, w, px[k0 + j], py[k0 + j], fl[k0 + j], L[j]);
+      if (k0 + j < NI) um_issue<PR>(R0, R1, np, h, w, px[k0 + j], py[k0 + j], fl[k0 + j], L[j]);
 #pragma unroll
     for (int j = 0; j < CH; ++j) {
       if (k0 + j < NI) {
         float m[5];
-        um_finish(L[j], h, w, px[k0 + j], py[k0 + j], fl[k0 + j], m);
+        um_finish<PR>(L[j], h, w, px[k0 + j], py[k0 + j], fl[k0 + j], m);
         const int i = tid + FT_NT * (k0 + j);
         if (i < FT_S * FT_S) {
           const int ty = i / FT_S, tx = i - ty * FT_S;
@@ -2674,7 +2725,7 @@
 static bool polyexp_frame_fits(int h, int w) { return (unsigned long long)h * (unsigned long long)w <= (1ull << 26); }
 
 int launch_polyexp(st_ctx* ctx, const float* img, int n, int h, int w, int poly_n, double poly_sigma, float* R,
-                   const uint8_t* gray = nullptr) {
+                   const uint8_t* gray = nullptr, bool pr = false) {
   if (!polyexp_frame_fits(h, w)) return st_set_error(ctx, ST_ERR_UNSUPPORTED, "polyexp: frames above 64 M pixels are not supported");
   PolyArgs a;
   a.img = img; a.gray = gray; a.R = R; a.h = h; a.w = w;
@@ -2684,16 +2735,18 @@
   dim3 grid(strips, (h + a.rows_per_seg - 1) / a.rows_per_seg, n);
   st_timed t(ctx, ST_K_POLYEXP);
   if (gray && w < 8) return st_set_error(ctx, ST_ERR_INVALID, "polyexp: the gray-source instance needs rows of at least 8 pixels");
-  if (gray && poly_n == 5) hipLaunchKernelGGL(k_polyexp_u8<5>, grid, dim3(256), 0, ctx->stream, a);
-  else if (gray) hipLaunchKernelGGL(k_polyexp_u8<7>, grid, dim3(256), 0, ctx->stream, a);
-  else if (poly_n == 5) hipLaunchKernelGGL(k_polyexp<5>, grid, dim3(256), 0, ctx->stream, a);
-  else hipLaunchKernelGGL(k_polyexp<7>, grid, dim3(256), 0, ctx->stream, a);
+#define ST_POLY_LAUNCH(K, N) do { if (pr) hipLaunchKernelGGL((K<N, true>), grid, dim3(256), 0, ctx->stream, a); \
+                                   else hipLaunchKernelGGL((K<N, false>), grid, dim3(256), 0, ctx->stream, a); } while (0)
+  if (gray && poly_n == 5) ST_POLY_LAUNCH(k_polyexp_u8, 5);
+  else if (gray) ST_POLY_LAUNCH(k_polyexp_u8, 7);
+  else if (poly_n == 5) ST_POLY_LAUNCH(k_polyexp, 5);
+  else ST_POLY_LAUNCH(k_polyexp, 7);
   ST_HIP(ctx, hipGetLastError());
   return ST_OK;
 }
 
 int launch_polyexp_ml(st_ctx* ctx, float* const* imgs, const LevelGeom* geom, float* const* R, const int* ks, int nk, int n,
-                      int poly_n, double poly_sigma) {
+                      int poly_n, double poly_sigma, bool pr) {
   if (nk < 1 || nk > 4) return st_set_error(ctx, ST_ERR_INVALID, "polyexp: bad level list");
   PolyArgsML a;
   memset(&a, 0, sizeof(a));
@@ -2711,8 +2764,10 @@
     blocks += l.strips * ((g.lh + l.rows_per_seg - 1) / l.rows_per_seg);
   }
   st_timed t(ctx, ST_K_POLYEXP);
-  if (poly_n == 5) hipLaunchKernelGGL(k_polyexp_ml<5>, dim3(blocks, n), dim3(256), 0, ctx->stream, a);
-  else hipLaunchKernelGGL(k_polyexp_ml<7>, dim3(blocks, n), dim3(256), 0, ctx->stream, a);
+  const dim3 grid(blocks, n);
+  if (poly_n == 5) ST_POLY_LAUNCH(k_polyexp_ml, 5);
+  else ST_POLY_LAUNCH(k_polyexp_ml, 7);
+#undef ST_POLY_LAUNCH
   ST_HIP(ctx, hipGetLastError());
   return ST_OK;
 }
@@ -2751,16 +2806,19 @@
   return ST_OK;
 }
 
-int launch_flow_iter(st_ctx* ctx, IterArgs a, int n_pairs) {
+#define ST_ITER_LAUNCH(K, GRID, BLK, ...) do { \
+    if (pr) hipExtLaunchKernelGGL((K<__VA_ARGS__, true>), GRID, BLK, 0, ctx->stream, e0, e1, 0, a); \
+    else hipExtLaunchKernelGGL((K<__VA_ARGS__, false>), GRID, BLK, 0, ctx->stream, e0, e1, 0, a); } while (0)
+int launch_flow_iter(st_ctx* ctx, IterArgs a, int n_pairs, bool pr) {
   hipEvent_t e0, e1;
   constexpr long long kTilePx = 600000;
   const bool tile = ctx->tile_mode == 1 || (ctx->tile_mode != 0 && (long long)n_pairs * a.h * a.w <= kTilePx);
   if (tile && (a.h + FT_T - 1) / FT_T <= 65535) {
     dim3 grid((a.w + FT_T - 1) / FT_T, (a.h + FT_T - 1) / FT_T, n_pairs);
     ST_TRY(st_time_dispatch(ctx, ST_K_BLUR_UPDATE, &e0, &e1));
-    if (a.coarse) hipExtLaunchKernelGGL((k_flow_iter_tile<FLOW_COARSE>), grid, dim3(FT_NT), 0, ctx->stream, e0, e1, 0, a);
-    else if (a.flow_in) hipExtLaunchKernelGGL((k_flow_iter_tile<FLOW_FIELD>), grid, dim3(FT_NT), 0, ctx->stream, e0, e1, 0, a);
-    else hipExtLaunchKernelGGL((k_flow_iter_tile<FLOW_ZERO>), grid, dim3(FT_NT), 0, ctx->stream, e0, e1, 0, a);
+    if (a.coarse) ST_ITER_LAUNCH(k_flow_iter_tile, grid, dim3(FT_NT), FLOW_COARSE);
+    else if (a.flow_in) ST_ITER_LAUNCH(k_flow_iter_tile, grid, dim3(FT_NT), FLOW_FIELD);
+    else ST_ITER_LAUNCH(k_flow_iter_tile, grid, dim3(FT_NT), FLOW_ZERO);
     ST_HIP(ctx, hipGetLastError());
     return ST_OK;
   }
@@ -2807,16 +2865,16 @@
       const int mode = a.coarse ? (a.h == 2 * a.ch ? FLOW_COARSE2 : FLOW_COARSE) : (a.flow_in ? FLOW_FIELD : FLOW_ZERO);
       if (best_ncw == 5) {
         const dim3 blk(FrGeom<5>::THREADS);
-        if (mode == FLOW_COARSE2) hipExtLaunchKernelGGL((k_flow_iter_roles<5, FLOW_COARSE2>), grid, blk, 0, ctx->stream, e0, e1, 0, a);
-        else if (mode == FLOW_COARSE) hipExtLaunchKernelGGL((k_flow_iter_roles<5, FLOW_COARSE>), grid, blk, 0, ctx->stream, e0, e1, 0, a);
-        else if (mode == FLOW_FIELD) hipExtLaunchKernelGGL((k_flow_iter_roles<5, FLOW_FIELD>), grid, blk, 0, ctx->stream, e0, e1, 0, a);
-        else hipExtLaunchKernelGGL((k_flow_iter_roles<5, FLOW_ZERO>), grid, blk, 0, ctx->stream, e0, e1, 0, a);
+        if (mode == FLOW_COARSE2) ST_ITER_LAUNCH(k_flow_iter_roles, grid, blk, 5, FLOW_COARSE2);
+        else if (mode == FLOW_COARSE) ST_ITER_LAUNCH(k_flow_iter_roles, grid, blk, 5, FLOW_COARSE);
+        else if (mode == FLOW_FIELD) ST_ITER_LAUNCH(k_flow_iter_roles, grid, blk, 5, FLOW_FIELD);
+        else ST_ITER_LAUNCH(k_flow_iter_roles, grid, blk, 5, FLOW_ZERO);
       } else {
         const dim3 blk(FrGeom<4>::THREADS);
-        if (mode == FLOW_COARSE2) hipExtLaunchKernelGGL((k_flow_iter_roles<4, FLOW_COARSE2>), grid, blk, 0, ctx->stream, e0, e1, 0, a);
-        else if (mode == FLOW_COARSE) hipExtLaunchKernelGGL((k_flow_iter_roles<4, FLOW_COARSE>), grid, blk, 0, ctx->stream, e0, e1, 0, a);
-        else if (mode == FLOW_FIELD) hipExtLaunchKernelGGL((k_flow_iter_roles<4, FLOW_FIELD>), grid, blk, 0, ctx->stream, e0, e1, 0, a);
-        else hipExtLaunchKernelGGL((k_flow_iter_roles<4, FLOW_ZERO>), grid, blk, 0, ctx->stream, e0, e1, 0, a);
+        if (mode == FLOW_COARSE2) ST_ITER_LAUNCH(k_flow_iter_roles, grid, blk, 4, FLOW_COARSE2);
+        else if (mode == FLOW_COARSE) ST_ITER_LAUNCH(k_flow_iter_roles, grid, blk, 4, FLOW_COARSE);
+        else if (mode == FLOW_FIELD) ST_ITER_LAUNCH(k_flow_iter_roles, grid, blk, 4, FLOW_FIELD);
+        else ST_ITER_LAUNCH(k_flow_iter_roles, grid, blk, 4, FLOW_ZERO);
       }
       ST_HIP(ctx, hipGetLastError());
       return ST_OK;
@@ -2836,13 +2894,14 @@
   dim3 grid(strips, nseg3, n_pairs);
   ST_TRY(st_time_dispatch(ctx, ST_K_BLUR_UPDATE, &e0, &e1));
   const int mode = a.coarse ? (a.h == 2 * a.ch ? FLOW_COARSE2 : FLOW_COARSE) : (a.flow_in ? FLOW_FIELD : FLOW_ZERO);
-  if (mode == FLOW_COARSE2) hipExtLaunchKernelGGL((k_flow_iter3<FLOW_COARSE2>), grid, dim3(B2_T), 0, ctx->stream, e0, e1, 0, a);
-  else if (mode == FLOW_COARSE) hipExtLaunchKernelGGL((k_flow_iter3<FLOW_COARSE>), grid, dim3(B2_T), 0, ctx->stream, e0, e1, 0, a);
-  else if (mode == FLOW_FIELD) hipExtLaunchKernelGGL((k_flow_iter3<FLOW_FIELD>), grid, dim3(B2_T), 0, ctx->stream, e0, e1, 0, a);
-  else hipExtLaunchKernelGGL((k_flow_iter3<FLOW_ZERO>), grid, dim3(B2_T), 0, ctx->stream, e0, e1, 0, a);
+  if (mode == FLOW_COARSE2) ST_ITER_LAUNCH(k_flow_iter3, grid, dim3(B2_T), FLOW_COARSE2);
+  else if (mode == FLOW_COARSE) ST_ITER_LAUNCH(k_flow_iter3, grid, dim3(B2_T), FLOW_COARSE);
+  else if (mode == FLOW_FIELD) ST_ITER_LAUNCH(k_flow_iter3, grid, dim3(B2_T), FLOW_FIELD);
+  else ST_ITER_LAUNCH(k_flow_iter3, grid, dim3(B2_T), FLOW_ZERO);
   ST_HIP(ctx, hipGetLastError());
   return ST_OK;
 }
+#undef ST_ITER_LAUNCH
 
 bool fused_path(int h, int w, const st_fb_params& p) {
   if (p.win_size != 15) return false;
@@ -2854,7 +2913,7 @@
   return true;
 }
 
-size_t pass_bytes(int h, int w, const st_fb_params& p, int nf, int npairs) {
+size_t pass_bytes(int h, int w, const st_fb_params& p, int nf, int npairs, bool r_pairs) {
   const int levels = fb_levels(h, w, p);
   size_t np0 = (size_t)h * w;
   size_t maxCoarse = 0;
@@ -2870,7 +2929,7 @@
     for (int k = 1; k <= 3; ++k) b += st_align_up(sizeof(float) * (np0 >> (2 * k)) * nf);
   for (int k = 0; k <= levels; ++k) {
     LevelGeom g = fb_level_geom(h, w, p, k);
-    b += st_align_up(sizeof(float) * 5 * (size_t)g.lh * g.lw * nf);
+    b += st_align_up(sizeof(float) * (r_pairs ? 6 : 5) * (size_t)g.lh * g.lw * nf);
   }
   b += 2 * st_align_up(sizeof(float) * (fused_path(h, w, p) ? 2 : 5) * np0 * npairs);
   b += 2 * st_align_up(sizeof(float) * 2 * (maxCoarse ? maxCoarse : 1) * npairs);
@@ -2882,7 +2941,8 @@
                    const st_fb_params& p, float* const* outs) {
   const int levels = fb_levels(h, w, p);
   const size_t np0 = (size_t)h * w;
-  ST_TRY(st_ws_reserve(ctx, pass_bytes(h, w, p, nf, npairs)));
+  const bool r_pairs = ctx->r_pairs && fused_path(h, w, p);
+  ST_TRY(st_ws_reserve(ctx, pass_bytes(h, w, p, nf, npairs, r_pairs)));
   uint8_t* gray = (uint8_t*)st_ws_alloc(ctx, np0 * nf);
   float* img = (float*)st_ws_alloc(ctx, sizeof(float) * np0 * nf);
   const bool pyr1 = pyr_fused_ok(h, w, p);
@@ -2899,7 +2959,7 @@
     geom[k] = fb_level_geom(h, w, p, k);
     size_t npk = (size_t)geom[k].lh * geom[k].lw;
     if (k >= 1 && npk > maxCoarse) maxCoarse = npk;
-    R[k] = (float*)st_ws_alloc(ctx, sizeof(float) * 5 * npk * nf);
+    R[k] = (float*)st_ws_alloc(ctx, sizeof(float) * (r_pairs ? 6 : 5) * npk * nf);
   }
   float* M[2];
   const bool fused = fused_path(h, w, p);
@@ -2944,12 +3004,12 @@
   if (single) {
     int ks[4], nk = 0;
     for (int k = 0; k <= levels; ++k) ks[nk++] = k;
-    ST_TRY(launch_polyexp_ml(ctx, imgs, geom.data(), R.data(), ks, nk, nf, p.poly_n, p.poly_sigma));
+    ST_TRY(launch_polyexp_ml(ctx, imgs, geom.data(), R.data(), ks, nk, nf, p.poly_n, p.poly_sigma, r_pairs));
   } else {
     for (int k = levels; k >= 0; --k) {
       if (!pyr1) ST_TRY(launch_pyr(ctx, gray, nf, h, w, geom[k], img));
       ST_TRY(launch_polyexp(ctx, pyr1 ? imgs[k] : img, nf, geom[k].lh, geom[k].lw, p.poly_n, p.poly_sigma, R[k],
-                            k == 0 && poly_u8 ? gray : nullptr));
+                            k == 0 && poly_u8 ? gray : nullptr, r_pairs));
     }
   }
   if (fused) {
@@ -2979,7 +3039,7 @@
         } else {
           q.flow_out = fbuf[it & 1];
         }
-        ST_TRY(launch_flow_iter(ctx, q, npairs));
+        ST_TRY(launch_flow_iter(ctx, q, npairs, r_pairs));
       }
       cur ^= 1;
     }
@@ -3077,7 +3137,7 @@
           }
           pp.push_back(slot[f]);
         }
-      if (pass_bytes(h, w, p, (int)pf.size(), count) <= ctx->ws_limit || count == 1) break;
+      if (pass_bytes(h, w, p, (int)pf.size(), count, ctx->r_pairs && fused_path(h, w, p)) <= ctx->ws_limit || count == 1) break;
       count = (count + 1) / 2;
     }
     ST_TRY(farneback_pass(ctx, pf.data(), (int)pf.size(), pp.data(), count, h, w, p, flow_out_dev + start));
@@ -3170,7 +3230,7 @@
   } else {
     q.flow_in = flow_in_dev;
   }
-  return launch_flow_iter(ctx, q, 1);
+  return launch_flow_iter(ctx, q, 1, false);
 }
 
 ST_EXPORT int st_fb_update_flow_blur(st_ctx* ctx, const float* r0_dev, const float* r1_dev, const float* m_in_dev, int h,
diff --git a/scannertools_amd/csrc/st_internal.h b/scannertools_amd/csrc/st_internal.h
--- a/scannertools_amd/csrc/st_internal.h
+++ b/scannertools_amd/csrc/st_internal.h
@@ -26,6 +26,7 @@
   hipStream_t stream = nullptr;
   int tile_mode = -1;
   bool poly_u8 = true;
+  bool r_pairs = true;
   bool fold_gray = false;
   int roles_mode = -1, roles_ncw = 0, pyr_roles = -1;
   bool pyr_roles_rgb = true;
```

Result: slower. 10110 (-3.0%).
